# ShreyasBhaktharam/RDEIC

Hardware: AMD Instinct MI355X
Metric: 512x512 images/sec encode+relay-decode @ fixed bpp; 1/2/4/8 GPU (higher is better)
Workload: dtype bf16; 1 GPU; config 2: global batch 16 (16/GPU) 512x512, 2-step relay DDIM, encode+entropy-code+decode+VAE-decode; global_batch=16, image_size=512, ddim_steps=2, sampler=ddim, parallelism=dp1, codec_sessions_per_gpu=5

## Files before the change

### include/rdeic_hip.h

```cpp
#ifndef RDEIC_HIP_H
#define RDEIC_HIP_H
#include <stddef.h>
#include <stdint.h>
#ifdef __cplusplus
extern "C" {
#endif

int rdeic_version(void);
int rdeic_abi_count(void);

typedef struct rdeic_conv_desc {
  const void* in0;
  const void* in1;
  int32_t c0, c1;
  int32_t ld0, ld1;
  int32_t n, h, w;
  int32_t up2;
  const void* weight;
  int32_t wld;
  const float* bias;
  int32_t cout, kh, kw, stride, pad_t, pad_l;
  int32_t ho, wo;
  const float* gn_ab;
  int32_t gn_silu;
  const float* emb;
  int32_t emb_ld;
  int32_t act;
  float act_param;
  const void* res;
  int32_t res_ld;
  void* out;
  int32_t out_ld;
  int32_t out_mode;
  int32_t dtype;
  int32_t out_f32;
  int32_t batch;
  int64_t in_bs, w_bs, out_bs;
  float* gn_part;
  int32_t gn_hw;
  int32_t reserved;
  const float* ln_rows;
  const float* ln_colsum;
} rdeic_conv_desc;

int rdeic_conv2d(const rdeic_conv_desc* d, void* stream);
int rdeic_conv2d_tile(const rdeic_conv_desc* d, int32_t tile, void* stream);
int rdeic_conv2d_splitk(const rdeic_conv_desc* d, int32_t splits, float* ws, size_t ws_floats, void* stream);
int rdeic_conv2d_up2_phases(const rdeic_conv_desc* d, int64_t phase_stride, int32_t tile, void* stream);
int rdeic_conv2d_up2_group(const rdeic_conv_desc* d);
int rdeic_set_conv_path(int32_t path);
int rdeic_set_conv_option(int32_t key, int32_t value);

size_t rdeic_groupnorm_ws_floats(int32_t n, int32_t hw, int32_t c);
size_t rdeic_groupnorm_parts_floats(int64_t rows, int32_t c, int32_t hw);
int rdeic_groupnorm_parts_ab(const float* p0, int32_t c0, const float* p1, int32_t c1, int32_t n, int32_t hw,
                             int32_t groups, float eps, const float* gamma, const float* beta, float* ab,
                             void* stream);
int rdeic_groupnorm_stats(const void* x0, int32_t c0, int32_t ld0, const void* x1, int32_t c1, int32_t ld1,
                          int32_t n, int32_t hw, int32_t groups, float eps, const float* gamma, const float* beta,
                          float* ab, float* ws, int32_t dtype, void* stream);
int rdeic_groupnorm_parts_apply(const float* p0, int32_t c0, const float* p1, int32_t c1, const void* x0, int32_t ld0,
                                const void* x1, int32_t ld1, int32_t n, int32_t hw, int32_t groups, float eps,
                                const float* gamma, const float* beta, int32_t silu, float* ab, void* y, int32_t yld,
                                void* stream);
int rdeic_groupnorm_apply(const void* x, int32_t n, int32_t hw, int32_t c, int32_t ld, const float* ab,
                          int32_t ab_c, int32_t silu, float out_mul, void* y, int32_t yld, int32_t dtype,
                          void* stream);
int rdeic_layernorm(const void* x, int32_t rows, int32_t c, int32_t ld, const float* gamma, const float* beta,
                    float eps, void* y, int32_t yld, int32_t dtype, void* stream);

int rdeic_attention(const void* q, int32_t ldq, const void* k, int32_t ldk, const void* v, int32_t ldv,
                    void* o, int32_t ldo, int32_t batch, int32_t heads, int32_t lq, int32_t lk, int32_t dh,
                    float scale, int32_t kv_bcast, int32_t dtype, void* stream);
int rdeic_softmax_rows(const float* s, int64_t rows, int32_t cols, float scale, void* p, int32_t dtype, void* stream);
int rdeic_transpose(const void* in, int32_t rows, int32_t cols, int32_t ldin, void* out, int32_t ldout,
                    int32_t batch, int64_t in_bs, int64_t out_bs, int32_t dtype, void* stream);

int rdeic_geglu(const void* in, int32_t rows, int32_t c, int32_t ldin, void* out, int32_t ldout,
                int32_t dtype, void* stream);
int rdeic_nchw_to_nhwc(const float* in, int32_t n, int32_t c, int32_t h, int32_t w, float mul, float add,
                       void* out, int32_t ld, int32_t dtype, void* stream);
int rdeic_nhwc_to_nchw(const void* in, int32_t n, int32_t c, int32_t h, int32_t w, int32_t ld, float mul,
                       float add, float* out, int32_t dtype, void* stream);
int rdeic_axpby(const float* x, const float* z, int32_t n_img, int32_t per_img, const float* a,
                const float* b, float* y, void* stream);
int rdeic_timestep_embedding(const int64_t* t, const float* freqs, int32_t n, int32_t dim, float* out, void* stream);
int rdeic_ddim_step(const float* x, const float* e, int64_t count, float c_sq1m, float c_sqa, float c_sqap,
                    float c_dir, float* xp, float* x0, void* stream);
int rdeic_cfg_combine(const float* e_cond, const float* e_uncond, int64_t count, float scale, float* out,
                      void* stream);
int rdeic_spaced_step(const float* x, const float* e, const float* noise, int64_t count, float a, float b, float c1,
                      float c2, float s, float* xp, float* x0, void* stream);
int rdeic_silu_f32(const float* x, float* y, int64_t count, void* stream);
int rdeic_image_u8_to_nhwc(const uint8_t* img, int32_t n, int32_t h, int32_t w, void* out, int32_t ld,
                           int32_t dtype, void* stream);
int rdeic_nhwc_to_image_u8(const void* x, int32_t n, int32_t h, int32_t w, int32_t ld, uint8_t* img,
                           int32_t dtype, void* stream);
int rdeic_image_mse(const uint8_t* a, const uint8_t* b, int32_t n, int64_t per_img, float* out, void* stream);
int rdeic_fill_uniform(float* out, int64_t count, uint64_t seed, float scale, float offset, void* stream);
int rdeic_pack_conv_weight(const float* w, int32_t cout, int32_t cin, int32_t kh, int32_t kw, void* out,
                           int32_t wld, int32_t dtype, void* stream);
int rdeic_cast(const void* in, int32_t in_dtype, void* out, int32_t out_dtype, int64_t count, void* stream);

int rdeic_ckbd_encode(const void* y, int32_t yld, const void* params, int32_t pld, int32_t n, int32_t hy,
                      int32_t wy, int32_t c, int32_t phase, const float* scale_table, int32_t levels,
                      float scale_bound, int32_t* sym, int32_t* idx, int64_t img_stride, int64_t off,
                      void* yhat, int32_t yhld, void* anchor_out, int32_t ald, int32_t dtype, void* stream);
int rdeic_ckbd_indexes(const void* params, int32_t pld, int32_t n, int32_t hy, int32_t wy, int32_t c,
                       int32_t phase, const float* scale_table, int32_t levels, float scale_bound,
                       int32_t* idx, int64_t img_stride, int64_t off, int32_t dtype, void* stream);
int rdeic_ckbd_dequant(const int32_t* sym, const void* params, int32_t pld, int32_t n, int32_t hy,
                       int32_t wy, int32_t c, int32_t phase, int64_t img_stride, int64_t off, void* yhat,
                       int32_t yhld, void* anchor_out, int32_t ald, int32_t dtype, void* stream);
int rdeic_vq_argmin(const float* dot, const float* zn, const float* en, int32_t rows, int32_t ncode, int32_t* idx,
                    void* stream);
int rdeic_gather_rows(const float* table, int32_t ld_table, const int32_t* idx, int32_t rows, int32_t dim,
                      void* out, int32_t ld_out, int32_t dtype, void* stream);
int rdeic_row_sqnorm(const void* x, int32_t rows, int32_t dim, int32_t ld, float* out, int32_t dtype,
                     void* stream);

size_t rdeic_image_ssim_ws_floats(int32_t n, int32_t h, int32_t w, int32_t levels);
int rdeic_image_ssim(const uint8_t* a, const uint8_t* b, int32_t n, int32_t h, int32_t w, int32_t levels, float* ws,
                     size_t ws_floats, float* out, void* stream);

int rdeic_lpips_prep(const uint8_t* img, int32_t n, int32_t h, int32_t w, float* out, void* stream);
int rdeic_maxpool2d(const float* in, int32_t n, int32_t h, int32_t w, int32_t c, int32_t ld_in, int32_t k,
                    int32_t s, float* out, int32_t ld_out, void* stream);
size_t rdeic_lpips_layer_ws_floats(int32_t n, int64_t hw, int32_t c);
int rdeic_lpips_layer(const float* f0, int32_t ld0, const float* f1, int32_t ld1, const float* lin, int32_t n,
                      int64_t hw, int32_t c, int32_t accumulate, float* ws, size_t ws_floats, float* out,
                      void* stream);

int rdeic_pmf_to_quantized_cdf(const float* pmf, int32_t n, int32_t precision, uint32_t* cdf_out);
int rdeic_build_gaussian_tables(const float* pmf, const int32_t* pmf_len, int32_t levels, int32_t pmf_ld,
                                int32_t* cdf, int32_t cdf_ld, int32_t* cdf_len, void* reserved);

int rdeic_rans_encode(const int32_t* sym, const int32_t* idx, size_t n, const int32_t* cdf, int32_t cdf_ld,
                      const int32_t* cdf_len, const int32_t* offset, int32_t levels, uint8_t* out, size_t cap,
                      size_t* out_len);
int rdeic_rans_encode_batch(int32_t count, const int32_t* sym, const int32_t* idx, size_t n_per,
                            size_t stride, const int32_t* cdf, int32_t cdf_ld, const int32_t* cdf_len,
                            const int32_t* offset, int32_t levels, uint8_t* out, size_t cap_per,
                            size_t* out_len, int32_t threads);
void* rdeic_rans_enc_tables_create(const int32_t* cdf, int32_t cdf_ld, const int32_t* cdf_len,
                                   const int32_t* offset, int32_t levels);
void rdeic_rans_enc_tables_destroy(void* tables);
int rdeic_rans_encode_batch_t(const void* tables, int32_t count, const int32_t* sym, const int32_t* idx,
                              size_t n_per, size_t stride, uint8_t* out, size_t cap_per, size_t* out_len,
                              int32_t threads);
int rdeic_rans_enc_quotient(const void* tables, int32_t row, int32_t value, uint64_t x, uint64_t* q);
void* rdeic_rans_dec_open(const uint8_t* data, size_t len);
int rdeic_rans_decode(void* handle, const int32_t* idx, size_t n, const int32_t* cdf, int32_t cdf_ld,
                      const int32_t* cdf_len, const int32_t* offset, int32_t levels, int32_t* out);
int rdeic_rans_decode_batch(int32_t count, void** handles, const int32_t* idx, size_t n_per, size_t stride,
                            const int32_t* cdf, int32_t cdf_ld, const int32_t* cdf_len, const int32_t* offset,
                            int32_t levels, int32_t* out, int32_t threads);
void rdeic_rans_dec_close(void* handle);

int rdeic_ac_encode(const int16_t* sym, size_t n, const int16_t* cdf_row, int32_t lp, uint8_t* out,
                    size_t cap, size_t* out_len);
int rdeic_ac_decode(const uint8_t* data, size_t len, size_t n, const int16_t* cdf_row, int32_t lp,
                    int16_t* out);
int rdeic_ac_uniform_cdf(int32_t codebook_size, int16_t* cdf_row);

#define RDEIC_PROF_CONV 0
#define RDEIC_PROF_ATTN 1
#define RDEIC_PROF_ATTN_SMALL 2
#define RDEIC_PROF_GN_STATS 3
#define RDEIC_PROF_GN_APPLY 4
#define RDEIC_PROF_GEMM 5
#define RDEIC_PROF_ATTN_D512 6
#define RDEIC_PROF_CONV_BYTES 7
int rdeic_prof_start(int32_t capacity, int32_t every);
int rdeic_prof_read_keys(int32_t kind, int64_t* keys, int64_t* launches, double* work, double* ms, int32_t cap);
#define RDEIC_COUNT_HALO_CONV 0
#define RDEIC_COUNT_GN_APPLY 1
#define RDEIC_COUNT_LAYERNORM 2
#define RDEIC_COUNT_HALO_SMALL 3
#define RDEIC_COUNT_LN_FUSED 4
#define RDEIC_COUNT_SPLITK 5
#define RDEIC_COUNT_EDGE 6
#define RDEIC_COUNT_GN_PARTS_APPLY 7
#define RDEIC_COUNT_KINDS 8
int64_t rdeic_launch_count(int32_t kind);
int rdeic_layernorm_rowstats(const void* x, int32_t rows, int32_t c, int32_t ld, float eps, float* ms,
                             void* stream);
int rdeic_launch_count_reset(void);
int rdeic_prof_stop(void);
int rdeic_prof_read(int32_t kind, int64_t* launches, double* work, double* ms);

typedef struct rdeic_gemm_desc {
  const void* a;
  int64_t a_bs1, a_bs2, a_sm, a_sk;
  const void* b;
  int64_t b_bs1, b_bs2, b_sk, b_sn;
  void* c;
  int64_t c_bs1, c_bs2, c_sm;
  int32_t batch, nb2, m, n, k, ksplit, dtype, c_f32;
  float alpha, beta;
  float* rsum;
  int64_t rsum_bs;
} rdeic_gemm_desc;
int rdeic_gemm_strided(const rdeic_gemm_desc* d, void* stream);
int rdeic_pack_conv_weight_dgrad(const float* w, int32_t cout, int32_t cin, int32_t kh, int32_t kw, void* out,
                                 int32_t wld, int32_t to_bf16, void* stream);
typedef struct rdeic_pack_job {
  const float* w;
  void* out;
  int64_t start;
  int32_t cout, cin, kh, kw, wld, mode;
} rdeic_pack_job;
int rdeic_pack_batch(const rdeic_pack_job* jobs, int32_t njobs, int64_t total, int32_t row_floats, int32_t to_bf16,
                     void* stream);
int rdeic_zero_insert2(const void* src, int32_t n, int32_t h, int32_t w, int32_t c, int32_t ld, void* dst,
                       int32_t dst_ld, int32_t dtype, void* stream);
int rdeic_sum_pool2(const void* src, int32_t n, int32_t h, int32_t w, int32_t c, int32_t ld, void* dst,
                    int32_t dst_ld, int32_t dtype, void* stream);
int rdeic_pixel_unshuffle2(const void* src, int32_t n, int32_t h, int32_t w, int32_t c, int32_t ld, void* dst,
                           int32_t dst_ld, int32_t dtype, void* stream);
int rdeic_im2col(const void* x, int32_t n, int32_t h, int32_t w, int32_t c, int32_t ld, int32_t kh, int32_t kw,
                 int32_t stride, int32_t pad_t, int32_t pad_l, int32_t ho, int32_t wo, int32_t up2, void* out,
                 int64_t out_ld, int32_t dtype, void* stream);
int rdeic_wgrad_finalize(const float* part, int32_t splits, int32_t cout, int32_t cin, int32_t kh, int32_t kw,
                         float* dw, int32_t accumulate, const float* rpart, float* db, void* stream);
size_t rdeic_col_sum_ws_floats(int64_t rows, int32_t c, int32_t groups);
int rdeic_col_sum(const void* x, int64_t rows, int32_t c, int32_t ld, int32_t groups, float* out, int32_t accumulate,
                  float* ws, size_t ws_floats, int32_t dtype, void* stream);
int rdeic_act_fwd(const void* z, int64_t rows, int32_t c, int32_t ldz, const void* res, int32_t ldr, int32_t act,
                  float slope, void* out, int32_t ldo, int32_t dtype, void* stream);
int rdeic_act_bwd(const void* dy, int32_t ldy, const void* z, int32_t ldz, int64_t rows, int32_t c, int32_t act,
                  float slope, void* dz, int32_t lddz, int32_t dtype, void* stream);
size_t rdeic_gn_train_ws_doubles(int32_t n, int32_t hw, int32_t c);
int rdeic_gn_train_fwd(const void* x, int32_t ldx, int32_t n, int32_t hw, int32_t c, int32_t groups, float eps,
                       const float* gamma, const float* beta, float* mr, float* ab, double* ws, int32_t dtype,
                       void* stream);
int rdeic_gn_train_bwd(const void* x, int32_t ldx, const void* dy, int32_t ldy, int32_t n, int32_t hw, int32_t c,
                       int32_t groups, const float* mr, const float* gamma, const float* beta, int32_t silu, void* dx,
                       int32_t lddx, float* dgamma, float* dbeta, int32_t accumulate, double* ws, float* coef,
                       int32_t dtype, void* stream);
int rdeic_gn_train_bwd_res(const void* x, int32_t ldx, const void* dy, int32_t ldy, int32_t n, int32_t hw, int32_t c,
                           int32_t groups, const float* mr, const float* gamma, const float* beta, int32_t silu,
                           const void* dres, int32_t ldr, void* dx, int32_t lddx, float* dgamma, float* dbeta,
                           int32_t accumulate, double* ws, float* coef, int32_t dtype, void* stream);
size_t rdeic_layernorm_bwd_ws_floats(int64_t rows, int32_t c);
int rdeic_layernorm_bwd(const void* x, int32_t ldx, int64_t rows, int32_t c, const float* gamma, float eps,
                        const void* dy, int32_t ldy, void* dx, int32_t lddx, float* dgamma, float* dbeta,
                        int32_t accumulate, float* ws, size_t ws_floats, int32_t dtype, void* stream);
int rdeic_layernorm_bwd_res(const void* x, int32_t ldx, int64_t rows, int32_t c, const float* gamma, float eps,
                            const void* dy, int32_t ldy, const void* dres, int32_t ldr, void* dx, int32_t lddx,
                            float* dgamma, float* dbeta, int32_t accumulate, float* ws, size_t ws_floats,
                            int32_t dtype, void* stream);
int rdeic_softmax_bwd_rows(const void* p, const float* dp, int64_t rows, int32_t cols, float scale, void* ds,
                           int32_t dtype, void* stream);
int rdeic_attention_fwd_lse(const void* q, int32_t ldq, const void* k, int32_t ldk, const void* v, int32_t ldv,
                            void* o, int32_t ldo, float* lse, int32_t batch, int32_t heads, int32_t lq, int32_t lk,
                            int32_t dh, float scale, int32_t dtype, void* stream);
size_t rdeic_attention_bwd_workspace(int32_t batch, int32_t heads, int32_t lq, int32_t lk, int32_t dh);
int rdeic_attention_bwd(const void* q, int32_t ldq, const void* k, int32_t ldk, const void* v, int32_t ldv,
                        const void* o, int32_t ldo, const void* d_o, int32_t lddo, const float* lse,
                        void* dq, int32_t lddq, void* dk, int32_t lddk, void* dv, int32_t lddv,
                        void* ws, size_t ws_bytes, int32_t batch, int32_t heads, int32_t lq, int32_t lk,
                        int32_t dh, float scale, int32_t dtype, void* stream);
int rdeic_geglu_bwd(const void* x, int32_t ldx, int64_t rows, int32_t c, const void* dy, int32_t ldy, void* dx,
                    int32_t lddx, int32_t dtype, void* stream);
int rdeic_ckbd_train_anchor(const void* y, int32_t ldy, const void* pa, int32_t ldpa, int32_t n, int32_t h, int32_t w,
                            int32_t c, void* out, int32_t ldo, int32_t dtype, void* stream);
int rdeic_ckbd_mask(const void* x, int32_t ldx, int32_t n, int32_t h, int32_t w, int32_t c, int32_t which, void* out,
                    int32_t ldo, int32_t dtype, void* stream);
size_t rdeic_ckbd_train_ws_doubles(int32_t n, int32_t h, int32_t w, int32_t c);
int rdeic_ckbd_train_lik(const void* y, int32_t ldy, const void* pa, int32_t ldpa, const void* pn, int32_t ldpn,
                         const float* noise, int32_t n, int32_t h, int32_t w, int32_t c, void* nonanchor_hat,
                         int32_t ldo, double* ws, float* out2, int32_t dtype, void* stream);
int rdeic_ckbd_train_lik_bwd(const void* y, int32_t ldy, const void* pa, int32_t ldpa, const void* pn, int32_t ldpn,
                             const float* noise, int32_t n, int32_t h, int32_t w, int32_t c, const float* g_sum,
                             const void* d_nonanchor, int32_t ldd, void* dy, int32_t lddy, void* dpa, int32_t lddpa,
                             void* dpn, int32_t lddpn, int32_t dtype, void* stream);
int rdeic_vq_train(const float* dot, const float* zn, const float* en, const float* z, const int32_t* idx, int32_t P,
                   int32_t K, int32_t D, float* E, float* embed_prob, float beta, float decay, float temp,
                   float* code_out, float* dE_unit, float* loss3, void* stream);
int rdeic_vq_z_grad(const float* z, const float* zq, const void* dzq, int64_t count, const float* g_loss, float coef,
                    void* dz, int32_t dtype, void* stream);
int rdeic_scale_dev(const float* x, int64_t count, const float* s, float* y, int32_t accumulate, void* stream);
int rdeic_adamw(float* p, const float* g, float* m, float* v, int64_t count, float lr, float beta1, float beta2,
                float eps, float weight_decay, int32_t step, void* stream);
int rdeic_adamw_dev(float* p, const float* g, float* m, float* v, int64_t count, float lr, float beta1, float beta2,
                    float eps, float weight_decay, const float* step_scalars, void* stream);

#ifdef __cplusplus
}
#endif
#endif
```

### rdeic_amd/_lib.py

```python
from __future__ import annotations

import ctypes as C
import os
import threading

_HERE = os.path.dirname(os.path.abspath(__file__))
LIB_PATH = os.environ.get("RDEIC_LIB") or os.path.join(_HERE, "lib", "librdeic_hip.so")

EINVAL, ENOSPC, EBADMSG, ELAUNCH = -22, -28, -74, -5
_ERRNAMES = {EINVAL: "EINVAL (bad argument/shape)", ENOSPC: "ENOSPC (output capacity)",
             EBADMSG: "EBADMSG (corrupt or truncated bitstream)", ELAUNCH: "kernel launch failure"}


class RdeicError(RuntimeError):
    def __init__(self, fn: str, code: int):
        super().__init__(f"{fn} failed: {code} {_ERRNAMES.get(code, '')}")
        self.code = code


class BitstreamError(RdeicError, ValueError):
    """Corrupt / truncated bitstream (the reference's 'decode failure')."""


class ConvDesc(C.Structure):
    _fields_ = [
        ("in0", C.c_void_p), ("in1", C.c_void_p),
        ("c0", C.c_int32), ("c1", C.c_int32), ("ld0", C.c_int32), ("ld1", C.c_int32),
        ("n", C.c_int32), ("h", C.c_int32), ("w", C.c_int32), ("up2", C.c_int32),
        ("weight", C.c_void_p), ("wld", C.c_int32),
        ("bias", C.c_void_p),
        ("cout", C.c_int32), ("kh", C.c_int32), ("kw", C.c_int32), ("stride", C.c_int32),
        ("pad_t", C.c_int32), ("pad_l", C.c_int32),
        ("ho", C.c_int32), ("wo", C.c_int32),
        ("gn_ab", C.c_void_p), ("gn_silu", C.c_int32),
        ("emb", C.c_void_p), ("emb_ld", C.c_int32),
        ("act", C.c_int32), ("act_param", C.c_float),
        ("res", C.c_void_p), ("res_ld", C.c_int32),
        ("out", C.c_void_p), ("out_ld", C.c_int32), ("out_mode", C.c_int32),
        ("dtype", C.c_int32), ("out_f32", C.c_int32),
        ("batch", C.c_int32), ("in_bs", C.c_int64), ("w_bs", C.c_int64), ("out_bs", C.c_int64),
        ("gn_part", C.c_void_p), ("gn_hw", C.c_int32), ("reserved", C.c_int32),
        ("ln_rows", C.c_void_p), ("ln_colsum", C.c_void_p),
    ]


class GemmDesc(C.Structure):
    _fields_ = [
        ("a", C.c_void_p), ("a_bs1", C.c_int64), ("a_bs2", C.c_int64), ("a_sm", C.c_int64), ("a_sk", C.c_int64),
        ("b", C.c_void_p), ("b_bs1", C.c_int64), ("b_bs2", C.c_int64), ("b_sk", C.c_int64), ("b_sn", C.c_int64),
        ("c", C.c_void_p), ("c_bs1", C.c_int64), ("c_bs2", C.c_int64), ("c_sm", C.c_int64),
        ("batch", C.c_int32), ("nb2", C.c_int32), ("m", C.c_int32), ("n", C.c_int32), ("k", C.c_int32),
        ("ksplit", C.c_int32), ("dtype", C.c_int32), ("c_f32", C.c_int32),
        ("alpha", C.c_float), ("beta", C.c_float), ("rsum", C.c_void_p), ("rsum_bs", C.c_int64),
    ]


_p, _i32, _i64, _u64, _f, _sz = C.c_void_p, C.c_int32, C.c_int64, C.c_uint64, C.c_float, C.c_size_t

PROTOTYPES = {
    "rdeic_version": (C.c_int, []),
    "rdeic_abi_count": (C.c_int, []),
    "rdeic_conv2d": (C.c_int, [C.POINTER(ConvDesc), _p]),
    "rdeic_conv2d_splitk": (C.c_int, [C.POINTER(ConvDesc), _i32, _p, C.c_size_t, _p]),
    "rdeic_conv2d_tile": (C.c_int, [C.POINTER(ConvDesc), _i32, _p]),
    "rdeic_conv2d_up2_phases": (C.c_int, [C.POINTER(ConvDesc), _i64, _i32, _p]),
    "rdeic_conv2d_up2_group": (C.c_int, [C.POINTER(ConvDesc)]),
    "rdeic_prof_start": (C.c_int, [_i32, _i32]),
    "rdeic_prof_stop": (C.c_int, []),
    "rdeic_launch_count": (C.c_int64, [_i32]),
    "rdeic_launch_count_reset": (C.c_int, []),
    "rdeic_layernorm_rowstats": (C.c_int, [C.c_void_p, _i32, _i32, _i32, C.c_float, C.c_void_p, C.c_void_p]),
    "rdeic_prof_read": (C.c_int, [_i32, C.POINTER(C.c_int64), C.POINTER(C.c_double), C.POINTER(C.c_double)]),
    "rdeic_prof_read_keys": (C.c_int, [_i32, C.POINTER(C.c_int64), C.POINTER(C.c_int64), C.POINTER(C.c_double),
                                       C.POINTER(C.c_double), _i32]),
    "rdeic_groupnorm_ws_floats": (_sz, [_i32, _i32, _i32]),
    "rdeic_groupnorm_stats": (C.c_int, [_p, _i32, _i32, _p, _i32, _i32, _i32, _i32, _i32, _f, _p, _p, _p, _p,
                                        _i32, _p]),
    "rdeic_groupnorm_apply": (C.c_int, [_p, _i32, _i32, _i32, _i32, _p, _i32, _i32, _f, _p, _i32, _i32, _p]),
    "rdeic_set_conv_path": (C.c_int, [_i32]),
    "rdeic_set_conv_option": (C.c_int, [_i32, _i32]),
    "rdeic_layernorm": (C.c_int, [_p, _i32, _i32, _i32, _p, _p, _f, _p, _i32, _i32, _p]),
    "rdeic_softmax_rows": (C.c_int, [_p, _i64, _i32, _f, _p, _i32, _p]),
    "rdeic_transpose": (C.c_int, [_p, _i32, _i32, _i32, _p, _i32, _i32, _i64, _i64, _i32, _p]),
    "rdeic_attention": (C.c_int, [_p, _i32, _p, _i32, _p, _i32, _p, _i32, _i32, _i32, _i32, _i32, _i32, _f,
                                  _i32, _i32, _p]),
    "rdeic_geglu": (C.c_int, [_p, _i32, _i32, _i32, _p, _i32, _i32, _p]),
    "rdeic_nchw_to_nhwc": (C.c_int, [_p, _i32, _i32, _i32, _i32, _f, _f, _p, _i32, _i32, _p]),
    "rdeic_nhwc_to_nchw": (C.c_int, [_p, _i32, _i32, _i32, _i32, _i32, _f, _f, _p, _i32, _p]),
    "rdeic_axpby": (C.c_int, [_p, _p, _i32, _i32, _p, _p, _p, _p]),
    "rdeic_timestep_embedding": (C.c_int, [_p, _p, _i32, _i32, _p, _p]),
    "rdeic_ddim_step": (C.c_int, [_p, _p, _i64, _f, _f, _f, _f, _p, _p, _p]),
    "rdeic_spaced_step": (C.c_int, [_p, _p, _p, _i64, _f, _f, _f, _f, _f, _p, _p, _p]),
    "rdeic_cfg_combine": (C.c_int, [_p, _p, _i64, _f, _p, _p]),
    "rdeic_silu_f32": (C.c_int, [_p, _p, _i64, _p]),
    "rdeic_image_u8_to_nhwc": (C.c_int, [_p, _i32, _i32, _i32, _p, _i32, _i32, _p]),
    "rdeic_nhwc_to_image_u8": (C.c_int, [_p, _i32, _i32, _i32, _i32, _p, _i32, _p]),
    "rdeic_image_mse": (C.c_int, [_p, _p, _i32, _i64, _p, _p]),
    "rdeic_fill_uniform": (C.c_int, [_p, _i64, _u64, _f, _f, _p]),
    "rdeic_pack_conv_weight": (C.c_int, [_p, _i32, _i32, _i32, _i32, _p, _i32, _i32, _p]),
    "rdeic_cast": (C.c_int, [_p, _i32, _p, _i32, _i64, _p]),
    "rdeic_ckbd_encode": (C.c_int, [_p, _i32, _p, _i32, _i32, _i32, _i32, _i32, _i32, _p, _i32, _f, _p, _p,
                                    _i64, _i64, _p, _i32, _p, _i32, _i32, _p]),
    "rdeic_ckbd_indexes": (C.c_int, [_p, _i32, _i32, _i32, _i32, _i32, _i32, _p, _i32, _f, _p, _i64, _i64,
                                     _i32, _p]),
    "rdeic_ckbd_dequant": (C.c_int, [_p, _p, _i32, _i32, _i32, _i32, _i32, _i32, _i64, _i64, _p, _i32, _p,
                                     _i32, _i32, _p]),
    "rdeic_vq_argmin": (C.c_int, [_p, _p, _p, _i32, _i32, _p, _p]),
    "rdeic_gather_rows": (C.c_int, [_p, _i32, _p, _i32, _i32, _p, _i32, _i32, _p]),
    "rdeic_row_sqnorm": (C.c_int, [_p, _i32, _i32, _i32, _p, _i32, _p]),
    "rdeic_pmf_to_quantized_cdf": (C.c_int, [_p, _i32, _i32, _p]),
    "rdeic_build_gaussian_tables": (C.c_int, [_p, _p, _i32, _i32, _p, _i32, _p, _p]),
    "rdeic_rans_encode": (C.c_int, [_p, _p, _sz, _p, _i32, _p, _p, _i32, _p, _sz, C.POINTER(_sz)]),
    "rdeic_rans_encode_batch": (C.c_int, [_i32, _p, _p, _sz, _sz, _p, _i32, _p, _p, _i32, _p, _sz, _p, _i32]),
    "rdeic_image_ssim_ws_floats": (C.c_size_t, [_i32, _i32, _i32, _i32]),
    "rdeic_image_ssim": (C.c_int, [_p, _p, _i32, _i32, _i32, _i32, _p, C.c_size_t, _p, _p]),
    "rdeic_lpips_prep": (C.c_int, [_p, _i32, _i32, _i32, _p, _p]),
    "rdeic_maxpool2d": (C.c_int, [_p, _i32, _i32, _i32, _i32, _i32, _i32, _i32, _p, _i32, _p]),
    "rdeic_lpips_layer_ws_floats": (_sz, [_i32, _i64, _i32]),
    "rdeic_lpips_layer": (C.c_int, [_p, _i32, _p, _i32, _p, _i32, _i64, _i32, _i32, _p, _sz, _p, _p]),
    "rdeic_groupnorm_parts_floats": (C.c_size_t, [_i64, _i32, _i32]),
    "rdeic_groupnorm_parts_ab": (C.c_int, [_p, _i32, _p, _i32, _i32, _i32, _i32, _f, _p, _p, _p, _p]),
    "rdeic_groupnorm_parts_apply": (C.c_int, [_p, _i32, _p, _i32, _p, _i32, _p, _i32, _i32, _i32, _i32, _f, _p, _p,
                                              _i32, _p, _p, _i32, _p]),
    "rdeic_rans_enc_tables_create": (_p, [_p, _i32, _p, _p, _i32]),
    "rdeic_rans_enc_tables_destroy": (None, [_p]),
    "rdeic_rans_encode_batch_t": (C.c_int, [_p, _i32, _p, _p, _sz, _sz, _p, _sz, _p, _i32]),
    "rdeic_rans_enc_quotient": (C.c_int, [_p, _i32, _i32, C.c_uint64, C.POINTER(C.c_uint64)]),
    "rdeic_rans_dec_open": (_p, [_p, _sz]),
    "rdeic_rans_decode": (C.c_int, [_p, _p, _sz, _p, _i32, _p, _p, _i32, _p]),
    "rdeic_rans_decode_batch": (C.c_int, [_i32, _p, _p, _sz, _sz, _p, _i32, _p, _p, _i32, _p, _i32]),
    "rdeic_rans_dec_close": (None, [_p]),
    "rdeic_ac_encode": (C.c_int, [_p, _sz, _p, _i32, _p, _sz, C.POINTER(_sz)]),
    "rdeic_ac_decode": (C.c_int, [_p, _sz, _sz, _p, _i32, _p]),
    "rdeic_ac_uniform_cdf": (C.c_int, [_i32, _p]),
    "rdeic_gemm_strided": (C.c_int, [C.POINTER(GemmDesc), _p]),
    "rdeic_pack_conv_weight_dgrad": (C.c_int, [_p, _i32, _i32, _i32, _i32, _p, _i32, _i32, _p]),
    "rdeic_pack_batch": (C.c_int, [_p, _i32, _i64, _i32, _i32, _p]),
    "rdeic_zero_insert2": (C.c_int, [_p, _i32, _i32, _i32, _i32, _i32, _p, _i32, _i32, _p]),
    "rdeic_sum_pool2": (C.c_int, [_p, _i32, _i32, _i32, _i32, _i32, _p, _i32, _i32, _p]),
    "rdeic_pixel_unshuffle2": (C.c_int, [_p, _i32, _i32, _i32, _i32, _i32, _p, _i32, _i32, _p]),
    "rdeic_im2col": (C.c_int, [_p, _i32, _i32, _i32, _i32, _i32, _i32, _i32, _i32, _i32, _i32, _i32, _i32, _i32, _p,
                               _i64, _i32, _p]),
    "rdeic_wgrad_finalize": (C.c_int, [_p, _i32, _i32, _i32, _i32, _i32, _p, _i32, _p, _p, _p]),
    "rdeic_col_sum_ws_floats": (_sz, [_i64, _i32, _i32]),
    "rdeic_col_sum": (C.c_int, [_p, _i64, _i32, _i32, _i32, _p, _i32, _p, _sz, _i32, _p]),
    "rdeic_act_fwd": (C.c_int, [_p, _i64, _i32, _i32, _p, _i32, _i32, _f, _p, _i32, _i32, _p]),
    "rdeic_act_bwd": (C.c_int, [_p, _i32, _p, _i32, _i64, _i32, _i32, _f, _p, _i32, _i32, _p]),
    "rdeic_gn_train_ws_doubles": (_sz, [_i32, _i32, _i32]),
    "rdeic_gn_train_fwd": (C.c_int, [_p, _i32, _i32, _i32, _i32, _i32, _f, _p, _p, _p, _p, _p, _i32, _p]),
    "rdeic_gn_train_bwd": (C.c_int, [_p, _i32, _p, _i32, _i32, _i32, _i32, _i32, _p, _p, _p, _i32, _p, _i32, _p, _p,
                                     _i32, _p, _p, _i32, _p]),
    "rdeic_gn_train_bwd_res": (C.c_int, [_p, _i32, _p, _i32, _i32, _i32, _i32, _i32, _p, _p, _p, _i32, _p, _i32, _p,
                                         _i32, _p, _p, _i32, _p, _p, _i32, _p]),
    "rdeic_layernorm_bwd_ws_floats": (_sz, [_i64, _i32]),
    "rdeic_layernorm_bwd": (C.c_int, [_p, _i32, _i64, _i32, _p, _f, _p, _i32, _p, _i32, _p, _p, _i32, _p, _sz, _i32,
                                      _p]),
    "rdeic_layernorm_bwd_res": (C.c_int, [_p, _i32, _i64, _i32, _p, _f, _p, _i32, _p, _i32, _p, _i32, _p, _p, _i32, _p,
                                          _sz, _i32, _p]),
    "rdeic_softmax_bwd_rows": (C.c_int, [_p, _p, _i64, _i32, _f, _p, _i32, _p]),
    "rdeic_attention_fwd_lse": (C.c_int, [_p, _i32, _p, _i32, _p, _i32, _p, _i32, _p, _i32, _i32, _i32, _i32, _i32, _f,
                                          _i32, _p]),
    "rdeic_attention_bwd_workspace": (_sz, [_i32, _i32, _i32, _i32, _i32]),
    "rdeic_attention_bwd": (C.c_int, [_p, _i32, _p, _i32, _p, _i32, _p, _i32, _p, _i32, _p, _p, _i32, _p, _i32, _p,
                                      _i32, _p, _sz, _i32, _i32, _i32, _i32, _i32, _f, _i32, _p]),
    "rdeic_geglu_bwd": (C.c_int, [_p, _i32, _i64, _i32, _p, _i32, _p, _i32, _i32, _p]),
    "rdeic_ckbd_train_anchor": (C.c_int, [_p, _i32, _p, _i32, _i32, _i32, _i32, _i32, _p, _i32, _i32, _p]),
    "rdeic_ckbd_mask": (C.c_int, [_p, _i32, _i32, _i32, _i32, _i32, _i32, _p, _i32, _i32, _p]),
    "rdeic_ckbd_train_ws_doubles": (_sz, [_i32, _i32, _i32, _i32]),
    "rdeic_ckbd_train_lik": (C.c_int, [_p, _i32, _p, _i32, _p, _i32, _p, _i32, _i32, _i32, _i32, _p, _i32, _p, _p,
                                       _i32, _p]),
    "rdeic_ckbd_train_lik_bwd": (C.c_int, [_p, _i32, _p, _i32, _p, _i32, _p, _i32, _i32, _i32, _i32, _p, _p, _i32, _p,
                                           _i32, _p, _i32, _p, _i32, _i32, _p]),
    "rdeic_vq_train": (C.c_int, [_p, _p, _p, _p, _p, _i32, _i32, _i32, _p, _p, _f, _f, _f, _p, _p, _p, _p]),
    "rdeic_vq_z_grad": (C.c_int, [_p, _p, _p, _i64, _p, _f, _p, _i32, _p]),
    "rdeic_scale_dev": (C.c_int, [_p, _i64, _p, _p, _i32, _p]),
    "rdeic_adamw": (C.c_int, [_p, _p, _p, _p, _i64, _f, _f, _f, _f, _f, _i32, _p]),
    "rdeic_adamw_dev": (C.c_int, [_p, _p, _p, _p, _i64, _f, _f, _f, _f, _f, _p, _p]),
}

_lib = None
_lock = threading.Lock()


def load() -> C.CDLL:
    global _lib
    if _lib is not None:
        return _lib
    with _lock:
        if _lib is not None:
            return _lib
        if not os.path.exists(LIB_PATH):
            raise ImportError(f"librdeic_hip.so not built at {LIB_PATH}; run `make` (or __graft_entry__.build()).")
        import torch
        lib = C.CDLL(LIB_PATH, mode=C.RTLD_GLOBAL)
        for name, (res, args) in PROTOTYPES.items():
            fn = getattr(lib, name)
            fn.restype = res
            fn.argtypes = args
        _lib = lib
    return _lib


def check(name: str, rc: int) -> None:
    if rc != 0:
        if rc == EBADMSG:
            raise BitstreamError(name, rc)
        raise RdeicError(name, rc)


RECORDER = None


def call(name: str, *args, tag=None) -> None:
    fn = getattr(load(), name)
    if RECORDER is not None:
        RECORDER.append((name, fn, args, tag))
    rc = fn(*args)
    check(name, rc)


def call_soft(name: str, *args, tag=None) -> bool:
    fn = getattr(load(), name)
    rc = fn(*args)
    if rc == 1:
        return False
    check(name, rc)
    if RECORDER is not None:
        RECORDER.append((name, fn, args, tag))
    return True
```

### rdeic_amd/csrc/coders.cpp

```cpp
#include <stdint.h>
#include <string.h>

#include <algorithm>
#include <atomic>
#include <condition_variable>
#include <functional>
#include <mutex>
#include <cmath>
#include <new>
#include <stdexcept>
#include <thread>
#include <vector>

#include "../../include/rdeic_hip.h"

#define RDEIC_OK 0
#define RDEIC_EINVAL (-22)
#define RDEIC_ENOSPC (-28)
#define RDEIC_EBADMSG (-74)

namespace {

constexpr int kPrecision = 16;
constexpr uint32_t kBypassBits = 4;
// ... 94 lines not shown
  if (freq < 2) {
    s.rcp = ~0ull;
    s.shift = 0;
    s.bias = start + (1u << kPrecision) - 1;
  } else {
    uint32_t sh = 0;
    while (freq > (1u << sh)) ++sh;
    const unsigned __int128 num = ((unsigned __int128)1 << (sh + 63)) + (freq - 1);
    s.rcp = (uint64_t)(num / freq);
    s.shift = (uint8_t)(sh - 1);
    s.bias = start;
  }
  return s;
}

inline uint64_t enc_quot(uint64_t x, const EncSym& s) {
  return (uint64_t)(((unsigned __int128)x * s.rcp) >> 64) >> s.shift;
}

struct WordSink {
  std::vector<uint32_t>& buf;
  size_t wp;
  explicit WordSink(std::vector<uint32_t>& b) : buf(b), wp(b.size()) {}
  void emit(uint32_t w) {
    if (wp == 0) grow();
    buf[--wp] = w;
  }
  void grow() {
    const size_t old = buf.size(), add = std::max<size_t>(old, 1024);
    std::vector<uint32_t> nb(old + add);
    memcpy(nb.data() + add, buf.data(), old * sizeof(uint32_t));
    buf.swap(nb);
    wp += add;
  }
};

inline void enc_put(uint64_t& x, WordSink& ws, const EncSym& s) {
  if ((x >> 47) >= s.freq) {
    ws.emit((uint32_t)x);
    x >>= 32;
  }
  x = x + s.bias + enc_quot(x, s) * ((1u << kPrecision) - s.freq);
}

inline void enc_put_bits(uint64_t& x, WordSink& ws, uint32_t v) {
  if ((x >> 59) != 0) {
    ws.emit((uint32_t)x);
    x >>= 32;
  }
  x = (x << kBypassBits) | v;
}

int rans_encode_tab_impl(const EncTables& T, const int32_t* sym, const int32_t* idx, size_t n, uint8_t* out,
                         size_t cap, size_t* out_len, std::vector<uint32_t>& buf) {
  if (buf.size() < n / 2 + 256) buf.assign(n / 2 + 256, 0u);
  WordSink ws(buf);
  uint64_t x = kRansL;
  for (size_t i = n; i-- > 0;) {
    const int32_t ci = idx[i];
    if (ci < 0 || ci >= T.levels) return RDEIC_EINVAL;
    const int32_t max_value = T.max_value[ci];
    int32_t value = sym[i] - T.offset[ci];
    if (value < 0 || value >= max_value) {
      const uint32_t raw = value < 0 ? (uint32_t)(-2 * (int64_t)value - 1) : (uint32_t)(2 * (int64_t)(value - max_value));
      int32_t nb = 0;
      while (nb < 8 && (raw >> (nb * kBypassBits)) != 0) ++nb;
      for (int32_t j = nb; j-- > 0;) enc_put_bits(x, ws, (raw >> (j * kBypassBits)) & kBypassMax);
      enc_put_bits(x, ws, (uint32_t)(nb % (int32_t)kBypassMax));
      for (int32_t v = nb / (int32_t)kBypassMax; v-- > 0;) enc_put_bits(x, ws, kBypassMax);
      value = max_value;
    }
    enc_put(x, ws, T.sym[(size_t)T.row_off[ci] + value]);
  }
  ws.emit((uint32_t)(x >> 32));
  ws.emit((uint32_t)x);
  const size_t nbytes = (ws.buf.size() - ws.wp) * 4;
  *out_len = nbytes;
  if (nbytes > cap) return RDEIC_ENOSPC;
  memcpy(out, ws.buf.data() + ws.wp, nbytes);
  return RDEIC_OK;
}

struct RansDecoder {
  std::vector<uint32_t> words;
  size_t pos = 0;
  uint64_t x = 0;
  bool bad = false;

  bool read_word(uint32_t& w) {
    if (pos >= words.size()) { bad = true; return false; }
    w = words[pos++];
    return true;
  }
  uint32_t get_bits(uint32_t nbits) {
    uint32_t v = (uint32_t)(x & ((1u << nbits) - 1));
    x >>= nbits;
    if (x < kRansL) {
      uint32_t w;
      if (read_word(w)) x = (x << 32) | w;
    }
    return v;
  }
};

int rans_decode_impl(RansDecoder* d, const int32_t* idx, size_t n, const int32_t* cdf, int32_t cdf_ld,
                     const int32_t* cdf_len, const int32_t* offset, int32_t levels, int32_t* out) {
  if (d->bad) return RDEIC_EBADMSG;
  for (size_t i = 0; i < n; ++i) {
    const int32_t ci = idx[i];
    if (ci < 0 || ci >= levels) return RDEIC_EINVAL;
    const int32_t* row = cdf + (size_t)ci * cdf_ld;
    const int32_t len = cdf_len[ci];
    const int32_t max_value = len - 2;
    if (max_value < 0 || len > cdf_ld) return RDEIC_EINVAL;
    const uint32_t cum = (uint32_t)(d->x & ((1u << kPrecision) - 1));
    const int32_t* it = std::upper_bound(row, row + len, (int32_t)cum);
    int32_t s = (int32_t)(it - row) - 1;
    if (s < 0 || s >= len - 1) return RDEIC_EBADMSG;
    const uint64_t start = (uint32_t)row[s], freq = (uint32_t)(row[s + 1] - row[s]);
    uint64_t x = d->x;
    x = freq * (x >> kPrecision) + (x & ((1u << kPrecision) - 1)) - start;
    if (x < kRansL) {
      uint32_t w;
      if (!d->read_word(w)) return RDEIC_EBADMSG;
      x = (x << 32) | w;
    }
    d->x = x;
    int32_t value = s;
    if (value == max_value) {
      int32_t v = (int32_t)d->get_bits(kBypassBits);
      int32_t nb = v;
      while (v == (int32_t)kBypassMax) {
        if (d->bad || nb > 8) return RDEIC_EBADMSG;
        v = (int32_t)d->get_bits(kBypassBits);
        nb += v;
      }
      if (nb > 8) return RDEIC_EBADMSG;
      uint32_t raw = 0;
      for (int32_t j = 0; j < nb; ++j) {
        uint32_t nib = d->get_bits(kBypassBits);
        raw |= nib << (j * kBypassBits);
      }
      if (d->bad) return RDEIC_EBADMSG;
      value = (int32_t)(raw >> 1);
      if (raw & 1)
        value = -value - 1;
      else
        value += max_value;
    }
    out[i] = value + offset[ci];
  }
  return d->bad ? RDEIC_EBADMSG : RDEIC_OK;
}

class WorkerPool {
 public:
  static WorkerPool& get() {
    thread_local WorkerPool* p = new WorkerPool();
    return *p;
  }
  void run(int32_t count, int32_t threads, const std::function<void(int32_t)>& f) {
    std::lock_guard<std::mutex> job(job_mu_);
    int32_t helpers = std::max(0, std::min(threads, count) - 1);
    while ((int32_t)workers_.size() < helpers) {
      const int32_t id = (int32_t)workers_.size();
      try {
        workers_.reserve(workers_.size() + 1);
        std::thread(&WorkerPool::loop, this, id).detach();
      } catch (...) {
        helpers = (int32_t)workers_.size();
        break;
      }
      workers_.push_back(id);
    }
    {
      std::lock_guard<std::mutex> lk(mu_);
      fn_ = &f;
      count_ = count;
      next_.store(0);
      helpers_ = helpers;
      active_ = helpers;
      ++gen_;
    }
    cv_.notify_all();
    work();
    std::unique_lock<std::mutex> lk(mu_);
    done_cv_.wait(lk, [&] { return active_ == 0; });
    fn_ = nullptr;
  }

 private:
  void work() {
    for (;;) {
      const int32_t i = next_.fetch_add(1);
      if (i >= count_) break;
      (*fn_)(i);
    }
  }
  void loop(int32_t id) {
    uint64_t seen = 0;
    for (;;) {
      {
        std::unique_lock<std::mutex> lk(mu_);
        cv_.wait(lk, [&] { return gen_ != seen; });
        seen = gen_;
        if (id >= helpers_) continue;
      }
      work();
      std::lock_guard<std::mutex> lk(mu_);
      if (--active_ == 0) done_cv_.notify_all();
    }
  }

  std::mutex job_mu_, mu_;
  std::condition_variable cv_, done_cv_;
  std::vector<int32_t> workers_;
  const std::function<void(int32_t)>* fn_ = nullptr;
  std::atomic<int32_t> next_{0};
  int32_t count_ = 0, active_ = 0, helpers_ = 0;
  uint64_t gen_ = 0;
};

template <typename F>
int guard(F&& f) noexcept {
  try {
    return f();
  } catch (const std::bad_alloc&) {
    return RDEIC_ENOSPC;
  } catch (...) {
    return RDEIC_EINVAL;
  }
}

template <typename F>
void parallel_for(int32_t count, int32_t threads, F&& f) {
  if (threads <= 1 || count <= 1) {
    for (int32_t i = 0; i < count; ++i) f(i);
    return;
  }
  const std::function<void(int32_t)> fn = f;
  WorkerPool::get().run(count, threads, fn);
}

struct BitWriter {
  uint8_t* out;
  size_t cap;
  size_t len = 0;
  uint8_t cache = 0;
  int count = 0;
  bool overflow = false;
  void put(int bit) {
    cache = (uint8_t)((cache << 1) | (bit & 1));
    if (++count == 8) {
      if (len < cap) out[len] = cache; else overflow = true;
      ++len;
      count = 0;
      cache = 0;
    }
  }
  void put_with_pending(int bit, uint64_t& pending) {
    put(bit);
    while (pending > 0) { put(!bit); --pending; }
  }
  void flush() {
    while (count > 0) put(0);
  }
};

struct BitReader {
  const uint8_t* in;
  size_t n;
  size_t ptr = 0;
  uint8_t cache = 0;
  int cached = 0;
  void get(uint32_t& value) {
    if (cached == 0) {
      if (ptr == n) { value <<= 1; return; }
      cache = in[ptr++];
      cached = 8;
    }
    value = (value << 1) | ((cache >> (cached - 1)) & 1);
    --cached;
  }
};

inline uint16_t binsearch_u16(const uint16_t* cdf, uint16_t target, uint16_t max_sym) {
  uint16_t left = 0, right = (uint16_t)(max_sym + 1);
  while (left + 1 < right) {
    const uint16_t m = (uint16_t)((left + right) / 2);
    const uint16_t v = cdf[m];
    if (v < target) left = m;
    else if (v > target) right = m;
    else return m;
  }
  return left;
}

}

extern "C" {

int rdeic_version(void) { return 1; }

int rdeic_abi_count(void) { return 102; }

static int pmf_to_quantized_cdf_impl(const float* pmf, int32_t n, int32_t precision, uint32_t* cdf_out) {
  if (!pmf || !cdf_out || n <= 0 || precision <= 0 || precision > 24) return RDEIC_EINVAL;
  for (int32_t i = 0; i < n; ++i)
    if (!(pmf[i] >= 0.f) || !std::isfinite(pmf[i])) return RDEIC_EINVAL;
  const uint32_t one = 1u << precision;
  std::vector<uint32_t> cdf((size_t)n + 1);
  cdf[0] = 0;
  for (int32_t i = 0; i < n; ++i) cdf[i + 1] = (uint32_t)std::round(pmf[i] * (float)one);
  uint64_t total = 0;
  for (uint32_t v : cdf) total += v;
  if (total == 0) return RDEIC_EINVAL;
  for (auto& v : cdf) v = (uint32_t)(((uint64_t)one * v) / total);
  for (size_t i = 1; i < cdf.size(); ++i) cdf[i] += cdf[i - 1];
  cdf.back() = one;
  const int32_t m = (int32_t)cdf.size();
  for (int32_t i = 0; i < m - 1; ++i) {
    if (cdf[i] == cdf[i + 1]) {
      uint32_t best_freq = ~0u;
      int32_t best = -1;
      for (int32_t j = 0; j < m - 1; ++j) {
        const uint32_t f = cdf[j + 1] - cdf[j];
        if (f > 1 && f < best_freq) { best_freq = f; best = j; }
      }
      if (best < 0) return RDEIC_EINVAL;
      if (best < i) {
        for (int32_t j = best + 1; j <= i; ++j) cdf[j]--;
      } else {
        for (int32_t j = i + 1; j <= best; ++j) cdf[j]++;
      }
    }
  }
  memcpy(cdf_out, cdf.data(), cdf.size() * sizeof(uint32_t));
  return RDEIC_OK;
}

int rdeic_pmf_to_quantized_cdf(const float* pmf, int32_t n, int32_t precision, uint32_t* cdf_out) {
  return guard([&] { return pmf_to_quantized_cdf_impl(pmf, n, precision, cdf_out); });
}

static int build_gaussian_tables_impl(const float* pmf, const int32_t* pmf_len, int32_t levels, int32_t pmf_ld,
                                      int32_t* cdf, int32_t cdf_ld, int32_t* cdf_len) {
  if (!pmf || !pmf_len || !cdf || !cdf_len || levels <= 0) return RDEIC_EINVAL;
  std::vector<float> row;
  std::vector<uint32_t> q;
  for (int32_t i = 0; i < levels; ++i) {
    const int32_t L = pmf_len[i];
    if (L <= 0 || L + 1 > pmf_ld || L + 2 > cdf_ld) return RDEIC_EINVAL;
    row.assign(pmf + (size_t)i * pmf_ld, pmf + (size_t)i * pmf_ld + L + 1);
    q.assign((size_t)L + 2, 0u);
    int rc = pmf_to_quantized_cdf_impl(row.data(), L + 1, kPrecision, q.data());
    if (rc) return rc;
    int32_t* out = cdf + (size_t)i * cdf_ld;
    for (int32_t j = 0; j < cdf_ld; ++j) out[j] = j < L + 2 ? (int32_t)q[j] : 0;
    cdf_len[i] = L + 2;
  }
  return RDEIC_OK;
}

int rdeic_build_gaussian_tables(const float* pmf, const int32_t* pmf_len, int32_t levels, int32_t pmf_ld, int32_t* cdf,
                                int32_t cdf_ld, int32_t* cdf_len, void* reserved) {
  (void)reserved;
  return guard([&] { return build_gaussian_tables_impl(pmf, pmf_len, levels, pmf_ld, cdf, cdf_ld, cdf_len); });
}

int rdeic_rans_encode(const int32_t* sym, const int32_t* idx, size_t n, const int32_t* cdf, int32_t cdf_ld,
                      const int32_t* cdf_len, const int32_t* offset, int32_t levels, uint8_t* out, size_t cap,
                      size_t* out_len) {
  if ((!sym || !idx) && n) return RDEIC_EINVAL;
  if (!cdf || !cdf_len || !offset || !out || !out_len || levels <= 0) return RDEIC_EINVAL;
  return guard([&] {
    std::vector<RansSym> syms;
    std::vector<uint32_t> words;
    return rans_encode_impl(sym, idx, n, cdf, cdf_ld, cdf_len, offset, levels, out, cap, out_len, syms, words);
  });
}

int rdeic_rans_encode_batch(int32_t count, const int32_t* sym, const int32_t* idx, size_t n_per, size_t stride,
                            const int32_t* cdf, int32_t cdf_ld, const int32_t* cdf_len, const int32_t* offset,
                            int32_t levels, uint8_t* out, size_t cap_per, size_t* out_len, int32_t threads) {
  if (count <= 0 || !sym || !idx || !out || !out_len) return RDEIC_EINVAL;
  return guard([&] {
    std::vector<int> rc(count, 0);
    parallel_for(count, threads, [&](int32_t i) {
      rc[i] = guard([&] {
        std::vector<RansSym> syms;
        std::vector<uint32_t> words;
        return rans_encode_impl(sym + i * stride, idx + i * stride, n_per, cdf, cdf_ld, cdf_len, offset, levels,
                                out + i * cap_per, cap_per, &out_len[i], syms, words);
      });
    });
    for (int v : rc)
      if (v) return v;
    return (int)RDEIC_OK;
  });
}

void* rdeic_rans_enc_tables_create(const int32_t* cdf, int32_t cdf_ld, const int32_t* cdf_len, const int32_t* offset,
                                   int32_t levels) {
  if (!cdf || !cdf_len || !offset || levels <= 0 || cdf_ld < 2) return nullptr;
  EncTables* T = new (std::nothrow) EncTables();
  if (!T) return nullptr;
  try {
    T->levels = levels;
    T->row_off.resize(levels);
    T->max_value.resize(levels);
    T->offset.assign(offset, offset + levels);
    size_t total = 0;
    for (int32_t ci = 0; ci < levels; ++ci) {
      const int32_t len = cdf_len[ci];
      if (len < 2 || len > cdf_ld) throw std::invalid_argument("cdf_len");
      T->row_off[ci] = (int32_t)total;
      T->max_value[ci] = len - 2;
      total += (size_t)len - 1;
    }
    T->sym.resize(total);
    for (int32_t ci = 0; ci < levels; ++ci) {
      const int32_t* row = cdf + (size_t)ci * cdf_ld;
      for (int32_t v = 0; v <= T->max_value[ci]; ++v) {
        const int32_t start = row[v], freq = row[v + 1] - row[v];
        if (start < 0 || freq <= 0 || start + freq > (1 << kPrecision)) throw std::invalid_argument("cdf row");
        T->sym[(size_t)T->row_off[ci] + v] = make_enc_sym((uint32_t)start, (uint32_t)freq);
      }
    }
  } catch (...) {
    delete T;
    return nullptr;
  }
  return T;
}

void rdeic_rans_enc_tables_destroy(void* tables) { delete (EncTables*)tables; }

int rdeic_rans_encode_batch_t(const void* tables, int32_t count, const int32_t* sym, const int32_t* idx, size_t n_per,
                              size_t stride, uint8_t* out, size_t cap_per, size_t* out_len, int32_t threads) {
  if (!tables || count <= 0 || ((!sym || !idx) && n_per) || !out || !out_len) return RDEIC_EINVAL;
  const EncTables& T = *(const EncTables*)tables;
  return guard([&] {
    std::vector<int> rc(count, 0);
    parallel_for(count, threads, [&](int32_t i) {
      rc[i] = guard([&] {
        thread_local std::vector<uint32_t> buf;
        return rans_encode_tab_impl(T, sym + i * stride, idx + i * stride, n_per, out + i * cap_per, cap_per,
                                    &out_len[i], buf);
      });
    });
    for (int v : rc)
      if (v) return v;
    return (int)RDEIC_OK;
  });
}

int rdeic_rans_enc_quotient(const void* tables, int32_t row, int32_t value, uint64_t x, uint64_t* q) {
  if (!tables || !q) return RDEIC_EINVAL;
  const EncTables& T = *(const EncTables*)tables;
  if (row < 0 || row >= T.levels || value < 0 || value > T.max_value[row]) return RDEIC_EINVAL;
  const EncSym& s = T.sym[(size_t)T.row_off[row] + value];
  *q = s.freq < 2 ? x : enc_quot(x, s);
  return RDEIC_OK;
}

void* rdeic_rans_dec_open(const uint8_t* data, size_t len) {
  if (!data && len) return nullptr;
  RansDecoder* d = new (std::nothrow) RansDecoder();
  if (!d) return nullptr;
  const size_t nw = len / 4;
  try {
    d->words.resize(nw);
  } catch (...) {
    delete d;
    return nullptr;
  }
  if (nw) memcpy(d->words.data(), data, nw * 4);
  if (len % 4 != 0 || nw < 2) {
    d->bad = true;
    return d;
  }
  d->x = (uint64_t)d->words[0] | ((uint64_t)d->words[1] << 32);
  d->pos = 2;
  return d;
}

int rdeic_rans_decode(void* handle, const int32_t* idx, size_t n, const int32_t* cdf, int32_t cdf_ld,
                      const int32_t* cdf_len, const int32_t* offset, int32_t levels, int32_t* out) {
  if (!handle || (!idx && n) || (!out && n) || !cdf || !cdf_len || !offset) return RDEIC_EINVAL;
  return guard([&] { return rans_decode_impl((RansDecoder*)handle, idx, n, cdf, cdf_ld, cdf_len, offset, levels, out); });
}

int rdeic_rans_decode_batch(int32_t count, void** handles, const int32_t* idx, size_t n_per, size_t stride,
                            const int32_t* cdf, int32_t cdf_ld, const int32_t* cdf_len, const int32_t* offset,
                            int32_t levels, int32_t* out, int32_t threads) {
  if (count <= 0 || !handles || !idx || !out) return RDEIC_EINVAL;
  return guard([&] {
    std::vector<int> rc(count, 0);
    parallel_for(count, threads, [&](int32_t i) {
      rc[i] = handles[i] ? guard([&] {
        return rans_decode_impl((RansDecoder*)handles[i], idx + i * stride, n_per, cdf, cdf_ld, cdf_len, offset,
                                levels, out + i * stride);
      })
                         : (int)RDEIC_EINVAL;
    });
    for (int v : rc)
      if (v) return v;
    return (int)RDEIC_OK;
  });
}

void rdeic_rans_dec_close(void* handle) { delete (RansDecoder*)handle; }

int rdeic_ac_uniform_cdf(int32_t codebook_size, int16_t* cdf_row) {
  if (codebook_size <= 0 || codebook_size > 32768 || !cdf_row) return RDEIC_EINVAL;
  const int32_t lp = codebook_size + 1;
  const float p = 1.0f / (float)codebook_size;
  float acc = 0.f;
  const float maxv = 65536.0f - (float)(lp - 1);
  for (int32_t k = 0; k < lp; ++k) {
    float c = (k == lp - 1) ? 1.0f : acc;
    float v = std::nearbyint(c * maxv);
    int32_t iv = (int32_t)v;
    cdf_row[k] = (int16_t)(uint16_t)((uint32_t)(iv + k) & 0xFFFFu);
    acc += p;
  }
  return RDEIC_OK;
}

int rdeic_ac_encode(const int16_t* sym, size_t n, const int16_t* cdf_row, int32_t lp, uint8_t* out, size_t cap,
                    size_t* out_len) {
  if ((!sym && n) || !cdf_row || lp < 2 || !out || !out_len) return RDEIC_EINVAL;
  const uint16_t* cdf = (const uint16_t*)cdf_row;
  const int32_t max_symbol = lp - 2;
  BitWriter bw{out, cap};
  uint32_t low = 0, high = 0xFFFFFFFFu;
  uint64_t pending = 0;
  for (size_t i = 0; i < n; ++i) {
    const int32_t s = sym[i];
    if (s < 0 || s > max_symbol) return RDEIC_EINVAL;
    const uint64_t span = (uint64_t)high - (uint64_t)low + 1;
    const uint32_t c_low = cdf[s];
    const uint32_t c_high = s == max_symbol ? 0x10000u : cdf[s + 1];
    high = (low - 1) + (uint32_t)((span * c_high) >> kPrecision);
    low = low + (uint32_t)((span * c_low) >> kPrecision);
    for (;;) {
      if (high < 0x80000000u) {
        bw.put_with_pending(0, pending);
        low <<= 1;
        high = (high << 1) | 1;
      } else if (low >= 0x80000000u) {
        bw.put_with_pending(1, pending);
        low <<= 1;
        high = (high << 1) | 1;
      } else if (low >= 0x40000000u && high < 0xC0000000u) {
        ++pending;
        low = (low << 1) & 0x7FFFFFFFu;
        high = (high << 1) | 0x80000001u;
      } else {
        break;
      }
    }
  }
  pending += 1;
  bw.put_with_pending(low < 0x40000000u ? 0 : 1, pending);
  bw.flush();
  *out_len = bw.len;
  return bw.overflow ? RDEIC_ENOSPC : RDEIC_OK;
}

int rdeic_ac_decode(const uint8_t* data, size_t len, size_t n, const int16_t* cdf_row, int32_t lp, int16_t* out) {
  if ((!data && len) || !cdf_row || lp < 2 || (!out && n)) return RDEIC_EINVAL;
  if (n == 0) return RDEIC_OK;
  const uint16_t* cdf = (const uint16_t*)cdf_row;
  const uint16_t max_symbol = (uint16_t)(lp - 2);
  BitReader br{data, len};
  uint32_t low = 0, high = 0xFFFFFFFFu, value = 0;
  for (int i = 0; i < 32; ++i) br.get(value);
  for (size_t i = 0; i < n; ++i) {
    const uint64_t span = (uint64_t)high - (uint64_t)low + 1;
    const uint16_t count = (uint16_t)((((uint64_t)value - (uint64_t)low + 1) * 0x10000u - 1) / span);
    const uint16_t s = binsearch_u16(cdf, count, max_symbol);
    out[i] = (int16_t)s;
    if (i == n - 1) break;
    const uint32_t c_low = cdf[s];
    const uint32_t c_high = s == max_symbol ? 0x10000u : cdf[s + 1];
    high = (low - 1) + (uint32_t)((span * c_high) >> kPrecision);
    low = low + (uint32_t)((span * c_low) >> kPrecision);
    for (;;) {
      if (low >= 0x80000000u || high < 0x80000000u) {
        low <<= 1;
        high = (high << 1) | 1;
        br.get(value);
      } else if (low >= 0x40000000u && high < 0xC0000000u) {
        low = (low << 1) & 0x7FFFFFFFu;
        high = (high << 1) | 0x80000001u;
        value -= 0x40000000u;
        br.get(value);
      } else {
        break;
      }
    }
  }
  return RDEIC_OK;
}

}
// ... 1 lines not shown
```

### rdeic_amd/csrc/conv_gemm.hip

```cpp
#include "conv_common.h"

namespace rdeic_conv {

int g_conv_path = 2;
int g_epi_vec = 1;
int g_swz = 1;
int g_force_tile = -1;
int g_dma = 1;
int g_halo = 1;
int g_halo8 = 1;
int g_up2_phases = 1;

namespace {

template <typename T, int BM, int BN, int WGM, int WGN, bool VEC, bool GNP = true, bool SWZ = true>
__global__ __launch_bounds__(WGM * WGN * 64) void conv_kernel(ConvArgs a) {
  constexpr int NT = WGM * WGN * 64;
  constexpr int BK = MmaTraits<T>::BK;
  constexpr int EPC = MmaTraits<T>::EPC;
  constexpr int ES = sizeof(T);
  constexpr int WTM = BM / WGM, WTN = BN / WGN;
  constexpr int TM = WTM / 16, TN = WTN / 16;
  constexpr int RPI = NT / 8;
  constexpr int AR = BM / RPI;
// ... 425 lines not shown
    if (a.res) v[e] += a.out_f32 ? reinterpret_cast<const float*>(a.res)[(long)m * a.res_ld + nn + e]
                                 : to_f32(reinterpret_cast<const bf16*>(a.res)[(long)m * a.res_ld + nn + e]);
  }
  if (a.out_f32) {
    float* o = reinterpret_cast<float*>(a.out) + (long)m * a.out_ld + nn;
#pragma unroll
    for (int e = 0; e < 8; ++e) o[e] = v[e];
    if (st) {
#pragma unroll
      for (int e = 0; e < 8; ++e) st[e] = v[e];
    }
  } else {
    bf16 ov[8];
#pragma unroll
    for (int e = 0; e < 8; ++e) ov[e] = from_f32<bf16>(v[e]);
    *reinterpret_cast<uint4*>(reinterpret_cast<bf16*>(a.out) + (long)m * a.out_ld + nn) = *reinterpret_cast<uint4*>(ov);
    if (st) {
#pragma unroll
      for (int e = 0; e < 8; ++e) st[e] = to_f32(ov[e]);
    }
  }
}

__global__ __launch_bounds__(256) void splitk_reduce_kernel(ConvArgs a, const float* __restrict__ part) {
  const int cp = a.cout >> 3;
  const long i = (long)blockIdx.x * 256 + threadIdx.x;
  if (i >= (long)a.M * cp) return;
  const int m = (int)(i / cp), nn = (int)(i - (long)m * cp) * 8;
  splitk_reduce_chunk(a, part, m, nn);
}

}

int make_args(const rdeic_conv_desc* d, ConvArgs& a, bool& vec) {
  if (!d || !d->in0 || !d->weight || !d->out) return RDEIC_EINVAL;
  if (d->c0 <= 0 || d->c1 < 0 || (d->c1 > 0 && !d->in1) || d->cout <= 0 || d->kh <= 0 || d->kw <= 0 ||
      d->stride <= 0 || d->n <= 0 || d->ho <= 0 || d->wo <= 0)
    return RDEIC_EINVAL;
  if (d->dtype != 0 && d->dtype != 1) return RDEIC_EINVAL;
  a.in0 = (const char*)d->in0; a.in1 = (const char*)(d->in1 ? d->in1 : d->in0);
  a.c0 = d->c0; a.c1 = d->c1; a.ld0 = d->ld0; a.ld1 = d->c1 ? d->ld1 : d->ld0;
  a.n = d->n; a.h = d->h; a.w = d->w; a.up2 = d->up2;
  a.weight = (const char*)d->weight; a.wld = d->wld; a.bias = d->bias;
  a.cout = d->cout; a.kh = d->kh; a.kw = d->kw; a.stride = d->stride; a.pad_t = d->pad_t; a.pad_l = d->pad_l;
  a.ho = d->ho; a.wo = d->wo;
  a.gn_ab = d->gn_ab; a.gn_silu = d->gn_silu;
  a.emb = d->emb; a.emb_ld = d->emb_ld;
  a.act = d->act; a.act_param = d->act_param;
  a.res = (const char*)d->res; a.res_ld = d->res_ld;
  a.out = (char*)d->out; a.out_ld = d->out_ld; a.out_mode = d->out_mode;
  a.out_f32 = d->out_f32;
  a.epi_vec = g_epi_vec;
  a.splits = 1; a.kper = 0;
  a.gn_part = d->gn_part; a.gn_row0 = 0; a.gn_hw = d->gn_hw;
  a.ln_rows = d->ln_rows; a.ln_cs = d->ln_colsum;
  if ((d->ln_rows != nullptr) != (d->ln_colsum != nullptr)) return RDEIC_EINVAL;
  if (d->ln_rows && (d->dtype != 1 || d->batch > 1 || d->out_mode == 1 || d->gn_ab || ((uintptr_t)d->ln_colsum) % 16))
    return RDEIC_EINVAL;
  a.M = d->n * d->ho * d->wo;
  a.batch = d->batch > 1 ? d->batch : 1;
  a.in_bs = d->in_bs; a.w_bs = d->w_bs; a.out_bs = d->out_bs;
  if (a.batch > 1 && (d->res || d->emb || d->out_mode)) return RDEIC_EINVAL;
  a.cin = d->c0 + d->c1;
  a.ktot = d->kh * d->kw * a.cin;
  const int BK = d->dtype == 1 ? 64 : 32;
  if (d->wld < a.ktot || d->wld % 64 != 0) return RDEIC_EINVAL;
  a.nk = (a.ktot + BK - 1) / BK;
  if (d->out_mode < 0 || d->out_mode > 2) return RDEIC_EINVAL;
  if (d->out_mode == 1 && (d->cout % 4 != 0)) return RDEIC_EINVAL;
  if (d->out_mode == 2 && (d->dtype != 1 || d->cout % 8 || d->res || d->emb || d->act || d->out_f32 || d->gn_ab ||
                           a.batch > 1 || d->out_ld % 4 || ((uintptr_t)d->out) % 8))
    return RDEIC_EINVAL;
  const int epc = d->dtype == 1 ? 8 : 4;
  vec = (d->c0 % epc == 0) && (d->ld0 % epc == 0) && (((uintptr_t)d->in0) % 16 == 0);
  if (d->c1) vec = vec && (d->c1 % epc == 0) && (d->ld1 % epc == 0) && (((uintptr_t)d->in1) % 16 == 0);
  if (((uintptr_t)d->weight) % 16 != 0) return RDEIC_EINVAL;
  return RDEIC_OK;
}
}

using namespace rdeic_conv;

static int conv2d_run(const rdeic_conv_desc* d, void* stream, bool* fused) {
  ConvArgs a;
  bool vec = false;
  const int rc = make_args(d, a, vec);
  if (rc != RDEIC_OK) return rc;
  float* const part = a.gn_part;
  a.gn_part = nullptr;
  hipStream_t s = (hipStream_t)stream;
  {
    ConvArgs e = a;
    e.gn_part = part;
    const int rc2 = launch_edge(d, e, s, fused);
    if (rc2 != -1) return rc2;
  }
  if (d->out_mode == 2) {
    const int rc2 = vec ? dma_grouped(d, -1, s) : -1;
    return rc2 == -1 ? RDEIC_EINVAL : rc2;
  }

  if (vec && g_halo && (d->gn_ab || g_halo == 2) && halo_ok(d, a)) {
    a.gn_part = part;
    const int rc2 = launch_halo(d, a, s, fused);
    if (rc2 != -1) return rc2;
    a.gn_part = nullptr;
  }
  if (d->dtype == 1 && vec && d->cout <= 4 && d->c0 % 32 == 0 && d->kh == 3 && d->kw == 3 && d->stride == 1 && d->pad_t == 1 &&
      d->pad_l == 1 && !d->up2 && !d->c1 && d->out_mode == 0 && a.batch == 1 && d->ho == d->h && d->wo == d->w &&
      g_conv_path != 0)
    return launch_smallc(a, s);
  if (d->dtype == 1 && vec && !d->gn_ab && d->cout > 32 && g_conv_path != 0) {
    if (g_dma) {
      const int rc2 = dma_grouped(d, -1, s, fused);
      if (rc2 != -1) return rc2;
    }
    a.gn_part = part;
    return launch_plain_auto(a, s, -1, fused);
  }
  if (d->dtype == 1) {
    if (d->cout <= 16) return launch_cfg<bf16, 128, 16, 4, 1>(a, vec, s);
    if (d->cout <= 32) return launch_cfg<bf16, 128, 32, 4, 1>(a, vec, s);
    if (d->cout % 128 != 0 && d->cout % 64 == 0) return launch_cfg<bf16, 128, 64, 2, 2>(a, vec, s);
    if (a.M <= 4096) return launch_cfg<bf16, 64, 128, 2, 2>(a, vec, s);
    return launch_cfg<bf16, 128, 128, 2, 2>(a, vec, s);
  } else {
    if (d->cout <= 16) return launch_cfg<float, 64, 16, 4, 1>(a, vec, s);
    if (d->cout >= 128 && (long)cdiv(a.M, 128) * cdiv(a.cout, 128) * a.batch >= 512)
      return launch_cfg<float, 128, 128, 2, 2>(a, vec, s);
    return launch_cfg<float, 64, 64, 2, 2>(a, vec, s);
  }
}

static int conv2d_tile_run(const rdeic_conv_desc* d, int32_t tile, void* stream, bool* fused) {
  ConvArgs a;
  bool vec = false;
  const int rc = make_args(d, a, vec);
  if (rc != RDEIC_OK) return rc;
  if (vec) {
    const int rc2 = launch_edge(d, a, (hipStream_t)stream, fused);
    if (rc2 != -1) return rc2;
  }
  if (d->out_mode == 2) {
    const int rc2 = vec ? dma_grouped(d, tile >= 20 ? tile : -1, (hipStream_t)stream) : -1;
    return rc2 == -1 ? RDEIC_EINVAL : rc2;
  }
  if (d->dtype == 1 && vec && !d->gn_ab && d->cout > 32 && g_conv_path != 0) {
    if (tile >= 20) {
      const int rc2 = dma_grouped(d, tile, (hipStream_t)stream, fused);
      if (rc2 != -1) return rc2;
      tile = -1;
    }
    return launch_plain_auto(a, (hipStream_t)stream, tile, fused);
  }
  return conv2d_run(d, stream, fused);
}

static double conv_flops(const rdeic_conv_desc* d) {
  if (!d) return 0.0;
  const double b = d->batch > 1 ? d->batch : 1;
  return 2.0 * b * d->n * d->ho * d->wo * d->cout * (double)d->kh * d->kw * (d->c0 + d->c1);
}

static double conv_bytes(const rdeic_conv_desc* d) {
  if (!d) return 0.0;
  const double b = d->batch > 1 ? d->batch : 1;
  const double es = d->dtype == 1 ? 2.0 : 4.0, os = (d->dtype == 0 || d->out_f32) ? 4.0 : 2.0;
  const double in = b * d->n * (double)d->h * d->w * (d->c0 + d->c1) * es;
  const double w = (double)(d->batch > 1 ? b : 1) * d->cout * d->wld * es;
  double outc = d->out_mode == 2 ? d->cout / 2.0 : (double)d->cout;
  const double out = b * d->n * (d->out_mode == 1 ? 4.0 : 1.0) * d->ho * d->wo * (d->out_mode == 1 ? outc / 4 : outc) * os;
  return in + w + out + (d->res ? out : 0.0);
}

static int conv2d_impl(const rdeic_conv_desc* d, int32_t tile, void* stream) {
  if (d && d->gn_part &&
      (d->gn_hw <= 0 || d->gn_hw % 64 || d->batch > 1 || d->out_mode != 0 || (long)d->n * d->ho * d->wo % d->gn_hw))
    return RDEIC_EINVAL;
  bool fused = false;
  int rc;
  {
    rdeic_prof_add_bytes(conv_bytes(d));
    ProfScope ps((hipStream_t)stream, RDEIC_PROF_CONV, conv_flops(d));
    rc = tile == -2 ? conv2d_run(d, stream, &fused) : conv2d_tile_run(d, tile, stream, &fused);
  }
  if (rc != RDEIC_OK || !d->gn_part || fused) return rc;
  const long rows = (long)d->n * d->ho * d->wo;
  return gn_rows_partial(d->out, rows, d->cout, d->out_ld, d->gn_hw, d->gn_part,
                         (d->out_f32 || d->dtype == 0) ? 0 : 1, (hipStream_t)stream);
}

static int conv2d_splitk_impl(const rdeic_conv_desc* d, int32_t splits, float* ws, size_t ws_floats,
                              void* stream) {
  ConvArgs a;
  bool vec = false;
  const int rc = make_args(d, a, vec);
  if (rc != RDEIC_OK) return rc;
  if (!vec || d->gn_ab || d->out_mode != 0 || a.batch != 1 || d->cout % 8 || splits < 2 || !ws ||
      (d->out_ld % 8) || ((uintptr_t)d->out % 16) || ((uintptr_t)ws % 16))
    return RDEIC_EINVAL;
  if (ws_floats < (size_t)splits * a.M * a.cout) return RDEIC_ENOSPC;
  hipStream_t s = (hipStream_t)stream;
  float* const part = ws;
  if (d->dtype == 0) {
    ConvArgs p = a;
    p.bias = nullptr; p.emb = nullptr; p.act = 0; p.res = nullptr; p.gn_part = nullptr; p.ln_rows = nullptr;
    p.out = (char*)part; p.out_ld = a.cout; p.out_f32 = 0;
    p.splits = splits;
    p.kper = (a.nk + splits - 1) / splits;
    dim3 grid(cdiv(a.M, 64), cdiv(a.cout, 64), splits);
    constexpr int lds = conv_lds_bytes<float, 64, 64>();
    hipLaunchKernelGGL((conv_kernel<float, 64, 64, 2, 2, true, false, true>), grid, dim3(256), lds, s, p);
    a.splits = splits;
    a.out_f32 = 1;
    const long chunks = (long)a.M * (a.cout / 8);
    hipLaunchKernelGGL(splitk_reduce_kernel, dim3((unsigned)((chunks + 255) / 256)), dim3(256), 0, s, a,
                       (const float*)part);
    return launch_status();
  }
  if (g_dma) {
    rdeic_conv_desc e = *d;
    e.bias = nullptr; e.emb = nullptr; e.act = 0; e.res = nullptr; e.gn_part = nullptr; e.ln_rows = nullptr;
    e.out = part; e.out_ld = d->cout; e.out_f32 = 1;
    ConvArgs pa;
    bool pv = false;
    unsigned b0, b1, bw;
    if (make_args(&e, pa, pv) == RDEIC_OK && pv && dma_ok(&e, pa, b0, b1, bw)) {
      pa.splits = splits; pa.kper = (pa.nk + splits - 1) / splits;
      if (launch_dma_auto(pa, b0, b1, bw, s, -1) == RDEIC_OK) {
        a.splits = splits;
        const long chunks = (long)a.M * (a.cout / 8);
        hipLaunchKernelGGL(splitk_reduce_kernel, dim3((unsigned)((chunks + 255) / 256)), dim3(256), 0, s, a,
                           (const float*)part);
        return launch_status();
      }
    }
  }
  ConvArgs p = a;
  p.bias = nullptr; p.emb = nullptr; p.act = 0; p.res = nullptr; p.gn_part = nullptr; p.ln_rows = nullptr;
  p.out = (char*)part; p.out_ld = a.cout; p.out_f32 = 1;
  p.splits = splits;
  p.kper = (a.nk + splits - 1) / splits;
  dim3 grid(cdiv(a.M, 128), cdiv(a.cout, 128), splits);
  constexpr int lds = conv_lds_bytes<bf16, 128, 128>();
  hipLaunchKernelGGL((conv_kernel<bf16, 128, 128, 2, 2, true, false, true>), grid, dim3(256), lds, s, p);
  a.splits = splits;
  const long chunks = (long)a.M * (a.cout / 8);
  hipLaunchKernelGGL(splitk_reduce_kernel, dim3((unsigned)((chunks + 255) / 256)), dim3(256), 0, s, a,
                     (const float*)part);
  return launch_status();
}

extern "C" int rdeic_conv2d(const rdeic_conv_desc* d, void* stream) { return conv2d_impl(d, -2, stream); }

extern "C" int rdeic_conv2d_tile(const rdeic_conv_desc* d, int32_t tile, void* stream) {
  return conv2d_impl(d, tile, stream);
}

extern "C" int rdeic_conv2d_splitk(const rdeic_conv_desc* d, int32_t splits, float* ws, size_t ws_floats,
                                   void* stream) {
  if (d && d->gn_part && (d->gn_hw <= 0 || d->gn_hw % 64 || (long)d->n * d->ho * d->wo % d->gn_hw))
    return RDEIC_EINVAL;
  int rc;
  {
    rdeic_prof_add_bytes(conv_bytes(d));
    ProfScope ps((hipStream_t)stream, RDEIC_PROF_CONV, conv_flops(d));
    rc = conv2d_splitk_impl(d, splits, ws, ws_floats, stream);
  }
  if (rc == RDEIC_OK) rdeic_count_launch(RDEIC_COUNT_SPLITK);
  if (rc != RDEIC_OK || !d->gn_part) return rc;
  return gn_rows_partial(d->out, (long)d->n * d->ho * d->wo, d->cout, d->out_ld, d->gn_hw, d->gn_part,
                         d->out_f32 ? 0 : 1, (hipStream_t)stream);
}

extern "C" int rdeic_conv2d_up2_phases(const rdeic_conv_desc* d, int64_t phase_stride, int32_t tile, void* stream) {
  if (!d) return RDEIC_EINVAL;
  if (!g_up2_phases || !g_dma || g_conv_path == 0) return 1;
  if (d->gn_part && (d->gn_hw <= 0 || d->gn_hw % 64 || (long)d->n * d->ho * d->wo % d->gn_hw)) return RDEIC_EINVAL;
  if (!up2_phases_ok(d, phase_stride)) return 1;
  bool fused = false;
  int rc;
  {
    const double pix = (double)d->n * d->h * d->w;
    rdeic_prof_add_bytes(2.0 * (pix * d->c0 + 4.0 * d->cout * d->wld + 4.0 * pix * d->cout));
    ProfScope ps((hipStream_t)stream, RDEIC_PROF_CONV, 2.0 * pix * 4.0 * d->c0 * d->cout * 4.0);
    rc = launch_up2_phases(d, phase_stride, tile, (hipStream_t)stream, &fused);
  }
  if (rc == -1) return RDEIC_EINVAL;
  if (rc != RDEIC_OK || !d->gn_part || fused) return rc;
  return gn_rows_partial(d->out, (long)d->n * d->ho * d->wo, d->cout, d->out_ld, d->gn_hw, d->gn_part, 1,
                         (hipStream_t)stream);
}

extern "C" int rdeic_conv2d_up2_group(const rdeic_conv_desc* d) { return d ? up2_phase_group(d) : 0; }

extern "C" int rdeic_set_conv_path(int32_t path) {
  int prev = g_conv_path;
  g_conv_path = path;
  return prev;
}

extern int rdeic_g_attn64;
extern int rdeic_g_attn512;

extern "C" int rdeic_set_conv_option(int32_t key, int32_t value) {
  if (key == 0) { int prev = g_epi_vec; g_epi_vec = value; return prev; }
  if (key == 1) { int prev = rdeic_g_attn64; rdeic_g_attn64 = value; return prev; }
  if (key == 3) { int prev = g_swz; g_swz = value; return prev; }
  if (key == 4) { int prev = g_force_tile; g_force_tile = value; return prev; }
  if (key == 5) { int prev = g_dma; g_dma = value; return prev; }
  if (key == 6) { int prev = g_halo; g_halo = value; return prev; }
  if (key == 8) { int prev = rdeic_g_attn512; rdeic_g_attn512 = value; return prev; }
  if (key == 9) { int prev = g_halo8; g_halo8 = value; return prev; }
  if (key == 10) { int prev = g_edge; g_edge = value; return prev; }
  if (key == 11) { int prev = g_up2_phases; g_up2_phases = value; return prev; }
  return RDEIC_EINVAL;
}
```

### rdeic_amd/csrc/prof.hip

```cpp
#include <atomic>
#include <mutex>
#include <vector>

#include "common.h"
#include "prof.h"
#include "../../include/rdeic_hip.h"

std::atomic<long long> g_launch_counts[RDEIC_COUNT_KINDS];

void rdeic_count_launch(int kind) {
  if (kind >= 0 && kind < RDEIC_COUNT_KINDS) g_launch_counts[kind].fetch_add(1, std::memory_order_relaxed);
}

extern "C" int64_t rdeic_launch_count(int32_t kind) {
  if (kind < 0 || kind >= RDEIC_COUNT_KINDS) return RDEIC_EINVAL;
  return g_launch_counts[kind].load(std::memory_order_relaxed);
}

extern "C" int rdeic_launch_count_reset(void) {
  for (auto& c : g_launch_counts) c.store(0, std::memory_order_relaxed);
  return RDEIC_OK;
}

namespace {
struct Slot { hipEvent_t a = nullptr, b = nullptr; int kind = -1; double work = 0.0; double weight = 1.0; long long key = 0; };
std::vector<Slot> g_slots;
int g_used = 0;
bool g_on = false;
int g_every = 1;
long g_seen[8] = {};
double g_bytes_n = 0.0, g_bytes = 0.0;
std::mutex g_mu;

double always_threshold(int kind) {
  return (kind <= RDEIC_PROF_ATTN_SMALL || kind == RDEIC_PROF_GEMM || kind == RDEIC_PROF_ATTN_D512) ? 50e9 : 64e6;
}
}

int rdeic_prof_begin(hipStream_t s, int kind, double work) {
  if (!g_on) return -1;
  std::lock_guard<std::mutex> lk(g_mu);
  if (!g_on || g_used >= (int)g_slots.size()) return -1;
  double weight = 1.0;
  if (kind >= 0 && kind < 8 && g_every > 1 && work < always_threshold(kind)) {
    unsigned long long z = (unsigned long long)(g_seen[kind]++) + 0x9E3779B97F4A7C15ull;
    z = (z ^ (z >> 30)) * 0xBF58476D1CE4E5B9ull;
    z = (z ^ (z >> 27)) * 0x94D049BB133111EBull;
    z ^= z >> 31;
    if (z % (unsigned long long)g_every != 0) return -1;
    weight = (double)g_every;
  }
  const int i = g_used++;
  g_slots[i].kind = -1;
  g_slots[i].weight = weight;
  if (hipEventRecord(g_slots[i].a, s) != hipSuccess) return -1;
  return i;
}

void rdeic_prof_add_bytes(double bytes) {
  if (!g_on) return;
  std::lock_guard<std::mutex> lk(g_mu);
  if (!g_on) return;
  g_bytes_n += 1.0;
  g_bytes += bytes;
}

void rdeic_prof_end(int slot, hipStream_t s, int kind, double work, long long key) {
  if (slot < 0) return;
  std::lock_guard<std::mutex> lk(g_mu);
  if (hipEventRecord(g_slots[slot].b, s) != hipSuccess) return;
  g_slots[slot].kind = kind;
  g_slots[slot].work = work;
  g_slots[slot].key = key;
}

extern "C" int rdeic_prof_start(int32_t capacity, int32_t every) {
  if (capacity <= 0 || every <= 0) return RDEIC_EINVAL;
  std::lock_guard<std::mutex> lk(g_mu);
  while ((int)g_slots.size() < capacity) {
    Slot sl;
    if (hipEventCreateWithFlags(&sl.a, hipEventDisableSystemFence) != hipSuccess ||
        hipEventCreateWithFlags(&sl.b, hipEventDisableSystemFence) != hipSuccess)
      return RDEIC_ELAUNCH;
    g_slots.push_back(sl);
  }
  g_used = 0;
  g_bytes_n = g_bytes = 0.0;
  g_every = every;
  for (long& c : g_seen) c = 0;
  g_on = true;
  return RDEIC_OK;
}

extern "C" int rdeic_prof_stop(void) {
  std::lock_guard<std::mutex> lk(g_mu);
  g_on = false;
  return g_used;
}

extern "C" int rdeic_prof_read(int32_t kind, int64_t* launches, double* work, double* ms) {
  if (!launches || !work || !ms) return RDEIC_EINVAL;
  std::lock_guard<std::mutex> lk(g_mu);
  if (kind == RDEIC_PROF_CONV_BYTES) {
    *launches = (int64_t)(g_bytes_n + 0.5); *work = g_bytes; *ms = 0.0;
    return RDEIC_OK;
  }
  double n = 0.0, w = 0.0, t_ms = 0.0;
  for (int i = 0; i < g_used; ++i) {
    const Slot& sl = g_slots[i];
    if (sl.kind != kind) continue;
    if (hipEventSynchronize(sl.b) != hipSuccess) return RDEIC_ELAUNCH;
    float t = 0.f;
    if (hipEventElapsedTime(&t, sl.a, sl.b) != hipSuccess) return RDEIC_ELAUNCH;
    n += sl.weight; w += sl.weight * sl.work; t_ms += sl.weight * t;
  }
  *launches = (int64_t)(n + 0.5); *work = w; *ms = t_ms;
  return RDEIC_OK;
}

extern "C" int rdeic_prof_read_keys(int32_t kind, int64_t* keys, int64_t* launches, double* work, double* ms,
                                    int32_t cap) {
  if (!keys || !launches || !work || !ms || cap <= 0) return RDEIC_EINVAL;
  std::lock_guard<std::mutex> lk(g_mu);
  std::vector<long long> ks;
  std::vector<double> n, w, t;
  for (int i = 0; i < g_used; ++i) {
    const Slot& sl = g_slots[i];
    if (sl.kind != kind) continue;
    if (hipEventSynchronize(sl.b) != hipSuccess) return RDEIC_ELAUNCH;
    float e = 0.f;
    if (hipEventElapsedTime(&e, sl.a, sl.b) != hipSuccess) return RDEIC_ELAUNCH;
    size_t j = 0;
    while (j < ks.size() && ks[j] != sl.key) ++j;
    if (j == ks.size()) { ks.push_back(sl.key); n.push_back(0.0); w.push_back(0.0); t.push_back(0.0); }
    n[j] += sl.weight; w[j] += sl.weight * sl.work; t[j] += sl.weight * e;
  }
  const int m = (int)ks.size() < cap ? (int)ks.size() : cap;
  for (int j = 0; j < m; ++j) {
    keys[j] = ks[j]; launches[j] = (int64_t)(n[j] + 0.5); work[j] = w[j]; ms[j] = t[j];
  }
  return m;
}
```

### rdeic_amd/finetune.py

```python
from __future__ import annotations

import math
from typing import Dict, List, Optional, Sequence

import torch

from . import autograd as AG
from . import ops
from .rdeic import RDEIC
from .unet import Conv, Down, ResBlock, SpatialTransformer, Up

TRAINABLE_PREFIXES = ("control_model.", "preprocess_model.")


class FineTuneConfig:

    def __init__(self, learning_rate=2e-5, l_guide_weight=3.0, l_bpp_weight=1.0, used_timesteps=300,
                 betas=(0.9, 0.999), eps=1e-8, weight_decay=1e-2, vq_beta=0.25, vq_decay=0.99, vq_temp=0.07):
        self.learning_rate = learning_rate
        self.l_guide_weight = l_guide_weight
        self.l_bpp_weight = l_bpp_weight
        self.used_timesteps = used_timesteps
        self.betas, self.eps, self.weight_decay = betas, eps, weight_decay
        self.vq_beta, self.vq_decay, self.vq_temp = vq_beta, vq_decay, vq_temp


FT_SPLITK = "short"


def _ft_splitk_ctx():
    import contextlib
    if FT_SPLITK == "off":
        return contextlib.nullcontext()
    return ops.splitk_allowed(short_k=FT_SPLITK == "short")


class FineTuner:

    def __init__(self, model: RDEIC, cfg: Optional[FineTuneConfig] = None,
                 embed_prob: Optional[torch.Tensor] = None):
        self.m = model
        self.cfg = cfg or FineTuneConfig(used_timesteps=model.used_timesteps)
        st = model.store
        self.dtype = st.compute_dtype
        dev = st.device
        names = [n for n in st.names() if n.startswith(TRAINABLE_PREFIXES)]
        self.names = names
        total = sum(math.prod(st.shapes[n]) for n in names)
        self.flat = torch.empty(total, dtype=torch.float32, device=dev)
        self.grad = torch.zeros(total, dtype=torch.float32, device=dev)
        self.exp_avg = torch.zeros(total, dtype=torch.float32, device=dev)
        self.exp_avg_sq = torch.zeros(total, dtype=torch.float32, device=dev)
        self.offsets: Dict[str, tuple] = {}
        off = 0
        for n in names:
            shape = st.shapes[n]
            k = math.prod(shape)
            self.flat[off:off + k].copy_(st.t[n].reshape(-1))
            p = self.flat[off:off + k].view(shape)
            p.requires_grad_(True)
            p.grad = self.grad[off:off + k].view(shape)
            p._rdeic_gview = p.grad
            st.t[n] = p
            self.offsets[n] = (off, k)
            off += k
        st._packed.clear()
        AG.PACKS.clear()
        AG.STEP_PACKS.clear()
        cb = model.preprocess_model.codebook_size
        self.embed_prob = torch.zeros(cb, dtype=torch.float32, device=dev)
        if embed_prob is not None:
            if tuple(embed_prob.shape) != (cb,):
                raise ValueError(f"embed_prob has shape {tuple(embed_prob.shape)}, the codebook has {cb} codes")
            self.embed_prob.copy_(embed_prob.to(torch.float32))
        self.step_count = 0
        self.buckets = None

    def load_optimizer_state(self, exp_avg: torch.Tensor, exp_avg_sq: torch.Tensor, step: int) -> None:
        for dst, src, name in ((self.exp_avg, exp_avg, "exp_avg"), (self.exp_avg_sq, exp_avg_sq, "exp_avg_sq")):
            if src.numel() != dst.numel():
                raise ValueError(f"optimizer.{name} holds {src.numel()} values, the trainable buffer {dst.numel()}")
            dst.copy_(src.reshape(-1).to(torch.float32))
        self.step_count = int(step)

    def enable_ddp(self, bucket_bytes: int = 32 << 20, group=None):
        from .parallel import GradBuckets
        params = [(self.m.store.t[n], o, k) for n, (o, k) in self.offsets.items()]
        self.buckets = GradBuckets(self.grad, params, bucket_bytes, group)
        return self.buckets

    def p(self, name: str) -> torch.Tensor:
        return self.m.store.t[name]

    def num_params(self) -> int:
        return self.flat.numel()

    def conv(self, x, prefix, *, stride=1, pad=None, up2=False, emb=None, res=None, act=AG.NONE, slope=0.0,
             pixel_shuffle=False, out_f32=False):
        w = self.p(prefix + ".weight")
        b = self.m.store.t.get(prefix + ".bias")
        kh = w.shape[2] if w.dim() == 4 else 1
        cfg = AG.ConvCfg(kh, kh, stride, kh // 2 if pad is None else pad, up2, pixel_shuffle, act, slope, out_f32,
                         key=None if w.requires_grad else prefix)
        return AG.conv2d(x, w, b, emb=emb, res=res, cfg=cfg)

    def linear(self, x, prefix, *, res=None, out_f32=False):
        w = self.p(prefix + ".weight")
        b = self.m.store.t.get(prefix + ".bias")
        return AG.linear(x, w, b, res=res, key=None if w.requires_grad else prefix, out_f32=out_f32)

    def gn(self, x, prefix, groups, eps, silu, passthrough=False):
        return AG.group_norm(x, self.p(prefix + ".weight"), self.p(prefix + ".bias"), groups, eps, silu, passthrough)

    def ln(self, x, prefix, passthrough=False):
        return AG.layer_norm(x, self.p(prefix + ".weight"), self.p(prefix + ".bias"), 1e-5, passthrough)

    def time_embed(self, net, temb):
        e = AG.act(self.linear(temb, net.prefix + "time_embed.0"), AG.SILU)
        e = self.linear(e, net.prefix + "time_embed.2")
        return AG.act(e, AG.SILU)

    def resblock(self, rb: ResBlock, x, semb):
        h, xs = self.gn(x, rb.prefix + ".in_layers.0", rb.gn_in, 1e-5, True, passthrough=True)
        emb = self.linear(semb, rb.prefix + ".emb_layers.1")
        h = self.conv(h, rb.prefix + ".in_layers.2", emb=emb)
        h = self.gn(h, rb.prefix + ".out_layers.0", rb.gn_out, 1e-5, True)
        skip = xs if rb.cin == rb.cout else self.conv(xs, rb.prefix + ".skip_connection")
        return self.conv(h, rb.prefix + ".out_layers.3", res=skip)

    def transformer(self, t: SpatialTransformer, x, ctx_rows, batch):
        B, H, W_, C = x.shape
        L = H * W_
        tb = t.prefix + ".transformer_blocks.0"
        h, xs = self.gn(x, t.prefix + ".norm", t.gn, 1e-6, False, passthrough=True)
        h = self.linear(h.reshape(B * L, C), t.prefix + ".proj_in")
        scale = t.dh ** -0.5
        n1, hs = self.ln(h, tb + ".norm1", passthrough=True)
        q = self.linear(n1, tb + ".attn1.to_q")
        k = self.linear(n1, tb + ".attn1.to_k")
        v = self.linear(n1, tb + ".attn1.to_v")
        o = AG.attention(q, k, v, batch, t.heads, scale)
        h = self.linear(o, tb + ".attn1.to_out.0", res=hs)
        n2, hs = self.ln(h, tb + ".norm2", passthrough=True)
        q = self.linear(n2, tb + ".attn2.to_q")
        k = self.linear(ctx_rows, tb + ".attn2.to_k")
        v = self.linear(ctx_rows, tb + ".attn2.to_v")
        o = AG.attention(q, k, v, batch, t.heads, scale)
        h = self.linear(o, tb + ".attn2.to_out.0", res=hs)
        n3, hs = self.ln(h, tb + ".norm3", passthrough=True)
        g = AG.geglu(self.linear(n3, tb + ".ff.net.0.proj"))
        h = self.linear(g, tb + ".ff.net.2", res=hs)
        out = self.linear(h, t.prefix + ".proj_out", res=xs.reshape(B * L, C))
        return out.view(B, H, W_, C)

    def run_layers(self, net, layers, x, semb, ctx_rows, batch):
        for layer in layers:
            if isinstance(layer, Conv):
                x = self.conv(x, layer.prefix)
            elif isinstance(layer, ResBlock):
                x = self.resblock(layer, x, semb)
            elif isinstance(layer, SpatialTransformer):
                x = self.transformer(layer, x, ctx_rows, batch)
            elif isinstance(layer, Down):
                x = self.conv(x, layer.prefix, stride=2, pad=1)
            elif isinstance(layer, Up):
                x = self.conv(x, layer.prefix, up2=True)
            else:
                raise TypeError(layer)
        return x

    def noise_estimator(self, x_noisy, hint, t, ctx):
        ne = self.m.control_model
        if ne.control_scale != 1.0:
            raise NotImplementedError("control_scale != 1 in the fine-tune step")
        B = x_noisy.shape[0]
        temb = ne.timestep_embedding(t.to(device=x_noisy.device, dtype=torch.int64).contiguous())
        semb_c = self.time_embed(ne.ctrl, temb)
        semb_b = self.time_embed(ne.base, temb)
        Bc, Lc, Dc = ctx.shape
        if Bc != B:
            ctx = ctx.expand(B, Lc, Dc)
        ctx_rows = ctx.reshape(B * Lc, Dc).to(self.dtype).contiguous()
        h_base = AG.cast(x_noisy, self.dtype)
        h_ctr = torch.cat([h_base, hint], dim=3)
        hs_base, hs_ctr = [], []
        for i, (lb, lc) in enumerate(zip(ne.base.input_blocks, ne.ctrl.input_blocks)):
            h_base = self.run_layers(ne.base, lb, h_base, semb_b, ctx_rows, B)
            h_ctr = self.run_layers(ne.ctrl, lc, h_ctr, semb_c, ctx_rows, B)
            h_base = self.conv(h_ctr, ne.enc_zero[i], res=h_base)
            hs_base.append(h_base)
            hs_ctr.append(h_ctr)
        h_base = self.run_layers(ne.base, ne.base.middle, h_base, semb_b, ctx_rows, B)
        h_ctr = self.run_layers(ne.ctrl, ne.ctrl.middle, h_ctr, semb_c, ctx_rows, B)
        h_base = self.conv(h_ctr, ne.mid_zero, res=h_base)
        for i, lb in enumerate(ne.base.output_blocks):
            h_base = self.conv(hs_ctr.pop(), ne.dec_zero[i], res=h_base)
            h_base = torch.cat([h_base, hs_base.pop()], dim=3)
            h_base = self.run_layers(ne.base, lb, h_base, semb_b, ctx_rows, B)
        p = ne.base.prefix
        h = self.gn(h_base, p + "out.0", 32, 1e-5, True)
        return self.conv(h, p + "out.2", out_f32=True)

    def _block(self, blk, x):
        pre, kind, ci, co = blk
        L = AG.LEAKY
        if kind == "conv":
            return self.conv(x, pre)
        if kind == "rb":
            identity = x if ci == co else self.conv(x, pre + ".adaptor")
            out = self.conv(x, pre + ".conv1", act=L, slope=0.01)
            return self.conv(out, pre + ".conv2", act=L, slope=0.01, res=identity)
        if kind == "rbs":
            out = self.conv(x, pre + ".conv1", stride=2, pad=1, act=L, slope=0.01)
            identity = self.conv(x, pre + ".downsample", stride=2, pad=0)
            return self.conv(out, pre + ".conv2", act=L, slope=0.1, res=identity)
        if kind == "rbu":
            out = self.conv(x, pre + ".subpel_conv.0", pixel_shuffle=True, act=L, slope=0.01)
            identity = self.conv(x, pre + ".upsample.0", pixel_shuffle=True)
            return self.conv(out, pre + ".conv", act=L, slope=0.1, res=identity)
        raise ValueError(kind)

    def _seq(self, blocks, x):
        for b in blocks:
            x = self._block(b, x)
        return x

    def _ep(self, name, i, x):
        p = self.m.preprocess_model.p
        h = self.conv(x, f"{p}{name}.{i}.fusion.0", act=AG.GELU)
        h = self.conv(h, f"{p}{name}.{i}.fusion.2", act=AG.GELU)
        return self.conv(h, f"{p}{name}.{i}.fusion.4")

    def _channel_ctx(self, i, x):
        p = self.m.preprocess_model.p
        h = self.conv(x, f"{p}channel_context.{i}.fushion.0", act=AG.GELU)
        h = self.conv(h, f"{p}channel_context.{i}.fushion.2", act=AG.GELU)
        return self.conv(h, f"{p}channel_context.{i}.fushion.4")

    def compression_forward(self, h, slice_noise: Sequence[torch.Tensor]):
        cm = self.m.preprocess_model
        p = cm.p
        y = self._seq(cm.g_a, h)
        z = self._seq(cm.hyper_enc, y)
        zq, emb_loss = AG.VQTrainFn.apply(z, self.p(p + "quantize.embedding.weight"), self.embed_prob,
                                          self.cfg.vq_beta, self.cfg.vq_decay, self.cfg.vq_temp)
        hyper = self._seq(cm.hyper_dec, zq)
        S_tot, qS_tot = None, None
        yhat_slices: List[torch.Tensor] = []
        for i, c in enumerate(cm.slice_ch):
            s0 = cm.slice_off[i]
            ys = y[..., s0:s0 + c]
            if i == 0:
                pa = self._ep("entropy_parameters_anchor", 0, hyper)
                channel_ctx = None
            else:
                channel_ctx = self._channel_ctx(i, torch.cat(yhat_slices, dim=3))
                pa = self._ep("entropy_parameters_anchor", i, torch.cat([channel_ctx, hyper], dim=3))
            anchor_hat = AG.CkbdAnchorFn.apply(ys, pa)
            local_ctx = self.conv(anchor_hat, f"{p}local_context.{i}")
            ctx_in = [local_ctx, hyper] if i == 0 else [local_ctx, channel_ctx, hyper]
            pn = self._ep("entropy_parameters_nonanchor", i, torch.cat(ctx_in, dim=3))
            S, qS, non = AG.CkbdLikFn.apply(ys, pa, pn, slice_noise[i])
            yhat_slices.append(anchor_hat + non)
            S_tot = S if S_tot is None else S_tot + S
            qS_tot = qS if qS_tot is None else qS_tot + qS
        y_hat = torch.cat(yhat_slices, dim=3)
        guide_hint = self._seq(cm.g_s, y_hat)
        c_latent = self.conv(guide_hint, p + "out", out_f32=True)
        return c_latent, S_tot, qS_tot, emb_loss, guide_hint

    @torch.no_grad()
    def get_first_stage(self, img_u8: torch.Tensor, post_eps_nhwc: torch.Tensor):
        m = self.m
        B, H, W_, _ = img_u8.shape
        cpad = 8 if self.dtype == torch.bfloat16 else 3
        x = torch.empty((B, H, W_, cpad), dtype=self.dtype, device=img_u8.device)
        ops.call("rdeic_image_u8_to_nhwc", img_u8.contiguous().data_ptr(), B, H, W_, x.data_ptr(), cpad,
                 ops.dt_code(x), ops.stream_ptr())
        h, mom = m.first_stage_model.encode_hc_moments(x, out_mul=m.scale_factor)
        mean, logvar = mom[..., :4], mom[..., 4:]
        std = torch.exp(0.5 * torch.clamp(logvar, -30.0, 20.0))
        x_start = m.scale_factor * (mean + std * post_eps_nhwc)
        return x_start.contiguous(), h

    def losses(self, x_start, h, ctx, t, noise, slice_noise):
        m, cfg = self.m, self.cfg
        c_latent, S, qS, emb_loss, guide_hint = self.compression_forward(h, slice_noise)
        B, hl, wl, _ = x_start.shape
        num_pixels = B * hl * wl * 64
        bpp = AG.bpp_from_sum(S, num_pixels)
        q_bpp = AG.bpp_from_sum(qS, num_pixels)
        lamba = m.sqrt_recipm1_alphas_cumprod[m.used_timesteps - 1]
        t = t.to(device=x_start.device, dtype=torch.int64)
        noise = noise + (c_latent - x_start) / lamba
        a = m.sqrt_alphas_cumprod[t].view(-1, 1, 1, 1)
        b = m.sqrt_one_minus_alphas_cumprod[t].view(-1, 1, 1, 1)
        x_noisy = a * x_start + b * noise
        eps = self.noise_estimator(x_noisy, guide_hint, t, ctx)
        model_output = (m.sqrt_recip_alphas_cumprod[t].view(-1, 1, 1, 1) * x_noisy -
                        m.sqrt_recipm1_alphas_cumprod[t].view(-1, 1, 1, 1) * eps)
        loss_simple = ((x_start - model_output) ** 2).mean(dim=(1, 2, 3))
        loss = cfg.l_guide_weight * loss_simple.mean()
        loss = loss + cfg.l_bpp_weight * bpp[0]
        loss = loss + cfg.l_bpp_weight * emb_loss[0]
        loss_guide = ((x_start - c_latent) ** 2).mean()
        loss = loss + cfg.l_guide_weight * loss_guide
        d = {"T/l_simple": loss_simple.mean(), "T/l_bpp": bpp[0], "T/q_bpp": q_bpp[0], "T/l_emb": emb_loss[0],
             "T/l_guide": loss_guide, "T/loss": loss}
        self._last = dict(c_latent=c_latent.detach(), eps=eps.detach(), x_noisy=x_noisy.detach(),
                          guide_hint=guide_hint.detach())
        return loss, d

    def zero_grad(self):
        self.grad.zero_()
        for n in self.offsets:
            p = self.m.store.t[n]
            p._rdeic_uses = 0
            p._rdeic_direct = False

    def adam_scalars(self, step: int) -> torch.Tensor:
        c = self.cfg
        b1, b2 = c.betas
        return torch.tensor([-c.learning_rate / (1 - b1 ** step), (1 - b2 ** step) ** 0.5], dtype=torch.float32)

    def adamw_launch(self, sc_dev: torch.Tensor):
        c = self.cfg
        AG.call("rdeic_adamw_dev", self.flat.data_ptr(), self.grad.data_ptr(), self.exp_avg.data_ptr(),
                self.exp_avg_sq.data_ptr(), self.flat.numel(), float(c.learning_rate), float(c.betas[0]),
                float(c.betas[1]), float(c.eps), float(c.weight_decay), sc_dev.data_ptr(), ops.stream_ptr())

    def optimizer_step(self):
        self.step_count += 1
        if getattr(self, "_sc", None) is None:
            self._sc = torch.zeros(2, dtype=torch.float32, device=self.flat.device)
        self._sc.copy_(self.adam_scalars(self.step_count), non_blocking=True)
        self.adamw_launch(self._sc)

    def training_step(self, img_u8, ctx, draws: dict, sync_grads=None):
        self.zero_grad()
        AG.STEP_PACKS.refresh()
        x_start, h = self.get_first_stage(img_u8, draws["post_eps"])
        if self.buckets is not None:
            self.buckets.begin()
        with _ft_splitk_ctx(), AG.STEP_PACKS.active():
            loss, d = self.losses(x_start, h, ctx, draws["t"], draws["noise"], draws["slice_noise"])
            loss.backward()
        if self.buckets is not None:
            self.buckets.finish()
        elif sync_grads is not None:
            sync_grads(self.grad)
        self.optimizer_step()
        if self.buckets is not None:
            self.sync_codebook()
        return {k: v.detach() for k, v in d.items()}

    def sync_codebook(self, src: int = 0):
        import torch.distributed as dist
        if not (dist.is_available() and dist.is_initialized()) or dist.get_world_size() == 1:
            return
        o, k = self.offsets[self.m.preprocess_model.p + "quantize.embedding.weight"]
        dist.broadcast(self.flat[o:o + k], src)
        dist.broadcast(self.embed_prob, src)


class CapturedStep:

    def __init__(self, ft: "FineTuner", img_u8: torch.Tensor, ctx: torch.Tensor, draws: dict):
        if ft.buckets is not None:
            raise ValueError("graph capture is single-GPU (the DDP all-reduce runs from backward hooks)")
# ... 55 lines not shown
```

### rdeic_amd/ops.py

```python
from __future__ import annotations

import ctypes as C
import json
import math
import os
import threading
from dataclasses import dataclass
from typing import Optional

import torch

from . import _lib
from ._lib import ConvDesc, call

NONE, LEAKY, GELU, SILU = 0, 1, 2, 3


def dt_code(t: torch.Tensor) -> int:
    if t.dtype == torch.bfloat16:
        return 1
    if t.dtype == torch.float32:
        return 0
    raise TypeError(f"unsupported activation dtype {t.dtype}")

# ... 89 lines not shown
    if p.weight.dtype != x.dtype:
        raise TypeError(f"weight dtype {p.weight.dtype} != activation dtype {x.dtype}")
    hi, wi = (2 * h, 2 * w) if up2 else (h, w)
    pt = p.pad if pad_t is None else pad_t
    pl = p.pad if pad_l is None else pad_l
    if out_hw is None:
        ho = (hi + 2 * p.pad - p.kh) // p.stride + 1
        wo = (wi + 2 * p.pad - p.kw) // p.stride + 1
    else:
        ho, wo = out_hw
    odt = torch.float32 if (out_f32 or x.dtype == torch.float32) else x.dtype
    if geglu:
        if x.dtype != torch.bfloat16 or c0 % 64 or c1 % 64 or p.cout % 8 or res is not None or emb is not None \
                or act != NONE or out_f32 or pixel_shuffle:
            raise ValueError("fused GEGLU: bf16, 64-channel-aligned input, no residual / emb / activation")
        oshape = (n, ho, wo, p.cout // 2)
    elif pixel_shuffle:
        oshape = (n, 2 * ho, 2 * wo, p.cout // 4)
    else:
        oshape = (n, ho, wo, p.cout)
    if out is None:
        out = torch.empty(oshape, dtype=odt, device=x.device)
    elif tuple(out.shape) != oshape or out.dtype != odt:
        raise ValueError(f"out has shape {tuple(out.shape)}/{out.dtype}, expected {oshape}/{odt}")
    d = ConvDesc()
    d.in0 = x.data_ptr()
    d.in1 = _ptr(x2)
    d.c0, d.c1, d.ld0, d.ld1 = c0, c1, ld0, ld1
    d.n, d.h, d.w, d.up2 = n, h, w, int(up2)
    d.weight, d.wld, d.bias = p.weight.data_ptr(), p.wld, _ptr(p.bias)
    d.cout, d.kh, d.kw, d.stride, d.pad_t, d.pad_l = p.cout, p.kh, p.kw, p.stride, pt, pl
    d.ho, d.wo = ho, wo
    if gn is not None:
        if gn.shape != (n, p.cin, 2):
            raise ValueError("gn affine must be [n, cin, 2]")
        _ab_ready(gn)
        d.gn_ab = gn.data_ptr()
        d.gn_silu = int(gn_silu)
    if emb is not None:
        if emb.dtype != torch.float32 or emb.shape[0] != n or emb.stride(1) != 1:
            raise ValueError("emb must be fp32 [n, >=cout] row-major")
        d.emb = emb.data_ptr()
        d.emb_ld = emb.stride(0)
    d.act, d.act_param = act, float(slope)
    if res is not None:
        if tuple(res.shape) != oshape or res.dtype != odt:
            raise ValueError(f"residual {tuple(res.shape)}/{res.dtype} does not match output {oshape}/{odt}")
        d.res = res.data_ptr()
        d.res_ld = pix_ld(res)
    d.out = out.data_ptr()
    d.out_ld = pix_ld(out)
    d.out_mode = 2 if geglu else (1 if pixel_shuffle else 0)
    d.dtype = dt_code(x)
    d.out_f32 = int(odt == torch.float32 and x.dtype != torch.float32)
    d.batch = 1
    if ln_rows is not None:
        if p.ln_cs is None or ln_rows.dtype != torch.float32 or tuple(ln_rows.shape) != (n * ho * wo, 2) \
                or not ln_rows.is_contiguous():
            raise ValueError("ln_rows needs a ParamStore.conv_ln weight and an fp32 [M, 2] contiguous (mean, rstd)")
        d.ln_rows, d.ln_colsum = ln_rows.data_ptr(), p.ln_cs.data_ptr()
    elif p.ln_cs is not None:
        raise ValueError("a LayerNorm-folded weight needs ln_rows")
    part = None
    if stats and GN_STATS_FUSE and x.dtype == torch.bfloat16 and not (geglu or pixel_shuffle):
        ghw = int(stats_hw or ho * wo)
        nf = int(_lib.load().rdeic_groupnorm_parts_floats(n * ho * wo, p.cout, ghw))
        if nf:
            part = torch.empty(nf, dtype=torch.float32, device=x.device)
            d.gn_part, d.gn_hw = part.data_ptr(), ghw
    flops = 2.0 * n * ho * wo * p.cout * p.kh * p.kw * p.cin
    splits = _splitk_count(x, x2, n * ho * wo, p, gn is not None or pixel_shuffle or geglu, out,
                           n if images is None else images)

    tile = -1
    if splits == 1 and x.dtype == torch.bfloat16 and gn is None and _gn_materialize(x, x2, p):
        key = tile_key(n * ho * wo, c0, c1, p, up2, d.out_mode, res is not None, emb is not None, act, odt)
        tile = TILE_TABLE.get(key, -1) if FORCE_TILE is None else FORCE_TILE
        if AUTOTUNE and FORCE_TILE is None and key not in TILE_TABLE:
            scratch = torch.empty_strided(out.size(), out.stride(), dtype=out.dtype, device=out.device)
            dma = c0 % 64 == 0 and c1 % 64 == 0
            tile = _autotune_tile(d, scratch, DMA_TILE_CANDIDATES if dma else TILE_CANDIDATES)
            if tile >= 0:
                TILE_TABLE[key] = tile

    if up2 and phases is not None and UP2_PHASES and splits == 1 and x.dtype == torch.bfloat16 and gn is None \
            and x2 is None and emb is None and res is None and ln_rows is None and d.out_mode == 0 and not d.out_f32 \
            and (p.kh, p.kw, p.stride, pt, pl) == (3, 3, 1, 1, 1) and (ho, wo) == (2 * h, 2 * w) \
            and phases.weight.dtype == torch.bfloat16 and phases.cout == p.cout and phases.wld == 4 * c0:
        dp = ConvDesc.from_buffer_copy(d)
        dp.weight, dp.wld = phases.weight.data_ptr(), phases.wld
        key = tile_key(n * h * w, c0, 0, phases, 2, 0, False, False, act, odt)
        ptile = TILE_TABLE.get(key, -1) if FORCE_TILE is None else FORCE_TILE
        ptag = ("conv", 2.0 * n * h * w * 4 * c0 * p.cout * 4,
                (n, h, w, c0, c1, p.cout, p.kh, p.stride, False, 2, d.out_mode))
        if _launch_soft(ptag, "rdeic_conv2d_up2_phases", C.byref(dp), phases.weight.stride(0), ptile, stream_ptr()):
            if part is not None:
                _attach_gn_part(out, part, d.gn_hw)
            return out
    tag = ("conv", flops, (n, h, w, c0, c1, p.cout, p.kh, p.stride, gn is not None, int(up2), d.out_mode))
    if splits > 1:
        ws = _splitk_workspace(splits * n * ho * wo * p.cout, x.device)
        _launch(tag, "rdeic_conv2d_splitk", C.byref(d), splits, ws.data_ptr(), ws.numel(), stream_ptr())
    elif tile >= 0:
        _launch(tag, "rdeic_conv2d_tile", C.byref(d), tile, stream_ptr())
    else:
        _launch(tag, "rdeic_conv2d", C.byref(d), stream_ptr())
    if part is not None:
        _attach_gn_part(out, part, d.gn_hw)
    return out


GN_STATS_FUSE = True


def _attach_gn_part(t: torch.Tensor, part: torch.Tensor, hw: int) -> None:
    t._rdeic_gn_part = (part, t.data_ptr(), tuple(t.shape), tuple(t.stride()), hw)


def _gn_part_of(t: Optional[torch.Tensor], hw: int):
    info = getattr(t, "_rdeic_gn_part", None) if t is not None else None
    if info is None:
        return None
    part, ptr, shape, stride, phw = info
    if ptr != t.data_ptr() or shape != tuple(t.shape) or stride != tuple(t.stride()) or phw != hw:
        return None
    return part


AUTOTUNE = False
UP2_PHASES = True
FORCE_TILE: Optional[int] = None
GEGLU_FUSED = True
TILE_CANDIDATES = (0, 1, 3, 4, 6, 8, 10)
DMA_TILE_CANDIDATES = (25, 32, 34, 26, 30, 33, 24, 31, 35, 36, 37, 38)
ALL_TILES = (0, 1, 2, 3, 4, 6, 7, 8, 9, 10) + tuple(range(21, 39))
TILE_TABLE_PATH = os.environ.get("RDEIC_TILE_TABLE") or os.path.join(os.path.dirname(os.path.abspath(__file__)),
                                                                     "conv_tiles.json")


def tile_key(m: int, c0: int, c1: int, p: "ConvParams", up2, out_mode: int, res: bool, emb: bool, act: int,
             odt) -> str:
    return (f"m{m}:c{c0}+{c1}:o{p.cout}:k{p.kh}x{p.kw}:s{p.stride}:up{int(up2)}:om{out_mode}:"
            f"r{int(res)}:e{int(emb)}:a{act}:{'f32' if odt == torch.float32 else 'bf16'}")


def _load_tile_table() -> dict:
    if not os.path.exists(TILE_TABLE_PATH):
        return {}
    with open(TILE_TABLE_PATH) as f:
        tab = json.load(f)["tiles"]
    bad = {k: v for k, v in tab.items() if v not in ALL_TILES}
    if bad:
        raise ValueError(f"{TILE_TABLE_PATH}: unknown tile ids {bad}")
    return tab


TILE_TABLE: dict = _load_tile_table()


def _autotune_tile(d0, scratch: torch.Tensor, candidates=None) -> int:
    if _lib.RECORDER is not None:
        return -1
    d = ConvDesc.from_buffer_copy(d0)
    d.out = scratch.data_ptr()
    s = stream_ptr()
    best, best_t = -1, float("inf")
    for t in (TILE_CANDIDATES if candidates is None else candidates):
        call("rdeic_conv2d_tile", C.byref(d), t, s)
        e0 = torch.cuda.Event(enable_timing=True)
        e1 = torch.cuda.Event(enable_timing=True)
        e0.record()
        for _ in range(2):
            call("rdeic_conv2d_tile", C.byref(d), t, s)
        e1.record()
        e1.synchronize()
        ms = e0.elapsed_time(e1)
        if ms < best_t:
            best, best_t = t, ms
    return best


_SPLITK_WS: dict = {}
_SPLITK_TLS = threading.local()


def splitk_state():
    return getattr(_SPLITK_TLS, "allowed", False), getattr(_SPLITK_TLS, "short", False)


SPLITK_NOMINAL_BATCH = 16
SPLITK_BLOCKS, SPLITK_MAX = 512, 8
SPLITK_TRAIN = None
SPLITK_ENTROPY = True


class splitk_allowed:

    def __init__(self, short_k: bool = False):
        self.short_k = short_k

    def __enter__(self):
        self._prev = splitk_state()
        _SPLITK_TLS.allowed, _SPLITK_TLS.short = True, self.short_k or self._prev[1]
        return self

    def __exit__(self, *exc):
        _SPLITK_TLS.allowed, _SPLITK_TLS.short = self._prev


class splitk_as:

    def __init__(self, state):
        self.state = tuple(state)

    def __enter__(self):
        self._prev = splitk_state()
        _SPLITK_TLS.allowed, _SPLITK_TLS.short = self.state
        return self

    def __exit__(self, *exc):
        _SPLITK_TLS.allowed, _SPLITK_TLS.short = self._prev


def _splitk_count(x, x2, M: int, p: "ConvParams", fused: bool, out: torch.Tensor, n: int) -> int:
    allowed, short = splitk_state()
    if not short:
        M = (M // max(1, n)) * SPLITK_NOMINAL_BATCH
    if not allowed or fused or x.dtype not in (torch.bfloat16, torch.float32) or p.cout % 8 \
            or pix_ld(out) % 8 or out.data_ptr() % 16:
        return 1
    for t in (x, x2):
        if t is not None and (t.shape[3] % 8 or pix_ld(t) % 8 or t.data_ptr() % 16):
            return 1
    if x.dtype == torch.float32:
        tiles = -(-M // 64) * -(-p.cout // 64)
        nk = -(-(p.kh * p.kw * p.cin) // 32)
        if short and tiles < 256 and 8 <= nk < 32:
            return max(1, min(-(-512 // tiles), nk // 4, 16))
        if tiles >= 256 or nk < 32:
            return 1
        return max(1, min(-(-512 // tiles), nk // 8, 16))
    tiles = -(-M // 128) * -(-p.cout // 128)
    nk = -(-(p.kh * p.kw * p.cin) // 64)
    if short and tiles < 128 and 8 <= nk < 32:
        return max(1, min(-(-512 // tiles), nk // 4, 8))
    if short and SPLITK_TRAIN is not None and tiles < 192 and nk >= 32:
        kdiv, smax, target = SPLITK_TRAIN
        return max(1, min(-(-target // tiles), nk // kdiv, smax))
    if tiles >= 192 or nk < 32:
        return 1
    return max(1, min(SPLITK_BLOCKS // tiles, nk // 16, SPLITK_MAX))


_SPLITK_KEEP: list = []


def _splitk_workspace(n: int, device) -> torch.Tensor:
    key = (str(device), stream_ptr())
    buf = _SPLITK_WS.get(key)
    if buf is None or buf.numel() < n:
        buf = torch.empty(n, dtype=torch.float32, device=device)
        _SPLITK_WS[key] = buf
        _SPLITK_KEEP.append(buf)
    return buf


PROFILE = None
PROFILE_OTHER: dict = {}


def _launch(tag, name: str, *args):
    if PROFILE is None:
        return call(name, *args, tag=tag)
    ev0 = torch.cuda.Event(enable_timing=True)
    ev1 = torch.cuda.Event(enable_timing=True)
    ev0.record()
    call(name, *args, tag=tag)
    ev1.record()
    record_profile(tag, ev0, ev1)


def _launch_soft(tag, name: str, *args) -> bool:
    if PROFILE is None:
        return _lib.call_soft(name, *args, tag=tag)
    ev0 = torch.cuda.Event(enable_timing=True)
    ev1 = torch.cuda.Event(enable_timing=True)
    ev0.record()
    if not _lib.call_soft(name, *args, tag=tag):
        return False
    ev1.record()
    record_profile(tag, ev0, ev1)
    return True


def record_profile(tag, ev0, ev1):
    kind, work, meta = tag
    if kind == "conv":
        PROFILE.append((work, ev0, ev1, None, meta))
    else:
        PROFILE_OTHER.setdefault(kind, []).append((work, ev0, ev1))


PROF_KINDS = {"conv": 0, "attention": 1, "attention_dh16": 2, "gn_stats": 3, "gn_apply": 4, "gemm": 5,
              "attention_d512": 6, "conv_bytes": 7}


def prof_start(capacity: int = 65536, every: int = 1) -> None:
    call("rdeic_prof_start", capacity, every)


def prof_stop() -> int:
    return int(_lib.load().rdeic_prof_stop())


def prof_read() -> dict:
    out = {}
    for kind, code in PROF_KINDS.items():
        n, w, ms = C.c_int64(), C.c_double(), C.c_double()
        call("rdeic_prof_read", code, C.byref(n), C.byref(w), C.byref(ms))
        if n.value:
            out[kind] = (n.value, w.value, ms.value)
    return out


def prof_read_keys(kind: str, cap: int = 64) -> list:
    keys, n = (C.c_int64 * cap)(), (C.c_int64 * cap)()
    w, ms = (C.c_double * cap)(), (C.c_double * cap)()
    m = int(_lib.load().rdeic_prof_read_keys(PROF_KINDS[kind], keys, n, w, ms, cap))
    return [(int(keys[i]), int(n[i]), float(w[i]), float(ms[i])) for i in range(max(0, m))]


def attention_key(key: int) -> dict:
    return {"dh": (key >> 48) & 0xffff, "lq": (key >> 32) & 0xffff, "lk": (key >> 16) & 0xffff, "bh": key & 0xffff}


def other_profile_summary():
    out = {}
    for kind, recs in PROFILE_OTHER.items():
        out[kind] = (len(recs), sum(r[0] for r in recs), sum(r[1].elapsed_time(r[2]) for r in recs))
    return out


def conv_profile_summary(records):
    total_ms = 0.0
    total_flops = 0.0
    for rec in records:
        flops, e0, e1 = rec[0], rec[1], rec[2]
        total_ms += e0.elapsed_time(e1)
        total_flops += flops
    return len(records), total_flops, total_ms


def conv_profile_breakdown(records):
    out = {}
    for rec in records:
        flops, e0, e1, meta = rec[0], rec[1], rec[2], rec[4]
        key = str(meta)
        v = out.setdefault(key, [0, 0.0, 0.0])
        v[0] += 1
        v[1] += flops / 1e9
        v[2] += e0.elapsed_time(e1)
    return out


CONV_PATH = 2


def set_conv_path(path: int) -> int:
    global CONV_PATH
    prev = CONV_PATH
    CONV_PATH = int(path)
    _lib.load().rdeic_set_conv_path(CONV_PATH)
    return prev


def set_conv_option(key: int, value: int) -> int:
    return int(_lib.load().rdeic_set_conv_option(int(key), int(value)))


HALO_CONV = 1
HALO_MAX_C = 512


COUNT_HALO_CONV, COUNT_GN_APPLY, COUNT_LAYERNORM, COUNT_HALO_SMALL, COUNT_LN_FUSED, COUNT_SPLITK, COUNT_EDGE, \
    COUNT_GN_PARTS_APPLY = 0, 1, 2, 3, 4, 5, 6, 7


def set_up2_phases(on: bool) -> bool:
    global UP2_PHASES
    prev = UP2_PHASES
    UP2_PHASES = bool(on)
    _lib.load().rdeic_set_conv_option(11, int(UP2_PHASES))
    return prev


def launch_count(kind: int) -> int:
    return int(_lib.load().rdeic_launch_count(int(kind)))


def launch_count_reset() -> None:
    call("rdeic_launch_count_reset")


def set_halo_conv(mode: int) -> int:
    global HALO_CONV
    prev = HALO_CONV
    HALO_CONV = int(mode)
    _lib.load().rdeic_set_conv_option(6, HALO_CONV)
    return prev


def _halo_eligible(x, x2, p: "ConvParams", up2, pad_t, pad_l, out_hw, special, out) -> bool:
    if not HALO_CONV or x.dtype != torch.bfloat16 or x2 is not None or up2 or special:
        return False
    if p.kh != 3 or p.kw != 3 or p.stride != 1 or p.pad != 1 or (pad_t not in (None, 1)) or (pad_l not in (None, 1)):
        return False
    n, h, w, c = x.shape
    if out_hw is not None and tuple(out_hw) != (h, w):
        return False
    if c % 32 or c > min(512, HALO_MAX_C) or p.cout > HALO_MAX_C or p.cout % 128 or h % 4 or w % 64 \
            or x.stride(2) % 8 or x.data_ptr() % 16:
        return False
    if out is not None and (pix_ld(out) % 8 or out.data_ptr() % 16):
        return False
    return True


EDGE_CONV = 1


def set_edge_conv(mode: int) -> int:
    global EDGE_CONV
    prev = EDGE_CONV
    EDGE_CONV = int(mode)
    _lib.load().rdeic_set_conv_option(10, EDGE_CONV)
    return prev


def _edge_narrow_eligible(x, x2, p: "ConvParams", up2, pad_t, pad_l, out_hw, special) -> bool:
    if not EDGE_CONV or x.dtype != torch.bfloat16 or x2 is not None or up2 or special:
        return False
    if p.kh != 3 or p.kw != 3 or p.stride != 1 or p.pad != 1 or (pad_t not in (None, 1)) or (pad_l not in (None, 1)):
        return False
    n, h, w, c = x.shape
    if out_hw is not None and tuple(out_hw) != (h, w):
        return False
    lds = 10 * 66 * 64 + c * 8 + p.cout * 9 * c * 2
    return p.cout <= 16 and c % 32 == 0 and lds <= 160 * 1024 and h % 8 == 0 and w % 64 == 0 \
        and x.stride(2) % 8 == 0 and x.data_ptr() % 16 == 0


def _gn_materialize(x: torch.Tensor, x2: Optional[torch.Tensor], p: ConvParams) -> bool:
    if CONV_PATH == 0 or x.dtype != torch.bfloat16:
        return False
    if p.cout <= 32 and not (p.cout <= 4 and x.shape[0] * x.shape[1] * x.shape[2] >= (1 << 20)):
        return False
    for t in (x, x2):
        if t is None:
            continue
        if t.shape[3] % 8 or t.stride(2) % 8 or t.data_ptr() % 16:
            return False
    return True


def linear(x: torch.Tensor, p: ConvParams, *, act: int = NONE, res: Optional[torch.Tensor] = None,
           out: Optional[torch.Tensor] = None, out_f32: bool = False, geglu: bool = False,
           stats_hw: Optional[int] = None, images: int, ln_rows: Optional[torch.Tensor] = None) -> torch.Tensor:
    rows, c = x.shape
    x4 = x.as_strided((1, rows, 1, c), (rows * x.stride(0), x.stride(0), x.stride(0), 1))
    odt = torch.float32 if (out_f32 or x.dtype == torch.float32) else x.dtype
    cw = p.cout // 2 if geglu else p.cout
    if out is None:
        out = torch.empty((rows, cw), dtype=odt, device=x.device)
    o4 = out.as_strided((1, rows, 1, cw), (rows * out.stride(0), out.stride(0), out.stride(0), 1))
    r4 = None
    if res is not None:
        r4 = res.as_strided((1, rows, 1, p.cout), (rows * res.stride(0), res.stride(0), res.stride(0), 1))
    conv2d(x4, p, act=act, res=r4, out=o4, out_f32=out_f32, geglu=geglu, stats=stats_hw is not None,
           stats_hw=stats_hw, images=images, ln_rows=ln_rows)
    info = getattr(o4, "_rdeic_gn_part", None)
    if info is not None:
        out._rdeic_gn_tokens = info
    return out


def tokens_to_nhwc(t: torch.Tensor, n: int, h: int, w: int) -> torch.Tensor:
    v = t.view(n, h, w, t.shape[1])
    info = getattr(t, "_rdeic_gn_tokens", None)
    if info is not None and info[4] == h * w:
        _attach_gn_part(v, info[0], h * w)
    return v


def gemm_batched(a: torch.Tensor, b_nk: torch.Tensor, out: torch.Tensor, *, batch: int, m: int, n: int, k: int,
                 lda: int, ldb: int, a_bs: int, b_bs: int, out_bs: int) -> torch.Tensor:
    d = ConvDesc()
    d.in0 = a.data_ptr()
    d.c0, d.ld0 = k, lda
    d.n, d.h, d.w = 1, m, 1
    d.weight, d.wld = b_nk.data_ptr(), ldb
    d.cout, d.kh, d.kw, d.stride = n, 1, 1, 1
    d.ho, d.wo = m, 1
    d.out = out.data_ptr()
    d.out_ld = n
    d.dtype = dt_code(a)
    d.out_f32 = int(out.dtype == torch.float32 and a.dtype != torch.float32)
    d.batch = batch
    d.in_bs, d.w_bs, d.out_bs = a_bs, b_bs, out_bs
    _launch(("conv", 2.0 * batch * m * n * k, ("bgemm", batch, m, n, k)), "rdeic_conv2d", C.byref(d), stream_ptr())
    return out


GN_PARTS_APPLY = True
GN_PARTS_APPLY_HW = (64, 128, 256)


def _ab_ready(ab: Optional[torch.Tensor]) -> None:
    pend = getattr(ab, "_rdeic_pending", None) if ab is not None else None
    if pend is None:
        return
    p0, c0, p1, c1, n, hw, groups, eps, gamma, beta = pend
    call("rdeic_groupnorm_parts_ab", p0.data_ptr(), c0, _ptr(p1), c1, n, hw, groups, float(eps),
         gamma.data_ptr(), beta.data_ptr(), ab.data_ptr(), stream_ptr())
    del ab._rdeic_pending


def group_norm_ab(x: torch.Tensor, gamma: torch.Tensor, beta: torch.Tensor, groups: int, eps: float,
                  x2: Optional[torch.Tensor] = None, defer: bool = False) -> torch.Tensor:
    n, h, w, c0 = x.shape
    ld0 = pix_ld(x)
    c1, ld1 = (x2.shape[3], pix_ld(x2)) if x2 is not None else (0, 0)
    c = c0 + c1
    p0, p1 = _gn_part_of(x, h * w), _gn_part_of(x2, h * w)
    if p0 is not None and (x2 is None or p1 is not None):
        ab = torch.empty((n, c, 2), dtype=torch.float32, device=x.device)
        if defer and GN_PARTS_APPLY and h * w in GN_PARTS_APPLY_HW and x.dtype == torch.bfloat16 and groups <= 256:
            ab._rdeic_pending = (p0, c0, p1, c1, n, h * w, groups, float(eps), gamma, beta)
            return ab
        call("rdeic_groupnorm_parts_ab", p0.data_ptr(), c0, _ptr(p1), c1, n, h * w, groups, float(eps),
             gamma.data_ptr(), beta.data_ptr(), ab.data_ptr(), stream_ptr())
        return ab
    ws = torch.empty(int(_lib.load().rdeic_groupnorm_ws_floats(n, h * w, c)), dtype=torch.float32, device=x.device)
    ab = torch.empty((n, c, 2), dtype=torch.float32, device=x.device)
    _launch(("gn_stats", float(n * h * w * c * x.element_size()), None),
            "rdeic_groupnorm_stats", x.data_ptr(), c0, ld0, _ptr(x2), c1, ld1, n, h * w, groups,
            float(eps), gamma.data_ptr(), beta.data_ptr(), ab.data_ptr(), ws.data_ptr(), dt_code(x), stream_ptr())
    return ab


def group_norm_apply(x: torch.Tensor, ab: torch.Tensor, silu: bool, out: Optional[torch.Tensor] = None,
                     out_mul: float = 1.0) -> torch.Tensor:
    _ab_ready(ab)
    n, h, w, c = x.shape
    if out is None:
        out = torch.empty((n, h, w, c), dtype=x.dtype, device=x.device)
    if ab.shape[1] < c or ab.stride(2) != 1 or ab.stride(1) != 2:
        raise ValueError("group-norm affine must be [n, >=c, 2] with packed (a, b) pairs")
    _launch(("gn_apply", float(2 * n * h * w * c * x.element_size()), None),
            "rdeic_groupnorm_apply", x.data_ptr(), n, h * w, c, pix_ld(x), ab.data_ptr(),
            ab.stride(0) // 2, int(silu), float(out_mul), out.data_ptr(), pix_ld(out), dt_code(x), stream_ptr())
    return out


LN_FOLD = True


def layer_norm_rowstats(x: torch.Tensor, eps: float = 1e-5, out: Optional[torch.Tensor] = None) -> torch.Tensor:
    rows, c = x.shape
    if out is None:
        out = torch.empty((rows, 2), dtype=torch.float32, device=x.device)
    call("rdeic_layernorm_rowstats", x.data_ptr(), rows, c, x.stride(0), float(eps), out.data_ptr(), stream_ptr())
    return out


def layer_norm(x: torch.Tensor, gamma: torch.Tensor, beta: torch.Tensor, eps: float = 1e-5,
               out: Optional[torch.Tensor] = None) -> torch.Tensor:
    rows, c = x.shape
    if out is None:
        out = torch.empty((rows, c), dtype=x.dtype, device=x.device)
    call("rdeic_layernorm", x.data_ptr(), rows, c, x.stride(0), gamma.data_ptr(), beta.data_ptr(), float(eps),
         out.data_ptr(), out.stride(0), dt_code(x), stream_ptr())
    return out


def attention(q: torch.Tensor, k: torch.Tensor, v: torch.Tensor, out: torch.Tensor, *, batch: int, heads: int,
              lq: int, lk: int, dh: int, scale: float, kv_bcast: bool = False) -> torch.Tensor:
    _launch(("attention_d512" if dh == 512 else "attention" if dh >= 64 else "attention_dh%d" % dh,
             4.0 * batch * heads * lq * lk * dh, None),
            "rdeic_attention", q.data_ptr(), q.stride(0), k.data_ptr(), k.stride(0), v.data_ptr(),
            v.stride(0), out.data_ptr(), out.stride(0), batch, heads, lq, lk, dh, float(scale),
            int(kv_bcast), dt_code(q), stream_ptr())
    return out


VAE_FLASH_ATTENTION = True

SCORE_BUDGET_BYTES = 1 << 28


def attention_single_head_materialized(q: torch.Tensor, k: torch.Tensor, v: torch.Tensor, out: torch.Tensor, *,
                                       batch: int, length: int, dim: int, scale: float) -> torch.Tensor:
    if dim % 64 != 0 or length % 64 != 0:
        raise ValueError("materialised attention needs dim, length multiples of 64")
    dt = dt_code(q)
    L = length
    per_img = L * L * 4
    if per_img <= SCORE_BUDGET_BYTES:
        g, qrows = max(1, min(batch, SCORE_BUDGET_BYTES // per_img)), L
    else:
        g, qrows = 1, max(64, (SCORE_BUDGET_BYTES // (L * 4)) // 64 * 64)
    vt = torch.empty((batch, dim, L), dtype=q.dtype, device=q.device)
    call("rdeic_transpose", v.data_ptr(), L, dim, v.stride(0), vt.data_ptr(), L, batch,
         L * v.stride(0), dim * L, dt, stream_ptr())
    s = torch.empty((g, qrows, L), dtype=torch.float32, device=q.device)
    p = torch.empty((g, qrows, L), dtype=q.dtype, device=q.device)
    for b0 in range(0, batch, g):
        nb = min(g, batch - b0)
        for q0 in range(0, L, qrows):
            nq = min(qrows, L - q0)
            qa = q[b0 * L + q0:]
            gemm_batched(qa, k[b0 * L:], s, batch=nb, m=nq, n=L, k=dim, lda=q.stride(0), ldb=k.stride(0),
                         a_bs=L * q.stride(0), b_bs=L * k.stride(0), out_bs=nq * L)
            call("rdeic_softmax_rows", s.data_ptr(), nb * nq, L, float(scale), p.data_ptr(), dt, stream_ptr())
            gemm_batched(p, vt[b0:], out[b0 * L + q0:], batch=nb, m=nq, n=dim, k=L, lda=L, ldb=L,
                         a_bs=nq * L, b_bs=dim * L, out_bs=L * out.stride(0))
    return out


def geglu(x: torch.Tensor, out: Optional[torch.Tensor] = None) -> torch.Tensor:
    rows, c2 = x.shape
    c = c2 // 2
    if out is None:
        out = torch.empty((rows, c), dtype=x.dtype, device=x.device)
    call("rdeic_geglu", x.data_ptr(), rows, c, x.stride(0), out.data_ptr(), out.stride(0), dt_code(x), stream_ptr())
    return out


def cfg_combine(e_cond: torch.Tensor, e_uncond: torch.Tensor, scale: float) -> torch.Tensor:
    if e_cond.dtype != torch.float32 or e_uncond.dtype != torch.float32 or e_cond.shape != e_uncond.shape:
        raise ValueError("cfg_combine needs two fp32 tensors of one shape")
    ec, eu = e_cond.contiguous(), e_uncond.contiguous()
    out = torch.empty_like(ec)
    call("rdeic_cfg_combine", ec.data_ptr(), eu.data_ptr(), ec.numel(), float(scale), out.data_ptr(), stream_ptr())
    return out


def nchw_to_nhwc(x: torch.Tensor, dtype, mul: float = 1.0, add: float = 0.0, out=None) -> torch.Tensor:
    x = x.to(torch.float32).contiguous()
    n, c, h, w = x.shape
    if out is None:
        out = torch.empty((n, h, w, c), dtype=dtype, device=x.device)
    call("rdeic_nchw_to_nhwc", x.data_ptr(), n, c, h, w, float(mul), float(add), out.data_ptr(), pix_ld(out),
         dt_code(out), stream_ptr())
    return out


def nhwc_to_nchw(x: torch.Tensor, mul: float = 1.0, add: float = 0.0) -> torch.Tensor:
    n, h, w, c = x.shape
    out = torch.empty((n, c, h, w), dtype=torch.float32, device=x.device)
    call("rdeic_nhwc_to_nchw", x.data_ptr(), n, c, h, w, pix_ld(x), float(mul), float(add), out.data_ptr(),
         dt_code(x), stream_ptr())
    return out


def cast(x: torch.Tensor, dtype) -> torch.Tensor:
    x = x.contiguous()
    out = torch.empty(x.shape, dtype=dtype, device=x.device)
    call("rdeic_cast", x.data_ptr(), dt_code(x), out.data_ptr(), dt_code(out), x.numel(), stream_ptr())
    return out


def fill_uniform(out: torch.Tensor, seed: int, scale: float, offset: float) -> torch.Tensor:
    if out.dtype != torch.float32 or not out.is_contiguous():
        raise ValueError("fill_uniform expects a contiguous fp32 tensor")
    call("rdeic_fill_uniform", out.data_ptr(), out.numel(), C.c_uint64(seed & 0xFFFFFFFFFFFFFFFF),
         float(scale) * 2.0 ** -23, float(offset), stream_ptr())
    return out


def silu_f32(x: torch.Tensor) -> torch.Tensor:
    out = torch.empty_like(x)
    call("rdeic_silu_f32", x.data_ptr(), out.data_ptr(), x.numel(), stream_ptr())
    return out
```

### rdeic_amd/params.py

```python
from __future__ import annotations

from typing import Dict, Iterable, Optional, Sequence, Tuple

import torch

from . import ops
from . import weights as W


def fold_up2_phases(w: torch.Tensor, dtype=torch.float32) -> torch.Tensor:
    cout, cin, kh, kw = w.shape
    if (kh, kw) != (3, 3):
        raise ValueError("the phase fold is for 3x3 convs")
    r = torch.tensor([[[1, 0, 0], [0, 1, 1]], [[1, 1, 0], [0, 0, 1]]], dtype=torch.float64, device=w.device)
    f = torch.einsum("ayk,oikl,bxl->aboyxi", r, w.double(), r)
    return f.reshape(4, cout, 4 * cin).to(dtype).contiguous()


class ParamStore:
    def __init__(self, compute_dtype=torch.bfloat16, device="cuda"):
        self.compute_dtype = compute_dtype
        self.device = torch.device(device)
        self.shapes: Dict[str, Tuple[int, ...]] = {}
        self.t: Dict[str, torch.Tensor] = {}
        self._packed: Dict[tuple, ops.ConvParams] = {}

    def declare(self, name: str, shape: Sequence[int]):
        shape = tuple(int(s) for s in shape)
        if name in self.shapes and self.shapes[name] != shape:
            raise ValueError(f"{name} declared twice with different shapes")
        self.shapes[name] = shape

    def declare_conv(self, prefix: str, cout: int, cin: int, k: int, bias: bool = True):
        self.declare(prefix + ".weight", (cout, cin, k, k))
        if bias:
            self.declare(prefix + ".bias", (cout,))

    def declare_linear(self, prefix: str, cout: int, cin: int, bias: bool = True):
        self.declare(prefix + ".weight", (cout, cin))
        if bias:
            self.declare(prefix + ".bias", (cout,))

    def declare_norm(self, prefix: str, c: int):
        self.declare(prefix + ".weight", (c,))
        self.declare(prefix + ".bias", (c,))

    def init_synthetic(self, global_seed: int = W.GLOBAL_SEED, rate_gain: float = 1.0):
        for name, shape in self.shapes.items():
            scale, offset = W.init_spec(name, shape, rate_gain)
            t = torch.empty(shape, dtype=torch.float32, device=self.device)
            ops.fill_uniform(t, W.param_seed(name, global_seed), scale, offset)
            self.t[name] = t
        self._packed.clear()

    def load_state_dict(self, sd: Dict[str, torch.Tensor], strict: bool = True):
        missing = [n for n in self.shapes if n not in sd]
        if strict and missing:
            raise KeyError(f"missing parameters: {missing[:8]}{' ...' if len(missing) > 8 else ''}")
        for name, shape in self.shapes.items():
            if name not in sd:
                continue
            v = sd[name]
            if tuple(v.shape) != shape:
                raise ValueError(f"{name}: checkpoint shape {tuple(v.shape)} != {shape}")
            self.t[name] = v.detach().to(device=self.device, dtype=torch.float32).contiguous()
        self._packed.clear()

    def names(self) -> Iterable[str]:
        return self.shapes.keys()

    def get(self, name: str) -> torch.Tensor:
        return self.t[name]

    def has(self, name: str) -> bool:
        return name in self.shapes

    def conv(self, prefix: str, stride: int = 1, pad: Optional[int] = None, dtype=None,
             scale: float = 1.0, cin_pad: Optional[int] = None, cout_pad: Optional[int] = None) -> ops.ConvParams:
        dtype = dtype or self.compute_dtype
        key = (prefix, stride, pad, dtype, scale, cin_pad, cout_pad)
        p = self._packed.get(key)
        if p is None:
            w = self.t[prefix + ".weight"]
            b = self.t.get(prefix + ".bias")
            if scale != 1.0:
                w, b = w * scale, (None if b is None else b * scale)
            if cin_pad is not None and cin_pad > w.shape[1]:
                w = torch.nn.functional.pad(w, (0, 0) * (w.dim() - 2) + (0, cin_pad - w.shape[1]))
            if cout_pad is not None and cout_pad > w.shape[0]:
                w = torch.nn.functional.pad(w, (0, 0) * (w.dim() - 1) + (0, cout_pad - w.shape[0]))
                if b is not None:
                    b = torch.nn.functional.pad(b, (0, cout_pad - b.shape[0]))
            k = w.shape[-1] if w.dim() == 4 else 1
            p = ops.ConvParams.pack(w, b, stride=stride, pad=(k // 2 if pad is None else pad), dtype=dtype)
            self._packed[key] = p
        return p

    def conv_up2_phases(self, prefix: str) -> Optional[ops.ConvParams]:
        w = self.t[prefix + ".weight"]
        if self.compute_dtype != torch.bfloat16 or w.dim() != 4 or tuple(w.shape[2:]) != (3, 3) or w.shape[1] % 64:
            return None
        key = (prefix, "up2_phases")
        p = self._packed.get(key)
        if p is None:
            b = self.t.get(prefix + ".bias")
            f = fold_up2_phases(w).to(torch.bfloat16).contiguous()
            p = ops.ConvParams(f, 4 * w.shape[1], self.conv(prefix).bias if b is not None else None, w.shape[0],
                               w.shape[1], 2, 2, 1, 1)
            self._packed[key] = p
        return p

    def conv_split_pad(self, prefix: str, c0: int, c0_pad: int, dtype=None) -> ops.ConvParams:
        dtype = dtype or self.compute_dtype
        key = (prefix, "split_pad", c0, c0_pad, dtype)
        p = self._packed.get(key)
        if p is None:
            w = self.t[prefix + ".weight"]
            cout, cin, kh, kw = w.shape
            wp = torch.zeros((cout, cin - c0 + c0_pad, kh, kw), dtype=w.dtype, device=w.device)
            wp[:, :c0] = w[:, :c0]
            wp[:, c0_pad:] = w[:, c0:]
            p = ops.ConvParams.pack(wp, self.t.get(prefix + ".bias"), stride=1, pad=kh // 2, dtype=dtype)
            self._packed[key] = p
        return p

    def conv_geglu(self, prefix: str, dtype=None) -> ops.ConvParams:
        dtype = dtype or self.compute_dtype
        key = (prefix, "geglu", dtype)
        p = self._packed.get(key)
        if p is None:
            w = self.t[prefix + ".weight"]
            b = self.t.get(prefix + ".bias")
            c = w.shape[0] // 2
            if c % 4:
                raise ValueError("GEGLU width must be a multiple of 4")
            perm = torch.arange(2 * c, device=w.device).view(2, c // 4, 4).permute(1, 0, 2).reshape(-1)
            p = ops.ConvParams.pack(w[perm], None if b is None else b[perm], dtype=dtype)
            self._packed[key] = p
        return p

    def conv_ln(self, prefixes: Sequence[str], ln_prefix: str, geglu: bool = False, dtype=None) -> ops.ConvParams:
        dtype = dtype or self.compute_dtype
        key = (tuple(prefixes), "ln", ln_prefix, geglu, dtype)
        p = self._packed.get(key)
        if p is None:
            gamma, beta = self.t[ln_prefix + ".weight"], self.t[ln_prefix + ".bias"]
            ws, bs = [], []
            for pre in prefixes:
                w = self.t[pre + ".weight"]
                b = self.t.get(pre + ".bias")
                ws.append(w)
                bs.append(b if b is not None else torch.zeros(w.shape[0], device=self.device))
            w = torch.cat(ws, 0)
            b = torch.cat(bs, 0).double() + w.double() @ beta.double()
            w = w * gamma[None, :]
            if geglu:
                c = w.shape[0] // 2
                perm = torch.arange(2 * c, device=w.device).view(2, c // 4, 4).permute(1, 0, 2).reshape(-1)
                w, b = w[perm], b[perm]
            p = ops.ConvParams.pack(w, b.float(), dtype=dtype)
            p.ln_cs = p.weight.double().sum(1).float().contiguous()
            self._packed[key] = p
        return p

    def conv_cat(self, prefixes: Sequence[str], dtype=None) -> ops.ConvParams:
        dtype = dtype or self.compute_dtype
        key = (tuple(prefixes), "cat", dtype)
        p = self._packed.get(key)
        if p is None:
            ws, bs = [], []
            for pre in prefixes:
                w = self.t[pre + ".weight"]
                ws.append(w if w.dim() == 4 else w[:, :, None, None])
                b = self.t.get(pre + ".bias")
                bs.append(b if b is not None else torch.zeros(w.shape[0], device=self.device))
            any_bias = any(self.t.get(pre + ".bias") is not None for pre in prefixes)
            w = torch.cat(ws, 0)
            p = ops.ConvParams.pack(w, torch.cat(bs, 0) if any_bias else None, stride=1, pad=w.shape[-1] // 2,
                                    dtype=dtype)
            self._packed[key] = p
        return p
```

### rdeic_amd/rdeic.py

```python
from __future__ import annotations

import os
from pathlib import Path
from typing import Dict, List, Optional, Sequence

import numpy as np
import torch

from . import bitstream, ops
from .compression import Compression
from .config import default_config
from .params import ParamStore
from .unet import NoiseEstimator
from .vae import AutoencoderKL


def make_schedule(timesteps: int, linear_start: float, linear_end: float) -> Dict[str, torch.Tensor]:
    betas = (torch.linspace(linear_start ** 0.5, linear_end ** 0.5, timesteps, dtype=torch.float64) ** 2).numpy()
    alphas = 1.0 - betas
    ac = np.cumprod(alphas, axis=0)
    ac_prev = np.append(1.0, ac[:-1])
    f = lambda a: torch.tensor(a, dtype=torch.float32)
    return dict(betas=f(betas), alphas_cumprod=f(ac), alphas_cumprod_prev=f(ac_prev),
                sqrt_alphas_cumprod=f(np.sqrt(ac)), sqrt_one_minus_alphas_cumprod=f(np.sqrt(1.0 - ac)),
                log_one_minus_alphas_cumprod=f(np.log(1.0 - ac)), sqrt_recip_alphas_cumprod=f(np.sqrt(1.0 / ac)),
                sqrt_recipm1_alphas_cumprod=f(np.sqrt(1.0 / ac - 1)),
                posterior_variance=f(betas * (1.0 - ac_prev) / (1.0 - ac)),
                posterior_log_variance_clipped=f(np.log(np.maximum(betas * (1.0 - ac_prev) / (1.0 - ac), 1e-20))),
                posterior_mean_coef1=f(betas * np.sqrt(ac_prev) / (1.0 - ac)),
                posterior_mean_coef2=f((1.0 - ac_prev) * np.sqrt(alphas) / (1.0 - ac)))


class RDEIC:
    parameterization = "eps"

    def __init__(self, config: Optional[dict] = None, compute_dtype=torch.bfloat16, device="cuda"):
        cfg = config or default_config()
        self.cfg = cfg
        self.store = ParamStore(compute_dtype, device)
        self.control_model = NoiseEstimator(self.store, cfg["unet"], cfg["control"])
        self.first_stage_model = AutoencoderKL(self.store, cfg["ddconfig"], cfg["embed_dim"])
        self.preprocess_model = Compression(self.store, **cfg["compression"])
        self.scale_factor = float(cfg["scale_factor"])
        self.num_timesteps = int(cfg["timesteps"])
        self.used_timesteps = int(cfg["used_timesteps"])
        self.linear_start, self.linear_end = float(cfg["linear_start"]), float(cfg["linear_end"])
        self.channels = 4
        sched = make_schedule(self.num_timesteps, cfg["linear_start"], cfg["linear_end"])
        self._sched_cpu = sched
        self.device = torch.device(device)
        for k, v in sched.items():
            setattr(self, k, v.to(self.device))
        from .plan import PlanCache
        self.use_plans = True
        self._plans = PlanCache()
        self._consts = {}

    @property
    def compute_dtype(self):
        return self.store.compute_dtype

    def init_synthetic(self, seed: Optional[int] = None, rate_gain: float = 1.0):
        from . import weights as W
        self.store.init_synthetic(W.GLOBAL_SEED if seed is None else seed, rate_gain)
        self._clear_plans()
        return self

    def load_state_dict(self, sd: Dict[str, torch.Tensor], strict: bool = True):
        self.store.load_state_dict({k: v for k, v in sd.items() if k in self.store.shapes}, strict=strict)
        self._clear_plans()
        return self

    @property
    def use_plans(self) -> bool:
        return self._use_plans

    @use_plans.setter
    def use_plans(self, v: bool):
        self._use_plans = bool(v)
        self.preprocess_model.use_plans = bool(v)

    def session(self) -> "RDEIC":
        import copy
        from .plan import PlanCache
        s = copy.copy(self)
        s._plans = PlanCache()
        s._consts = {}
        pm = copy.copy(self.preprocess_model)
        pm._plans = PlanCache()
        pm._io = {}
        pm.__dict__.pop("_pin_cache", None)
        s.preprocess_model = pm
        return s

    def _clear_plans(self):
        self._plans.clear()
        self.preprocess_model._plans.clear()
        self.preprocess_model._en = None

    def param_shapes(self):
        return dict(self.store.shapes)

    def encode_images_nhwc(self, img_u8: torch.Tensor) -> torch.Tensor:
        B, H, W_, _ = img_u8.shape
        cpad = 8 if self.compute_dtype == torch.bfloat16 else 3
        x = torch.empty((B, H, W_, cpad), dtype=self.compute_dtype, device=img_u8.device)
        ops.call("rdeic_image_u8_to_nhwc", img_u8.contiguous().data_ptr(), B, H, W_, x.data_ptr(), cpad,
                 ops.dt_code(x), ops.stream_ptr())
        return self.first_stage_model.encode_hc(x, out_mul=self.scale_factor)

    def encode_nchw_nhwc(self, x: torch.Tensor) -> torch.Tensor:
        xh = ops.nchw_to_nhwc(x.to(self.device), self.compute_dtype, mul=2.0, add=-1.0)
        return self.first_stage_model.encode_hc(xh, out_mul=self.scale_factor)

    def q_sample_nhwc(self, x0: torch.Tensor, t: torch.Tensor, noise: torch.Tensor) -> torch.Tensor:
        B = x0.shape[0]
        t = t.to(self.device).long()
        a = self.sqrt_alphas_cumprod[t].contiguous()
        b = self.sqrt_one_minus_alphas_cumprod[t].contiguous()
        out = torch.empty_like(x0)
        ops.call("rdeic_axpby", x0.contiguous().data_ptr(), noise.contiguous().data_ptr(), B, x0[0].numel(),
                 a.data_ptr(), b.data_ptr(), out.data_ptr(), ops.stream_ptr())
        return out

    def eps_nhwc(self, x: torch.Tensor, t: torch.Tensor, guide_hint: torch.Tensor, context: torch.Tensor):
        return self.control_model.forward(x, guide_hint, t, context.to(self.device))

    def eps_uncond_nhwc(self, x: torch.Tensor, t: torch.Tensor, context: torch.Tensor):
        return self.control_model.forward_unconditional(x, t, context.to(self.device))

    def decode_nhwc(self, z: torch.Tensor, out_f32: bool = True, consts=None) -> torch.Tensor:
        B = z.shape[0]
        zs = torch.empty_like(z)
        consts = consts or self._region_consts(B, 0, z.device)
        inv, zero = consts["inv_scale"], consts["zero"]
        ops.call("rdeic_axpby", z.contiguous().data_ptr(), z.contiguous().data_ptr(), B, z[0].numel(), inv.data_ptr(),
                 zero.data_ptr(), zs.data_ptr(), ops.stream_ptr())
        zc = ops.cast(zs, self.compute_dtype)
        return self.first_stage_model.decode(zc, out_f32=out_f32)

    def to_image_u8(self, x: torch.Tensor) -> torch.Tensor:
        B, H, W_, C = x.shape
        img = torch.empty((B, H, W_, 3), dtype=torch.uint8, device=x.device)
        ops.call("rdeic_nhwc_to_image_u8", x.data_ptr(), B, H, W_, ops.pix_ld(x), img.data_ptr(), ops.dt_code(x),
                 ops.stream_ptr())
        return img

    @torch.no_grad()
    def apply_condition_compress(self, x: torch.Tensor, stream_path: str, H: int, W: int) -> float:
        if x.shape[0] != 1:
            raise ValueError("apply_condition_compress codes one image per file (the reference's decompress "
                             "supports batch 1 only); use compress_images for batches")
        h = self.encode_nchw_nhwc(x)
        out = self.preprocess_model.compress(h)[0]
        with Path(stream_path).open("wb") as f:
            bitstream.write_body(f, out["shape"], out["strings"])
        size = bitstream.filesize(stream_path)
        return float(size) * 8 / (H * W)

    @torch.no_grad()
    def apply_condition_decompress(self, stream_path: str):
        with Path(stream_path).open("rb") as f:
            strings, shape = bitstream.read_body(f)
        c_lat, hint = self.preprocess_model.decompress([strings], shape, device=self.device)
        return ops.nhwc_to_nchw(c_lat), ops.nhwc_to_nchw(hint)

    def q_sample(self, x_start: torch.Tensor, t: torch.Tensor, noise: Optional[torch.Tensor] = None):
        if noise is None:
            noise = torch.randn_like(x_start)
        B, C, H, W_ = x_start.shape
        out = self.q_sample_nhwc(x_start.float().contiguous(), t, noise.float().contiguous().to(x_start.device))
        return out

    @torch.no_grad()
    def apply_model(self, x_noisy: torch.Tensor, t: torch.Tensor, cond: dict) -> torch.Tensor:
        ctx = torch.cat(cond["c_crossattn"], 1)
        x = ops.nchw_to_nhwc(x_noisy.float().to(self.device), torch.float32)
        hint = cond["guide_hint"]
        hint_nhwc = ops.nchw_to_nhwc(hint.float().to(self.device), self.compute_dtype)
        eps = self.eps_nhwc(x, t.to(self.device), hint_nhwc, ctx)
        return ops.nhwc_to_nchw(eps)

    @torch.no_grad()
    def apply_model_unconditional(self, x_noisy: torch.Tensor, t: torch.Tensor, cond: dict) -> torch.Tensor:
        ctx = torch.cat(cond["c_crossattn"], 1)
        x = ops.nchw_to_nhwc(x_noisy.float().to(self.device), torch.float32)
        return ops.nhwc_to_nchw(self.eps_uncond_nhwc(x, t.to(self.device), ctx))

    @torch.no_grad()
    def decode_first_stage(self, z: torch.Tensor) -> torch.Tensor:
        zn = ops.nchw_to_nhwc(z.float().to(self.device), torch.float32)
        return ops.nhwc_to_nchw(self.decode_nhwc(zn, out_f32=True))

    @torch.no_grad()
    def compress_images(self, img_u8: torch.Tensor) -> List[bytes]:
        img = img_u8.to(self.device).contiguous()
        outs = self.preprocess_model.compress_with(self.encode_images_nhwc, img)
        return [bitstream.pack_body(o["shape"], o["strings"]) for o in outs]

    @torch.no_grad()
    def decompress_bodies(self, bodies: Sequence[bytes]):
        parsed = [bitstream.unpack_body(b) for b in bodies]
        shape = parsed[0][1]
        if any(p[1] != shape for p in parsed):
            raise ValueError("batched decompress needs one latent shape per batch")
        return self.preprocess_model.decompress([p[0] for p in parsed], shape, device=self.device)

    @staticmethod
    def _sampler(model, sampler: str):
        if sampler == "ddim":
            from .ddim_sampler_relay import DDIMSampler
            return DDIMSampler(model)
        if sampler == "ddpm":
            from .spaced_sampler_relay import SpacedSampler
            return SpacedSampler(model, var_type="fixed_small")
        raise ValueError(f"sampler {sampler!r} (ddpm | ddim)")

    def _step_timesteps(self, steps: int, sampler: str):
        if sampler == "ddpm":
            from .spaced_sampler_relay import space_timesteps
            return sorted(space_timesteps(self.used_timesteps, str(steps)))
        from .ddim_sampler_relay import make_ddim_timesteps
        return [int(t) for t in make_ddim_timesteps(steps, self.used_timesteps)]

    @torch.no_grad()
    def relay_sample_nhwc(self, c_latent: torch.Tensor, guide_hint: torch.Tensor, context: torch.Tensor,
                          noise: torch.Tensor, steps: int, sampler: str = "ddim", step_noise=None) -> torch.Tensor:
        B = c_latent.shape[0]
        t = torch.full((B,), self.used_timesteps - 1, dtype=torch.long, device=self.device)
        x = self.q_sample_nhwc(c_latent, t, noise)
        if sampler == "ddpm":
            return self._sampler(self, sampler).sample_nhwc(steps, x, guide_hint, context, step_noise=step_noise)
        return self._sampler(self, sampler).sample_nhwc(steps, x, guide_hint, context)

    def _region_consts(self, B: int, steps: int, device, sampler: str = "ddim") -> dict:
        key = (B, steps, str(device), sampler)
        c = self._consts.get(key)
        if c is None:
            t = torch.full((B,), self.used_timesteps - 1, dtype=torch.long, device=device)
            c = {"qa": self.sqrt_alphas_cumprod[t].contiguous(), "qb": self.sqrt_one_minus_alphas_cumprod[t].contiguous(),
                 "inv_scale": torch.full((B,), 1.0 / self.scale_factor, dtype=torch.float32, device=device),
                 "zero": torch.zeros((B,), dtype=torch.float32, device=device), "ts": {}}
            if steps:
                for st in self._step_timesteps(steps, sampler):
                    c["ts"][int(st)] = torch.full((B,), int(st), dtype=torch.long, device=device)
            self._consts[key] = c
        return c

    def _relay_decode_u8(self, c_latent, guide_hint, context, noise, steps: int, sampler: str = "ddim",
                         step_noise=None):
        B = c_latent.shape[0]
        c = self._region_consts(B, steps, c_latent.device, sampler)
        x = torch.empty_like(c_latent)
        ops.call("rdeic_axpby", c_latent.data_ptr(), noise.data_ptr(), B, c_latent[0].numel(), c["qa"].data_ptr(),
                 c["qb"].data_ptr(), x.data_ptr(), ops.stream_ptr())
        smp = self._sampler(self, sampler)
        if sampler == "ddpm":
            z = smp.sample_nhwc(steps, x, guide_hint, context, step_noise=list(step_noise.unbind(0)),
                                ts_tensors=c["ts"])
        else:
            z = smp.sample_nhwc(steps, x, guide_hint, context, ts_tensors=c["ts"])
        return self.to_image_u8(self.decode_nhwc(z, out_f32=True, consts=c))

    @torch.no_grad()
    def relay_decode_u8(self, c_latent: torch.Tensor, guide_hint: torch.Tensor, context: torch.Tensor,
                        noise: torch.Tensor, steps: int, sampler: str = "ddim", step_noise=None) -> torch.Tensor:
        ctx = context.to(device=self.device, dtype=self.compute_dtype).contiguous()
        ins = [c_latent.contiguous(), guide_hint.contiguous(), ctx, noise.contiguous()]
        if sampler == "ddpm":
            if step_noise is None or tuple(step_noise.shape) != (steps,) + tuple(noise.shape):
                raise ValueError("sampler 'ddpm' needs step_noise of shape [steps, *noise.shape]")
            ins.append(step_noise.to(device=self.device, dtype=torch.float32).contiguous())
        elif sampler != "ddim":
            raise ValueError(f"sampler {sampler!r} (ddpm | ddim)")
        fn = (lambda a, b, c, d, *e: self._relay_decode_u8(a, b, c, d, steps, sampler, e[0] if e else None))
        if not self.use_plans:
            return fn(*ins)
        key = ("relay_decode", steps, sampler) + tuple((tuple(t.shape), t.dtype) for t in ins)
        return self._plans.run(key, fn, ins).clone()

    @torch.no_grad()
    def codec_images(self, img_u8: torch.Tensor, context: torch.Tensor, noise_nchw: torch.Tensor, steps: int = 2,
                     sampler: str = "ddim", step_noise_nchw: Optional[torch.Tensor] = None):
        bodies = self.compress_images(img_u8)
        c_lat, hint = self.decompress_bodies(bodies)
        noise = ops.nchw_to_nhwc(noise_nchw.float().to(self.device), torch.float32)
        step_noise = None
        if step_noise_nchw is not None:
            step_noise = torch.stack([ops.nchw_to_nhwc(n.float().to(self.device), torch.float32)
                                      for n in step_noise_nchw])
        return self.relay_decode_u8(c_lat, hint, context, noise, steps, sampler, step_noise), bodies
```

### rdeic_amd/unet.py

```python
from __future__ import annotations

from dataclasses import dataclass, field
from typing import List, Optional

import torch

from . import ops
from .params import ParamStore


def find_denominator(number: int, start: int) -> int:
    if start >= number:
        return number
    while start != 0:
        if number % start == 0:
            return start
        start -= 1
    return 1


@dataclass
class ResBlock:
    prefix: str
    cin: int
    cout: int
    gn_in: int
    gn_out: int
    emb_off: int = 0


@dataclass
class SpatialTransformer:
    prefix: str
    ch: int
    heads: int
    dh: int
    gn: int


@dataclass
class Conv:
    prefix: str
    cin: int
    cout: int


@dataclass
class Down:
    prefix: str
    ch: int


@dataclass
class Up:
    prefix: str
    ch: int


class UNet:

    def __init__(self, store: ParamStore, prefix: str, cfg: dict, control: bool = False):
        self.store, self.prefix, self.control = store, prefix, control
        mc0 = cfg["model_channels"]
        self.mc0 = mc0
        ted = mc0 * 4
        self.ted = ted
        ctx_dim = cfg["context_dim"]
        self.ctx_dim = ctx_dim
        store.declare_linear(prefix + "time_embed.0", ted, mc0)
        store.declare_linear(prefix + "time_embed.2", ted, ted)
        mc = int(mc0 * cfg["control_model_ratio"]) if control else mc0
        in_ch = cfg["in_channels"] + (cfg["hint_channels"] if control else 0)
        nhc = cfg["num_head_channels"]
        attn_res = cfg["attention_resolutions"]
        nrb = cfg["num_res_blocks"]
        mults = cfg["channel_mult"]
        self.resblocks: List[ResBlock] = []
        gn = (lambda c: find_denominator(c, 32)) if control else (lambda c: 32)

        def res(pre, cin, cout):
            rb = ResBlock(pre, cin, cout, gn(cin), gn(cout))
            store.declare_norm(pre + ".in_layers.0", cin)
            store.declare_conv(pre + ".in_layers.2", cout, cin, 3)
            store.declare_linear(pre + ".emb_layers.1", cout, ted)
            store.declare_norm(pre + ".out_layers.0", cout)
            store.declare_conv(pre + ".out_layers.3", cout, cout, 3)
            if cin != cout:
                store.declare_conv(pre + ".skip_connection", cout, cin, 1)
            self.resblocks.append(rb)
            return rb

        def st(pre, ch):
            nonlocal nhc_cur
            if control:
                nhc_cur = find_denominator(ch, nhc)
            heads, dh = ch // nhc_cur, nhc_cur
            inner = heads * dh
            store.declare_norm(pre + ".norm", ch)
            store.declare_linear(pre + ".proj_in", inner, ch)
            tb = pre + ".transformer_blocks.0"
            for a in ("attn1", "attn2"):
                kv_in = ch if a == "attn1" else ctx_dim
                store.declare_linear(f"{tb}.{a}.to_q", inner, ch, bias=False)
                store.declare_linear(f"{tb}.{a}.to_k", inner, kv_in, bias=False)
                store.declare_linear(f"{tb}.{a}.to_v", inner, kv_in, bias=False)
                store.declare_linear(f"{tb}.{a}.to_out.0", ch, inner)
            store.declare_linear(tb + ".ff.net.0.proj", inner * 8, inner)
            store.declare_linear(tb + ".ff.net.2", inner, inner * 4)
            for nn_ in ("norm1", "norm2", "norm3"):
                store.declare_norm(f"{tb}.{nn_}", inner)
            store.declare_linear(pre + ".proj_out", inner, ch)
            return SpatialTransformer(pre, ch, heads, dh, find_denominator(ch, 32))

        nhc_cur = nhc
        self.input_blocks: List[list] = []
        p0 = prefix + "input_blocks.0.0"
        store.declare_conv(p0, mc, in_ch, 3)
        self.input_blocks.append([Conv(p0, in_ch, mc)])
        chans, ch, ds, idx = [mc], mc, 1, 1
        for level, mult in enumerate(mults):
            for _ in range(nrb):
                layers = [res(f"{prefix}input_blocks.{idx}.0", ch, mult * mc)]
                ch = mult * mc
                if ds in attn_res:
                    layers.append(st(f"{prefix}input_blocks.{idx}.1", ch))
                self.input_blocks.append(layers)
                chans.append(ch)
                idx += 1
            if level != len(mults) - 1:
                pre = f"{prefix}input_blocks.{idx}.0.op"
                store.declare_conv(pre, ch, ch, 3)
                self.input_blocks.append([Down(pre, ch)])
                chans.append(ch)
                ds *= 2
                idx += 1
        self.enc_out_ch = list(chans)
        self.middle = [res(prefix + "middle_block.0", ch, ch), st(prefix + "middle_block.1", ch),
                       res(prefix + "middle_block.2", ch, ch)]
        self.mid_ch = ch
        self.output_blocks: List[list] = []
        self.dec_out_ch: List[int] = []
        if not control:
            k = 0
            for level, mult in list(enumerate(mults))[::-1]:
                for i in range(nrb + 1):
                    ich = chans.pop()
                    layers = [res(f"{prefix}output_blocks.{k}.0", ch + ich, mc * mult)]
                    ch = mc * mult
                    if ds in attn_res:
                        layers.append(st(f"{prefix}output_blocks.{k}.1", ch))
                    if level and i == nrb:
                        pre = f"{prefix}output_blocks.{k}.{len(layers)}.conv"
                        store.declare_conv(pre, ch, ch, 3)
                        layers.append(Up(pre, ch))
                        ds //= 2
                    self.output_blocks.append(layers)
                    self.dec_out_ch.append(ch)
                    k += 1
            store.declare_norm(prefix + "out.0", ch)
            store.declare_conv(prefix + "out.2", cfg["out_channels"], mc, 3)
        off = 0
        for rb in self.resblocks:
            rb.emb_off = off
            off += rb.cout
        self.emb_total = off

    def time_embed(self, temb: torch.Tensor) -> torch.Tensor:
        s = self.store
        B = temb.shape[0]
        e = ops.linear(temb, s.conv(self.prefix + "time_embed.0", dtype=torch.float32), act=ops.SILU, images=B)
        e = ops.linear(e, s.conv(self.prefix + "time_embed.2", dtype=torch.float32), act=ops.SILU, images=B)
        stacked = s.conv_cat([rb.prefix + ".emb_layers.1" for rb in self.resblocks], dtype=torch.float32)
        return ops.linear(e, stacked, images=B)

    def resblock(self, rb: ResBlock, x: torch.Tensor, emb_all: torch.Tensor,
                 x2: Optional[torch.Tensor] = None, stats: bool = False) -> torch.Tensor:
        s = self.store
        ab1 = ops.group_norm_ab(x, s.get(rb.prefix + ".in_layers.0.weight"), s.get(rb.prefix + ".in_layers.0.bias"),
                                rb.gn_in, 1e-5, x2=x2, defer=True)
        h = ops.conv2d(x, s.conv(rb.prefix + ".in_layers.2"), x2=x2, gn=ab1, gn_silu=True,
                       emb=emb_all[:, rb.emb_off:rb.emb_off + rb.cout], stats=True)
        ab2 = ops.group_norm_ab(h, s.get(rb.prefix + ".out_layers.0.weight"),
                                s.get(rb.prefix + ".out_layers.0.bias"), rb.gn_out, 1e-5, defer=True)
        if rb.cin != rb.cout:
            skip = ops.conv2d(x, s.conv(rb.prefix + ".skip_connection"), x2=x2)
        else:
            if x2 is not None:
                raise ValueError("identity skip with a concatenated input")
            skip = x
        return ops.conv2d(h, s.conv(rb.prefix + ".out_layers.3"), gn=ab2, gn_silu=True, res=skip, stats=stats)

    def transformer(self, t: SpatialTransformer, x: torch.Tensor, ctx_kv_in: torch.Tensor, ctx_batch: int,
                    ctx_len: int, stats: bool = False) -> torch.Tensor:
        s = self.store
        B, H, W_, C = x.shape
        L = H * W_
        rows = B * L
        tb = t.prefix + ".transformer_blocks.0"
        ab = ops.group_norm_ab(x, s.get(t.prefix + ".norm.weight"), s.get(t.prefix + ".norm.bias"), t.gn, 1e-6,
                               defer=True)
        h4 = ops.conv2d(x, s.conv(t.prefix + ".proj_in"), gn=ab, gn_silu=False)
        h = h4.view(rows, C)
        scale = t.dh ** -0.5
        fold = x.dtype == torch.bfloat16 and ops.LN_FOLD and C % 64 == 0
        qkv_names = [tb + ".attn1.to_q", tb + ".attn1.to_k", tb + ".attn1.to_v"]
        if fold:
            qkv = ops.linear(h, s.conv_ln(qkv_names, tb + ".norm1"), ln_rows=ops.layer_norm_rowstats(h), images=B)
        else:
            n1 = ops.layer_norm(h, s.get(tb + ".norm1.weight"), s.get(tb + ".norm1.bias"))
            qkv = ops.linear(n1, s.conv_cat(qkv_names), images=B)
        o = torch.empty((rows, C), dtype=x.dtype, device=x.device)
        ops.attention(qkv[:, :C], qkv[:, C:2 * C], qkv[:, 2 * C:], o, batch=B, heads=t.heads, lq=L, lk=L, dh=t.dh,
                      scale=scale)
        h = ops.linear(o, s.conv(tb + ".attn1.to_out.0"), res=h, images=B)
        if fold:
            q = ops.linear(h, s.conv_ln([tb + ".attn2.to_q"], tb + ".norm2"), ln_rows=ops.layer_norm_rowstats(h),
                           images=B)
        else:
            n2 = ops.layer_norm(h, s.get(tb + ".norm2.weight"), s.get(tb + ".norm2.bias"))
            q = ops.linear(n2, s.conv(tb + ".attn2.to_q"), images=B)
        kv = ops.linear(ctx_kv_in, s.conv_cat([tb + ".attn2.to_k", tb + ".attn2.to_v"]), images=ctx_batch)
        ops.attention(q, kv[:, :C], kv[:, C:], o, batch=B, heads=t.heads, lq=L, lk=ctx_len, dh=t.dh, scale=scale,
                      kv_bcast=(ctx_batch == 1 and B > 1))
        h = ops.linear(o, s.conv(tb + ".attn2.to_out.0"), res=h, images=B)
        if fold and ops.GEGLU_FUSED:
            gg = ops.linear(h, s.conv_ln([tb + ".ff.net.0.proj"], tb + ".norm3", geglu=True),
                            ln_rows=ops.layer_norm_rowstats(h), geglu=True, images=B)
        else:
            n3 = ops.layer_norm(h, s.get(tb + ".norm3.weight"), s.get(tb + ".norm3.bias"))
            if x.dtype == torch.bfloat16 and ops.GEGLU_FUSED and C % 64 == 0:
                gg = ops.linear(n3, s.conv_geglu(tb + ".ff.net.0.proj"), geglu=True, images=B)
            else:
                gg = ops.geglu(ops.linear(n3, s.conv(tb + ".ff.net.0.proj"), images=B))
        h = ops.linear(gg, s.conv(tb + ".ff.net.2"), res=h, images=B)
        if not x.is_contiguous():
            raise ValueError("transformer input must be contiguous NHWC")
        out = ops.linear(h, s.conv(t.prefix + ".proj_out"), res=x.view(rows, C), stats_hw=L if stats else None,
                         images=B)
        return ops.tokens_to_nhwc(out, B, H, W_)

    def run_layers(self, layers, x, emb_all, ctx_rows, ctx_batch, ctx_len, x2=None, stats_last: bool = True):
        s = self.store
        for li, layer in enumerate(layers):
            st = stats_last or li + 1 < len(layers)
            if isinstance(layer, Conv):
                x = ops.conv2d(x, s.conv(layer.prefix), x2=x2, stats=st)
                x2 = None
            elif isinstance(layer, ResBlock):
                x = self.resblock(layer, x, emb_all, x2=x2, stats=st)
                x2 = None
            elif isinstance(layer, SpatialTransformer):
                x = self.transformer(layer, x, ctx_rows, ctx_batch, ctx_len, stats=st)
            elif isinstance(layer, Down):
                x = ops.conv2d(x, s.conv(layer.prefix, stride=2, pad=1), stats=st)
            elif isinstance(layer, Up):
                x = ops.conv2d(x, s.conv(layer.prefix), up2=True, stats=st, phases=s.conv_up2_phases(layer.prefix))
            else:
                raise TypeError(layer)
        return x


class NoiseEstimator:

    def __init__(self, store: ParamStore, unet_cfg: dict, control_cfg: dict,
                 base_prefix: str = "model.diffusion_model.", ctrl_prefix: str = "control_model."):
        self.store = store
        self.base = UNet(store, base_prefix, unet_cfg, control=False)
        self.ctrl = UNet(store, ctrl_prefix + "control_model.", control_cfg, control=True)
        self.model_channels = unet_cfg["model_channels"]
        self.control_scale = float(control_cfg.get("control_scale", 1.0))
        cp = ctrl_prefix
        enc_c, enc_b = self.ctrl.enc_out_ch, self.base.enc_out_ch
        self.enc_zero = [f"{cp}enc_zero_convs_out.{i}.0" for i in range(len(enc_c))]
        for i, pre in enumerate(self.enc_zero):
            store.declare_conv(pre, enc_b[i], enc_c[i], 1)
        self.mid_zero = f"{cp}middle_block_out.0"
        store.declare_conv(self.mid_zero, self.base.mid_ch, self.ctrl.mid_ch, 1)
        self.dec_zero = []
        for i in range(len(enc_c)):
            pre = f"{cp}dec_zero_convs_out.{i}.0"
            cout = self.base.mid_ch if i == 0 else self.base.dec_out_ch[i - 1]
            store.declare_conv(pre, cout, enc_c[-(i + 1)], 1)
            self.dec_zero.append(pre)
        half = self.model_channels // 2
        import math
        self._freqs_cpu = torch.exp(-math.log(10000) * torch.arange(start=0, end=half, dtype=torch.float32) / half)
        self._freqs = None

    def _pad64(self, x: torch.Tensor) -> torch.Tensor:
        B, H, W_, c = x.shape
        key = (B, H, W_, x.dtype, ops.stream_ptr())
        cache = self.__dict__.setdefault("_pad_cache", {})
        buf = cache.get(key)
        if buf is None:
            buf = torch.zeros((B, H, W_, 64), dtype=x.dtype, device=x.device)
            cache[key] = buf
        xc = x.contiguous()
        ops.call("rdeic_act_fwd", xc.data_ptr(), B * H * W_, c, c, None, 0, 0, 0.0, buf.data_ptr(), 64,
                 ops.dt_code(x), ops.stream_ptr())
        return buf

    def timestep_embedding(self, t: torch.Tensor) -> torch.Tensor:
        if self._freqs is None:
            self._freqs = self._freqs_cpu.to(t.device)
        B = t.shape[0]
        out = torch.empty((B, self.model_channels), dtype=torch.float32, device=t.device)
        ops.call("rdeic_timestep_embedding", t.data_ptr(), self._freqs.data_ptr(), B, self.model_channels,
                 out.data_ptr(), ops.stream_ptr())
        return out

    def forward(self, x: torch.Tensor, hint: torch.Tensor, t: torch.Tensor, ctx: torch.Tensor) -> torch.Tensor:
        with ops.splitk_allowed():
            return self._forward(x, hint, t, ctx)

    def forward_unconditional(self, x: torch.Tensor, t: torch.Tensor, ctx: torch.Tensor) -> torch.Tensor:
        with ops.splitk_allowed():
            s = self.store
            dt = s.compute_dtype
            t = t.to(device=x.device, dtype=torch.int64).contiguous()
            emb_b = self.base.time_embed(self.timestep_embedding(t))
            ctx = ctx.to(dt).contiguous()
            Bc, Lc, Dc = ctx.shape
            ctx_rows = ctx.view(Bc * Lc, Dc)
            h_base = ops.cast(x, dt)
            hs_base = []
            for lb in self.base.input_blocks:
                h_base = self.base.run_layers(lb, h_base, emb_b, ctx_rows, Bc, Lc)
                hs_base.append(h_base)
            h_base = self.base.run_layers(self.base.middle, h_base, emb_b, ctx_rows, Bc, Lc)
            for lb in self.base.output_blocks:
                h_base = self.base.run_layers(lb, h_base, emb_b, ctx_rows, Bc, Lc, x2=hs_base.pop())
            p = self.base.prefix
            ab = ops.group_norm_ab(h_base, s.get(p + "out.0.weight"), s.get(p + "out.0.bias"), 32, 1e-5)
            return ops.conv2d(h_base, s.conv(p + "out.2"), gn=ab, gn_silu=True, out_f32=True)

    def _forward(self, x: torch.Tensor, hint: torch.Tensor, t: torch.Tensor, ctx: torch.Tensor) -> torch.Tensor:
        s = self.store
        dt = s.compute_dtype
        B = x.shape[0]
        t = t.to(device=x.device, dtype=torch.int64).contiguous()
        temb = self.timestep_embedding(t)
        emb_c = self.ctrl.time_embed(temb)
        emb_b = self.base.time_embed(temb)
        ctx = ctx.to(dt).contiguous()
        Bc, Lc, Dc = ctx.shape
        ctx_rows = ctx.view(Bc * Lc, Dc)
        sc = self.control_scale * self.control_scale
        h_base = ops.cast(x, dt)
        h_ctr, ctr_x2 = h_base, hint
        hs_base, hs_ctr = [], []
        for i, (lb, lc) in enumerate(zip(self.base.input_blocks, self.ctrl.input_blocks)):
            h_base0 = h_base
            h_base = self.base.run_layers(lb, h_base, emb_b, ctx_rows, Bc, Lc, stats_last=False)
            if i == 0 and dt == torch.bfloat16 and len(lc) == 1 and isinstance(lc[0], Conv) and \
                    h_base0.shape[3] % 64 and hint.shape[3] % 64 == 0:
                h_ctr = ops.conv2d(self._pad64(h_base0), s.conv_split_pad(lc[0].prefix, h_base0.shape[3], 64),
                                   x2=hint, stats=True)
            else:
                h_ctr = self.ctrl.run_layers(lc, h_ctr, emb_c, ctx_rows, Bc, Lc, x2=ctr_x2)
            ctr_x2 = None
            h_base = ops.conv2d(h_ctr, s.conv(self.enc_zero[i], scale=sc), res=h_base, stats=True)
            hs_base.append(h_base)
            hs_ctr.append(h_ctr)
        h_base = self.base.run_layers(self.base.middle, h_base, emb_b, ctx_rows, Bc, Lc, stats_last=False)
        h_ctr = self.ctrl.run_layers(self.ctrl.middle, h_ctr, emb_c, ctx_rows, Bc, Lc, stats_last=False)
        h_base = ops.conv2d(h_ctr, s.conv(self.mid_zero, scale=sc), res=h_base, stats=True)
        nout = len(self.base.output_blocks)
        for i, lb in enumerate(self.base.output_blocks):
            h_base = ops.conv2d(hs_ctr.pop(), s.conv(self.dec_zero[i], scale=sc), res=h_base, stats=True)
            h_base = self.base.run_layers(lb, h_base, emb_b, ctx_rows, Bc, Lc, x2=hs_base.pop(),
                                          stats_last=(i + 1 == nout))
        p = self.base.prefix
        ab = ops.group_norm_ab(h_base, s.get(p + "out.0.weight"), s.get(p + "out.0.bias"), 32, 1e-5)
        return ops.conv2d(h_base, s.conv(p + "out.2"), gn=ab, gn_silu=True, out_f32=True)
```

Before: 161.4 images/s.

## Fuse cross-attention with a batch-1 context into one precomputed-weight kernel

Result: no change. 162.8 images/s, median of 5 (+0.9%).

```diff
diff --git a/include/rdeic_hip.h b/include/rdeic_hip.h
--- a/include/rdeic_hip.h
+++ b/include/rdeic_hip.h
@@ -72,6 +72,9 @@
 int rdeic_attention(const void* q, int32_t ldq, const void* k, int32_t ldk, const void* v, int32_t ldv,
                     void* o, int32_t ldo, int32_t batch, int32_t heads, int32_t lq, int32_t lk, int32_t dh,
                     float scale, int32_t kv_bcast, int32_t dtype, void* stream);
+int rdeic_xattn_ctx(const void* h, int32_t ldh, int64_t rows, int32_t c, const void* mt, const void* nt,
+                    const float* colsum, const float* betam, const float* bias, int32_t heads, int32_t lk,
+                    int32_t lp, float eps, void* out, int32_t ldo, void* stream);
 int rdeic_softmax_rows(const float* s, int64_t rows, int32_t cols, float scale, void* p, int32_t dtype, void* stream);
 int rdeic_transpose(const void* in, int32_t rows, int32_t cols, int32_t ldin, void* out, int32_t ldout,
                     int32_t batch, int64_t in_bs, int64_t out_bs, int32_t dtype, void* stream);
@@ -171,6 +174,8 @@
 #define RDEIC_PROF_GEMM 5
 #define RDEIC_PROF_ATTN_D512 6
 #define RDEIC_PROF_CONV_BYTES 7
+#define RDEIC_PROF_ATTN_CTX 8
+#define RDEIC_PROF_KINDS 9
 int rdeic_prof_start(int32_t capacity, int32_t every);
 int rdeic_prof_read_keys(int32_t kind, int64_t* keys, int64_t* launches, double* work, double* ms, int32_t cap);
 #define RDEIC_COUNT_HALO_CONV 0
diff --git a/rdeic_amd/_lib.py b/rdeic_amd/_lib.py
--- a/rdeic_amd/_lib.py
+++ b/rdeic_amd/_lib.py
@@ -84,6 +84,7 @@
     "rdeic_transpose": (C.c_int, [_p, _i32, _i32, _i32, _p, _i32, _i32, _i64, _i64, _i32, _p]),
     "rdeic_attention": (C.c_int, [_p, _i32, _p, _i32, _p, _i32, _p, _i32, _i32, _i32, _i32, _i32, _i32, _f,
                                   _i32, _i32, _p]),
+    "rdeic_xattn_ctx": (C.c_int, [_p, _i32, _i64, _i32, _p, _p, _p, _p, _p, _i32, _i32, _i32, _f, _p, _i32, _p]),
     "rdeic_geglu": (C.c_int, [_p, _i32, _i32, _i32, _p, _i32, _i32, _p]),
     "rdeic_nchw_to_nhwc": (C.c_int, [_p, _i32, _i32, _i32, _i32, _f, _f, _p, _i32, _i32, _p]),
     "rdeic_nhwc_to_nchw": (C.c_int, [_p, _i32, _i32, _i32, _i32, _i32, _f, _f, _p, _i32, _p]),
diff --git a/rdeic_amd/csrc/coders.cpp b/rdeic_amd/csrc/coders.cpp
--- a/rdeic_amd/csrc/coders.cpp
+++ b/rdeic_amd/csrc/coders.cpp
@@ -420,7 +420,7 @@
 
 int rdeic_version(void) { return 1; }
 
-int rdeic_abi_count(void) { return 102; }
+int rdeic_abi_count(void) { return 103; }
 
 static int pmf_to_quantized_cdf_impl(const float* pmf, int32_t n, int32_t precision, uint32_t* cdf_out) {
   if (!pmf || !cdf_out || n <= 0 || precision <= 0 || precision > 24) return RDEIC_EINVAL;
diff --git a/rdeic_amd/csrc/conv_gemm.hip b/rdeic_amd/csrc/conv_gemm.hip
--- a/rdeic_amd/csrc/conv_gemm.hip
+++ b/rdeic_amd/csrc/conv_gemm.hip
@@ -751,6 +751,7 @@
 
 extern int rdeic_g_attn64;
 extern int rdeic_g_attn512;
+extern int rdeic_g_xattn_ctx;
 
 extern "C" int rdeic_set_conv_option(int32_t key, int32_t value) {
   if (key == 0) { int prev = g_epi_vec; g_epi_vec = value; return prev; }
@@ -763,5 +764,6 @@
   if (key == 9) { int prev = g_halo8; g_halo8 = value; return prev; }
   if (key == 10) { int prev = g_edge; g_edge = value; return prev; }
   if (key == 11) { int prev = g_up2_phases; g_up2_phases = value; return prev; }
+  if (key == 12) { int prev = rdeic_g_xattn_ctx; rdeic_g_xattn_ctx = value; return prev; }
   return RDEIC_EINVAL;
 }
diff --git a/rdeic_amd/csrc/prof.hip b/rdeic_amd/csrc/prof.hip
--- a/rdeic_amd/csrc/prof.hip
+++ b/rdeic_amd/csrc/prof.hip
@@ -28,12 +28,13 @@
 int g_used = 0;
 bool g_on = false;
 int g_every = 1;
-long g_seen[8] = {};
+long g_seen[RDEIC_PROF_KINDS] = {};
 double g_bytes_n = 0.0, g_bytes = 0.0;
 std::mutex g_mu;
 
 double always_threshold(int kind) {
-  return (kind <= RDEIC_PROF_ATTN_SMALL || kind == RDEIC_PROF_GEMM || kind == RDEIC_PROF_ATTN_D512) ? 50e9 : 64e6;
+  return (kind <= RDEIC_PROF_ATTN_SMALL || kind == RDEIC_PROF_GEMM || kind == RDEIC_PROF_ATTN_D512 ||
+          kind == RDEIC_PROF_ATTN_CTX) ? 50e9 : 64e6;
 }
 }
 
@@ -42,7 +43,7 @@
   std::lock_guard<std::mutex> lk(g_mu);
   if (!g_on || g_used >= (int)g_slots.size()) return -1;
   double weight = 1.0;
-  if (kind >= 0 && kind < 8 && g_every > 1 && work < always_threshold(kind)) {
+  if (kind >= 0 && kind < RDEIC_PROF_KINDS && g_every > 1 && work < always_threshold(kind)) {
     unsigned long long z = (unsigned long long)(g_seen[kind]++) + 0x9E3779B97F4A7C15ull;
     z = (z ^ (z >> 30)) * 0xBF58476D1CE4E5B9ull;
     z = (z ^ (z >> 27)) * 0x94D049BB133111EBull;
diff --git a/rdeic_amd/csrc/xattn_ctx.hip b/rdeic_amd/csrc/xattn_ctx.hip
--- /dev/null
+++ b/rdeic_amd/csrc/xattn_ctx.hip
@@ -0,0 +1,264 @@
+#include "common.h"
+#include "prof.h"
+#include "../../include/rdeic_hip.h"
+
+int rdeic_g_xattn_ctx = 1;
+
+namespace {
+
+typedef __attribute__((ext_vector_type(4))) short s16x4;
+typedef __attribute__((ext_vector_type(4))) unsigned u32x4;
+
+__device__ __forceinline__ f32x4 mma32(bf16x8 a, bf16x8 b, f32x4 c) {
+  return __builtin_amdgcn_mfma_f32_16x16x32_bf16(a, b, c, 0, 0, 0);
+}
+__device__ __forceinline__ f32x4 mma16(bf16x4 a, bf16x4 b, f32x4 c) {
+  return __builtin_amdgcn_mfma_f32_16x16x16bf16_1k(__builtin_bit_cast(s16x4, a), __builtin_bit_cast(s16x4, b), c, 0,
+                                                   0, 0);
+}
+__device__ __forceinline__ bf16x4 cvt4(f32x4 v) { return bf16x4{(bf16)v[0], (bf16)v[1], (bf16)v[2], (bf16)v[3]}; }
+__device__ __forceinline__ bf16x8 cat8(bf16x4 lo, bf16x4 hi) {
+  return __builtin_shufflevector(lo, hi, 0, 1, 2, 3, 4, 5, 6, 7);
+}
+
+struct XArgs {
+  const bf16* h; int ldh; long rows;
+  const bf16* mt; const bf16* nt; const float* colsum; const float* betam; const float* bias;
+  int heads, lk; float eps;
+  bf16* out; int ldo;
+};
+
+template <int C> struct XSlab { static constexpr int KS = C <= 160 ? C : (C % 160 == 0 ? 160 : 128); };
+
+template <int C, int NT, int NW> constexpr int xattn_lds_bytes() {
+  constexpr int KS = XSlab<C>::KS, LP = NT * 16;
+  constexpr int ms = LP * (KS + 8), ns = KS * (LP + 8), slab = ms > ns ? ms : ns;
+  constexpr int ring = 2 * slab, epi = NW * 16 * (C + 8);
+  return 2 * (ring > epi ? ring : epi);
+}
+
+template <int C, int NT, int NW>
+__global__ __launch_bounds__(NW * 64) void xattn_ctx_kernel(const XArgs a) {
+  constexpr int KS = XSlab<C>::KS, NS = C / KS, LP = NT * 16, KK = C / 32, CT = C / 16, NTH = NW * 64;
+  constexpr int MST = KS + 8, NST = LP + 8;
+  constexpr int MSLAB = LP * MST, NSLAB = KS * NST, SLAB = MSLAB > NSLAB ? MSLAB : NSLAB;
+  constexpr int CHUNKS = LP * KS / 8, NCH = (CHUNKS + NTH - 1) / NTH;
+  constexpr int EST = C + 8;
+  static_assert(C % KS == 0 && KS % 32 == 0 && C % 32 == 0, "slab");
+  extern __shared__ __attribute__((aligned(16))) char lds_raw[];
+  bf16* lds = (bf16*)lds_raw;
+
+  const int nwg = gridDim.x, orig = blockIdx.x;
+  const int xcd = orig & 7, q8 = nwg >> 3, rr = nwg & 7;
+  const int wgid = (xcd < rr ? xcd * (q8 + 1) : rr * (q8 + 1) + (xcd - rr) * q8) + (orig >> 3);
+
+  const int tid = threadIdx.x, lane = tid & 63, wv = tid >> 6, r16 = lane & 15, g = lane >> 4;
+  const long row0 = (long)wgid * (NW * 16) + wv * 16;
+  const long row = row0 + r16;
+  const bool rv = row < a.rows;
+  const int hl = a.heads * LP;
+
+  bf16x8 hf[KK];
+#pragma unroll
+  for (int kk = 0; kk < KK; ++kk)
+    hf[kk] = rv ? *(const bf16x8*)(a.h + row * a.ldh + kk * 32 + g * 8) : bf16x8{};
+
+  float mean, rstd;
+  {
+    float s = 0.f;
+#pragma unroll
+    for (int kk = 0; kk < KK; ++kk)
+#pragma unroll
+      for (int j = 0; j < 8; ++j) s += (float)hf[kk][j];
+    s += __shfl_xor(s, 16, 64);
+    s += __shfl_xor(s, 32, 64);
+    mean = s * (1.0f / C);
+    float v = 0.f;
+#pragma unroll
+    for (int kk = 0; kk < KK; ++kk)
+#pragma unroll
+      for (int j = 0; j < 8; ++j) {
+        const float d = (float)hf[kk][j] - mean;
+        v += d * d;
+      }
+    v += __shfl_xor(v, 16, 64);
+    v += __shfl_xor(v, 32, 64);
+    rstd = rsqrtf(v * (1.0f / C) + a.eps);
+  }
+
+  u32x4 pre[NCH];
+  auto slab_load = [&](int head, int w) {
+#pragma unroll
+    for (int i = 0; i < NCH; ++i) {
+      int c = tid + i * NTH;
+      if (CHUNKS % NTH != 0 && c >= CHUNKS) c = CHUNKS - 1;
+      const bf16* src;
+      if (w < NS) {
+        const int n = c / (KS / 8), kc = c % (KS / 8);
+        src = a.mt + (long)(head * LP + n) * C + w * KS + kc * 8;
+      } else {
+        const int col = c / (LP / 8), kc = c % (LP / 8);
+        src = a.nt + (long)((w - NS) * KS + col) * hl + head * LP + kc * 8;
+      }
+      pre[i] = *(const u32x4*)src;
+    }
+  };
+  auto slab_store = [&](bf16* buf, int w) {
+#pragma unroll
+    for (int i = 0; i < NCH; ++i) {
+      int c = tid + i * NTH;
+      if (CHUNKS % NTH != 0 && c >= CHUNKS) c = CHUNKS - 1;
+      bf16* dst;
+      if (w < NS) {
+        const int n = c / (KS / 8), kc = c % (KS / 8);
+        dst = buf + n * MST + kc * 8;
+      } else {
+        const int col = c / (LP / 8), kc = c % (LP / 8);
+        dst = buf + col * NST + kc * 8;
+      }
+      *(u32x4*)dst = pre[i];
+    }
+  };
+
+  f32x4 acc[CT];
+#pragma unroll
+  for (int i = 0; i < CT; ++i) acc[i] = f32x4{0.f, 0.f, 0.f, 0.f};
+
+  slab_load(0, 0);
+  for (int head = 0; head < a.heads; ++head) {
+    f32x4 S[NT];
+#pragma unroll
+    for (int t = 0; t < NT; ++t) S[t] = f32x4{0.f, 0.f, 0.f, 0.f};
+    bf16x8 P32[NT / 2 > 0 ? NT / 2 : 1];
+    bf16x4 P16 = bf16x4{};
+#pragma unroll
+    for (int w = 0; w < 2 * NS; ++w) {
+      bf16* buf = lds + (w & 1) * SLAB;
+      slab_store(buf, w);
+      __syncthreads();
+      if (w + 1 < 2 * NS) slab_load(head, w + 1);
+      else if (head + 1 < a.heads) slab_load(head + 1, 0);
+      if (w < NS) {
+#pragma unroll
+        for (int kk = 0; kk < KS / 32; ++kk)
+#pragma unroll
+          for (int t = 0; t < NT; ++t) {
+            const bf16x8 mf = *(const bf16x8*)(buf + (t * 16 + r16) * MST + kk * 32 + g * 8);
+            S[t] = mma32(mf, hf[w * (KS / 32) + kk], S[t]);
+          }
+        if (w == NS - 1) {
+          float mx = -INFINITY;
+#pragma unroll
+          for (int t = 0; t < NT; ++t) {
+            const f32x4 csv = *(const f32x4*)(a.colsum + head * LP + t * 16 + g * 4);
+            const f32x4 bmv = *(const f32x4*)(a.betam + head * LP + t * 16 + g * 4);
+#pragma unroll
+            for (int i = 0; i < 4; ++i) {
+              float x = rstd * (S[t][i] - mean * csv[i]) + bmv[i];
+              if (t * 16 + g * 4 + i >= a.lk) x = -INFINITY;
+              S[t][i] = x;
+              mx = fmaxf(mx, x);
+            }
+          }
+          mx = fmaxf(mx, __shfl_xor(mx, 16, 64));
+          mx = fmaxf(mx, __shfl_xor(mx, 32, 64));
+          float sum = 0.f;
+#pragma unroll
+          for (int t = 0; t < NT; ++t)
+#pragma unroll
+            for (int i = 0; i < 4; ++i) {
+              const float e = __expf(S[t][i] - mx);
+              S[t][i] = e;
+              sum += e;
+            }
+          sum += __shfl_xor(sum, 16, 64);
+          sum += __shfl_xor(sum, 32, 64);
+          const float inv = 1.0f / sum;
+#pragma unroll
+          for (int t = 0; t < NT; ++t) S[t] *= inv;
+#pragma unroll
+          for (int p = 0; p < NT / 2; ++p) P32[p] = cat8(cvt4(S[2 * p]), cvt4(S[2 * p + 1]));
+          if (NT & 1) P16 = cvt4(S[NT - 1]);
+        }
+      } else {
+#pragma unroll
+        for (int ct = 0; ct < KS / 16; ++ct) {
+          const bf16* nr = buf + (ct * 16 + r16) * NST + g * 4;
+          f32x4 o = acc[(w - NS) * (KS / 16) + ct];
+#pragma unroll
+          for (int p = 0; p < NT / 2; ++p)
+            o = mma32(cat8(*(const bf16x4*)(nr + 32 * p), *(const bf16x4*)(nr + 32 * p + 16)), P32[p], o);
+          if (NT == 1) o = mma16(*(const bf16x4*)(nr + (NT - 1) * 16), P16, o);
+          else if (NT & 1) o = mma32(cat8(*(const bf16x4*)(nr + (NT - 1) * 16), bf16x4{}), cat8(P16, bf16x4{}), o);
+          acc[(w - NS) * (KS / 16) + ct] = o;
+        }
+      }
+    }
+  }
+
+  __syncthreads();
+  bf16* ep = lds + wv * 16 * EST;
+#pragma unroll
+  for (int kk = 0; kk < KK; ++kk) *(bf16x8*)(ep + r16 * EST + kk * 32 + g * 8) = hf[kk];
+  __syncthreads();
+#pragma unroll
+  for (int ct = 0; ct < CT; ++ct) {
+    bf16* p = ep + r16 * EST + ct * 16 + g * 4;
+    const bf16x4 hv = *(const bf16x4*)p;
+    const f32x4 bv = a.bias ? *(const f32x4*)(a.bias + ct * 16 + g * 4) : f32x4{0.f, 0.f, 0.f, 0.f};
+    f32x4 o;
+#pragma unroll
+    for (int i = 0; i < 4; ++i) o[i] = acc[ct][i] + bv[i] + (float)hv[i];
+    *(bf16x4*)p = cvt4(o);
+  }
+  __syncthreads();
+  for (int idx = lane; idx < 16 * (C / 8); idx += 64) {
+    const int r = idx / (C / 8), c8 = idx % (C / 8);
+    if (row0 + r < a.rows) *(u32x4*)(a.out + (row0 + r) * a.ldo + c8 * 8) = *(const u32x4*)(ep + r * EST + c8 * 8);
+  }
+}
+
+template <int C, int NT, int NW> int launch_xattn(const XArgs& a, hipStream_t s) {
+  constexpr int lds = xattn_lds_bytes<C, NT, NW>();
+  static_assert(lds <= 160 * 1024, "LDS");
+  const unsigned grid = (unsigned)((a.rows + NW * 16 - 1) / (NW * 16));
+  hipLaunchKernelGGL((xattn_ctx_kernel<C, NT, NW>), dim3(grid), dim3(NW * 64), lds, s, a);
+  return launch_status();
+}
+
+}
+
+extern "C" int rdeic_xattn_ctx(const void* h, int32_t ldh, int64_t rows, int32_t c, const void* mt, const void* nt,
+                               const float* colsum, const float* betam, const float* bias, int32_t heads, int32_t lk,
+                               int32_t lp, float eps, void* out, int32_t ldo, void* stream) {
+  if (!h || !mt || !nt || !colsum || !betam || !out || rows <= 0 || heads <= 0 || lk <= 0 || lk > lp || lp % 16)
+    return RDEIC_EINVAL;
+  if (ldh % 8 || ldo % 8 || ldh < c || ldo < c || ((uintptr_t)h) % 16 || ((uintptr_t)out) % 16 ||
+      ((uintptr_t)mt) % 16 || ((uintptr_t)nt) % 16 || ((uintptr_t)colsum) % 16 || ((uintptr_t)betam) % 16 ||
+      (bias && ((uintptr_t)bias) % 16))
+    return RDEIC_EINVAL;
+  if (!rdeic_g_xattn_ctx) return 1;
+  XArgs a{(const bf16*)h, ldh, (long)rows, (const bf16*)mt, (const bf16*)nt, colsum, betam, bias,
+          heads, lk, eps, (bf16*)out, ldo};
+  hipStream_t s = (hipStream_t)stream;
+#define XATTN_CASE(C_, NT_, NW_)                                                                              \
+  if (c == C_ && lp == NT_ * 16) {                                                                             \
+                             \
+    const long long key = ((long long)(C_ & 0xffff) << 48) | ((long long)(rows < 0xffff ? rows : 0xffff) << 32) | \
+                          ((long long)lk << 16) | (heads & 0xffff);                                            \
+    ProfScope ps(s, RDEIC_PROF_ATTN_CTX, 4.0 * (double)rows * C_ * heads * lp, key);                           \
+    return launch_xattn<C_, NT_, NW_>(a, s);                                                                   \
+  }
+  XATTN_CASE(64, 1, 8)
+  XATTN_CASE(64, 5, 8)
+  XATTN_CASE(128, 1, 8)
+  XATTN_CASE(128, 5, 8)
+  XATTN_CASE(256, 1, 8)
+  XATTN_CASE(256, 5, 8)
+  XATTN_CASE(320, 1, 8)
+  XATTN_CASE(320, 5, 8)
+  XATTN_CASE(640, 1, 4)
+  XATTN_CASE(640, 5, 4)
+#undef XATTN_CASE
+  return 1;
+}
diff --git a/rdeic_amd/finetune.py b/rdeic_amd/finetune.py
--- a/rdeic_amd/finetune.py
+++ b/rdeic_amd/finetune.py
@@ -65,6 +65,7 @@
             self.offsets[n] = (off, k)
             off += k
         st._packed.clear()
+        st._gen += 1
         AG.PACKS.clear()
         AG.STEP_PACKS.clear()
         cb = model.preprocess_model.codebook_size
diff --git a/rdeic_amd/ops.py b/rdeic_amd/ops.py
--- a/rdeic_amd/ops.py
+++ b/rdeic_amd/ops.py
@@ -415,7 +415,7 @@
 
 
 PROF_KINDS = {"conv": 0, "attention": 1, "attention_dh16": 2, "gn_stats": 3, "gn_apply": 4, "gemm": 5,
-              "attention_d512": 6, "conv_bytes": 7}
+              "attention_d512": 6, "conv_bytes": 7, "attention_ctx": 8}
 
 
 def prof_start(capacity: int = 65536, every: int = 1) -> None:
@@ -703,6 +703,50 @@
             "rdeic_attention", q.data_ptr(), q.stride(0), k.data_ptr(), k.stride(0), v.data_ptr(),
             v.stride(0), out.data_ptr(), out.stride(0), batch, heads, lq, lk, dh, float(scale),
             int(kv_bcast), dt_code(q), stream_ptr())
+    return out
+
+
+XATTN_CTX = True
+XATTN_CTX_TABLE = {(320, 5, 65536), (64, 4, 65536)}
+
+
+@dataclass
+class XattnCtx:
+    c: int
+    heads: int
+    lk: int
+    lp: int
+    kv: torch.Tensor
+    mt: Optional[torch.Tensor]
+    nt: Optional[torch.Tensor]
+    colsum: Optional[torch.Tensor]
+    betam: Optional[torch.Tensor]
+    bias: Optional[torch.Tensor]
+
+
+def set_xattn_ctx(on: bool) -> bool:
+    global XATTN_CTX
+    prev = XATTN_CTX
+    XATTN_CTX = bool(on)
+    _lib.load().rdeic_set_conv_option(12, int(XATTN_CTX))
+    return prev
+
+
+def xattn_ctx_fused(c: int, heads: int, rows: int) -> bool:
+    return XATTN_CTX_TABLE is None or (c, heads, rows) in XATTN_CTX_TABLE
+
+
+def xattn_ctx(h: torch.Tensor, f: XattnCtx, eps: float = 1e-5, out: Optional[torch.Tensor] = None):
+    rows, c = h.shape
+    if f.mt is None or h.dtype != torch.bfloat16 or c != f.c or h.stride(1) != 1:
+        return None
+    if out is None:
+        out = torch.empty((rows, c), dtype=h.dtype, device=h.device)
+    tag = ("attention_ctx", 4.0 * rows * c * f.heads * f.lp, None)
+    if not _launch_soft(tag, "rdeic_xattn_ctx", h.data_ptr(), h.stride(0), rows, c, f.mt.data_ptr(), f.nt.data_ptr(),
+                        f.colsum.data_ptr(), f.betam.data_ptr(), _ptr(f.bias), f.heads, f.lk, f.lp, float(eps),
+                        out.data_ptr(), out.stride(0), stream_ptr()):
+        return None
     return out
 
 
diff --git a/rdeic_amd/params.py b/rdeic_amd/params.py
--- a/rdeic_amd/params.py
+++ b/rdeic_amd/params.py
@@ -1,5 +1,6 @@
 from __future__ import annotations
 
+import threading
 from typing import Dict, Iterable, Optional, Sequence, Tuple
 
 import torch
@@ -17,6 +18,41 @@
     return f.reshape(4, cout, 4 * cin).to(dtype).contiguous()
 
 
+def fold_xattn_ctx(wq: torch.Tensor, wk: torch.Tensor, wv: torch.Tensor, wo: torch.Tensor, ctx: torch.Tensor,
+                   heads: int, gamma: Optional[torch.Tensor] = None, beta: Optional[torch.Tensor] = None,
+                   bq: Optional[torch.Tensor] = None, bk: Optional[torch.Tensor] = None,
+                   bv: Optional[torch.Tensor] = None, lp: Optional[int] = None):
+    C = wq.shape[0]
+    d = C // heads
+    lk = ctx.shape[0]
+    lp = -(-lk // 16) * 16 if lp is None else lp
+    c64 = ctx.double()
+    K = c64 @ wk.double().t()
+    V = c64 @ wv.double().t()
+    if bk is not None:
+        K = K + bk.double()
+    if bv is not None:
+        V = V + bv.double()
+    Kh, Vh = K.view(lk, heads, d), V.view(lk, heads, d)
+    scale = float(d) ** -0.5
+    m = scale * torch.einsum("hdc,lhd->chl", wq.double().view(heads, d, C), Kh)
+    bm = torch.zeros((heads, lk), dtype=torch.float64, device=m.device)
+    if beta is not None:
+        bm = bm + torch.einsum("c,chl->hl", beta.double(), m)
+    if bq is not None:
+        bm = bm + scale * torch.einsum("hd,lhd->hl", bq.double().view(heads, d), Kh)
+    if gamma is not None:
+        m = gamma.double()[:, None, None] * m
+    n = torch.einsum("lhd,chd->hlc", Vh, wo.double().view(C, heads, d))
+    mp = torch.zeros((C, heads, lp), dtype=torch.float64, device=m.device)
+    mp[:, :, :lk] = m
+    npad = torch.zeros((heads, lp, C), dtype=torch.float64, device=m.device)
+    npad[:, :lk] = n
+    bmp = torch.zeros((heads, lp), dtype=torch.float64, device=m.device)
+    bmp[:, :lk] = bm
+    return mp.reshape(C, heads * lp), npad.reshape(heads * lp, C), bmp.reshape(heads * lp)
+
+
 class ParamStore:
     def __init__(self, compute_dtype=torch.bfloat16, device="cuda"):
         self.compute_dtype = compute_dtype
@@ -24,6 +60,10 @@
         self.shapes: Dict[str, Tuple[int, ...]] = {}
         self.t: Dict[str, torch.Tensor] = {}
         self._packed: Dict[tuple, ops.ConvParams] = {}
+        self._gen = 0
+        self._xctx_key = None
+        self._xctx: Dict[str, ops.XattnCtx] = {}
+        self._xctx_lock = threading.Lock()
 
     def declare(self, name: str, shape: Sequence[int]):
         shape = tuple(int(s) for s in shape)
@@ -52,6 +92,7 @@
             ops.fill_uniform(t, W.param_seed(name, global_seed), scale, offset)
             self.t[name] = t
         self._packed.clear()
+        self._gen += 1
 
     def load_state_dict(self, sd: Dict[str, torch.Tensor], strict: bool = True):
         missing = [n for n in self.shapes if n not in sd]
@@ -65,6 +106,7 @@
                 raise ValueError(f"{name}: checkpoint shape {tuple(v.shape)} != {shape}")
             self.t[name] = v.detach().to(device=self.device, dtype=torch.float32).contiguous()
         self._packed.clear()
+        self._gen += 1
 
     def names(self) -> Iterable[str]:
         return self.shapes.keys()
@@ -180,3 +222,58 @@
                                     dtype=dtype)
             self._packed[key] = p
         return p
+
+    XCTX_MAX_FOLD_C = 640
+
+    def xattn_ctx(self, ctx: torch.Tensor, blocks: Sequence[Tuple[str, int, int]]) -> Dict[str, ops.XattnCtx]:
+        if ctx.dim() != 3 or ctx.shape[0] != 1:
+            raise ValueError("the context fold is for one context shared by the batch ([1, Lk, D])")
+        names = [b[0] + s for b in blocks for s in (".attn2.to_q.weight", ".attn2.to_k.weight", ".attn2.to_v.weight",
+                                                    ".attn2.to_out.0.weight", ".norm2.weight", ".norm2.bias")]
+        key = (ctx.data_ptr(), tuple(ctx.shape), ctx.dtype, ctx._version, str(ctx.device), self._gen,
+               tuple(b for b in blocks), tuple((self.t[n].data_ptr(), self.t[n]._version) for n in names))
+        with self._xctx_lock:
+            if key == self._xctx_key:
+                return self._xctx
+            from . import _lib
+            if _lib.RECORDER is not None:
+                raise RuntimeError("ParamStore.xattn_ctx inside a recorded region: fold the context before it")
+            dt = self.compute_dtype
+            c2 = ctx.detach().to(device=self.device, dtype=dt).contiguous()[0]
+            lk = c2.shape[0]
+            lp = -(-lk // 16) * 16
+            torch.cuda.synchronize()
+            self._xctx_key = None
+            for tb, C, heads in blocks:
+                ent = self._xctx.get(tb)
+                if ent is None or ent.lk != lk or ent.c != C or ent.heads != heads:
+                    fold = C <= self.XCTX_MAX_FOLD_C and C % 64 == 0 and dt == torch.bfloat16
+                    ent = ops.XattnCtx(
+                        c=C, heads=heads, lk=lk, lp=lp,
+                        kv=torch.empty((lk, 2 * C), dtype=dt, device=self.device),
+                        mt=torch.empty((heads * lp, C), dtype=dt, device=self.device) if fold else None,
+                        nt=torch.empty((C, heads * lp), dtype=dt, device=self.device) if fold else None,
+                        colsum=torch.empty(heads * lp, dtype=torch.float32, device=self.device) if fold else None,
+                        betam=torch.empty(heads * lp, dtype=torch.float32, device=self.device) if fold else None,
+                        bias=None)
+                    self._xctx[tb] = ent
+                ops.linear(c2, self.conv_cat([tb + ".attn2.to_k", tb + ".attn2.to_v"]), images=1, out=ent.kv)
+                if ent.mt is None:
+                    continue
+                g = lambda n: self.t.get(tb + n)
+                m, n, bm = fold_xattn_ctx(g(".attn2.to_q.weight").reshape(C, -1), g(".attn2.to_k.weight").reshape(C, -1),
+                                          g(".attn2.to_v.weight").reshape(C, -1),
+                                          g(".attn2.to_out.0.weight").reshape(C, -1), c2, heads,
+                                          gamma=g(".norm2.weight"), beta=g(".norm2.bias"), bq=g(".attn2.to_q.bias"),
+                                          bk=g(".attn2.to_k.bias"), bv=g(".attn2.to_v.bias"), lp=lp)
+                ent.mt.copy_(m.t().float())
+                ent.nt.copy_(n.t().float())
+                ent.colsum.copy_(ent.mt.double().sum(1).float())
+                ent.betam.copy_(bm.float())
+                ent.bias = self.conv(tb + ".attn2.to_out.0").bias
+            for tb in [k for k in self._xctx if k not in {b[0] for b in blocks}]:
+                del self._xctx[tb]
+            torch.cuda.current_stream().synchronize()
+            self._xctx_key = key
+            self._xctx_ref = ctx
+            return self._xctx
diff --git a/rdeic_amd/rdeic.py b/rdeic_amd/rdeic.py
--- a/rdeic_amd/rdeic.py
+++ b/rdeic_amd/rdeic.py
@@ -11,7 +11,7 @@
 from .compression import Compression
 from .config import default_config
 from .params import ParamStore
-from .unet import NoiseEstimator
+from .unet import NoiseEstimator, ctx_fold_bind, ctx_fold_handed
 from .vae import AutoencoderKL
 
 
@@ -255,6 +255,7 @@
         ops.call("rdeic_axpby", c_latent.data_ptr(), noise.data_ptr(), B, c_latent[0].numel(), c["qa"].data_ptr(),
                  c["qb"].data_ptr(), x.data_ptr(), ops.stream_ptr())
         smp = self._sampler(self, sampler)
+        ctx_fold_bind(context)
         if sampler == "ddpm":
             z = smp.sample_nhwc(steps, x, guide_hint, context, step_noise=list(step_noise.unbind(0)),
                                 ts_tensors=c["ts"])
@@ -274,10 +275,11 @@
         elif sampler != "ddim":
             raise ValueError(f"sampler {sampler!r} (ddpm | ddim)")
         fn = (lambda a, b, c, d, *e: self._relay_decode_u8(a, b, c, d, steps, sampler, e[0] if e else None))
-        if not self.use_plans:
-            return fn(*ins)
-        key = ("relay_decode", steps, sampler) + tuple((tuple(t.shape), t.dtype) for t in ins)
-        return self._plans.run(key, fn, ins).clone()
+        with ctx_fold_handed(self.control_model.ctx_fold(context)):
+            if not self.use_plans:
+                return fn(*ins)
+            key = ("relay_decode", steps, sampler) + tuple((tuple(t.shape), t.dtype) for t in ins)
+            return self._plans.run(key, fn, ins).clone()
 
     @torch.no_grad()
     def codec_images(self, img_u8: torch.Tensor, context: torch.Tensor, noise_nchw: torch.Tensor, steps: int = 2,
diff --git a/rdeic_amd/unet.py b/rdeic_amd/unet.py
--- a/rdeic_amd/unet.py
+++ b/rdeic_amd/unet.py
@@ -1,11 +1,12 @@
 from __future__ import annotations
 
+import threading
 from dataclasses import dataclass, field
 from typing import List, Optional
 
 import torch
 
-from . import ops
+from . import _lib, ops
 from .params import ParamStore
 
 
@@ -17,6 +18,34 @@
             return start
         start -= 1
     return 1
+
+
+_CTX_TLS = threading.local()
+
+
+def ctx_fold_entry(tb: str):
+    fold = getattr(_CTX_TLS, "active", None)
+    return None if fold is None else fold.get(tb)
+
+
+class ctx_fold_handed:
+
+    def __init__(self, fold):
+        self.fold = fold
+
+    def __enter__(self):
+        self._prev = (getattr(_CTX_TLS, "handed", None), getattr(_CTX_TLS, "is_handed", False),
+                      getattr(_CTX_TLS, "handed_ptr", None))
+        _CTX_TLS.handed, _CTX_TLS.is_handed, _CTX_TLS.handed_ptr = self.fold, True, None
+        return self
+
+    def __exit__(self, *exc):
+        _CTX_TLS.handed, _CTX_TLS.is_handed, _CTX_TLS.handed_ptr = self._prev
+
+
+def ctx_fold_bind(ctx: torch.Tensor) -> None:
+    if getattr(_CTX_TLS, "is_handed", False):
+        _CTX_TLS.handed_ptr = ctx.data_ptr()
 
 
 @dataclass
@@ -213,16 +242,26 @@
         ops.attention(qkv[:, :C], qkv[:, C:2 * C], qkv[:, 2 * C:], o, batch=B, heads=t.heads, lq=L, lk=L, dh=t.dh,
                       scale=scale)
         h = ops.linear(o, s.conv(tb + ".attn1.to_out.0"), res=h, images=B)
-        if fold:
-            q = ops.linear(h, s.conv_ln([tb + ".attn2.to_q"], tb + ".norm2"), ln_rows=ops.layer_norm_rowstats(h),
-                           images=B)
+        xf = ctx_fold_entry(tb) if (fold and ctx_batch == 1 and ops.XATTN_CTX) else None
+        if xf is not None and (xf.lk != ctx_len or xf.c != C or xf.heads != t.heads):
+            xf = None
+        h2 = ops.xattn_ctx(h, xf) if (xf is not None and ops.xattn_ctx_fused(C, t.heads, rows)) else None
+        if h2 is not None:
+            h = h2
         else:
-            n2 = ops.layer_norm(h, s.get(tb + ".norm2.weight"), s.get(tb + ".norm2.bias"))
-            q = ops.linear(n2, s.conv(tb + ".attn2.to_q"), images=B)
-        kv = ops.linear(ctx_kv_in, s.conv_cat([tb + ".attn2.to_k", tb + ".attn2.to_v"]), images=ctx_batch)
-        ops.attention(q, kv[:, :C], kv[:, C:], o, batch=B, heads=t.heads, lq=L, lk=ctx_len, dh=t.dh, scale=scale,
-                      kv_bcast=(ctx_batch == 1 and B > 1))
-        h = ops.linear(o, s.conv(tb + ".attn2.to_out.0"), res=h, images=B)
+            if fold:
+                q = ops.linear(h, s.conv_ln([tb + ".attn2.to_q"], tb + ".norm2"), ln_rows=ops.layer_norm_rowstats(h),
+                               images=B)
+            else:
+                n2 = ops.layer_norm(h, s.get(tb + ".norm2.weight"), s.get(tb + ".norm2.bias"))
+                q = ops.linear(n2, s.conv(tb + ".attn2.to_q"), images=B)
+            if xf is not None:
+                kv = xf.kv
+            else:
+                kv = ops.linear(ctx_kv_in, s.conv_cat([tb + ".attn2.to_k", tb + ".attn2.to_v"]), images=ctx_batch)
+            ops.attention(q, kv[:, :C], kv[:, C:], o, batch=B, heads=t.heads, lq=L, lk=ctx_len, dh=t.dh, scale=scale,
+                          kv_bcast=(ctx_batch == 1 and B > 1))
+            h = ops.linear(o, s.conv(tb + ".attn2.to_out.0"), res=h, images=B)
         if fold and ops.GEGLU_FUSED:
             gg = ops.linear(h, s.conv_ln([tb + ".ff.net.0.proj"], tb + ".norm3", geglu=True),
                             ln_rows=ops.layer_norm_rowstats(h), geglu=True, images=B)
@@ -309,9 +348,32 @@
                  out.data_ptr(), ops.stream_ptr())
         return out
 
+    def ctx_fold(self, ctx: torch.Tensor):
+        if not (ops.XATTN_CTX and ops.LN_FOLD and self.store.compute_dtype == torch.bfloat16 and ctx.dim() == 3
+                and ctx.shape[0] == 1):
+            return None
+        blocks = self.__dict__.get("_xattn_blocks")
+        if blocks is None:
+            blocks = tuple((st.prefix + ".transformer_blocks.0", st.ch, st.heads)
+                           for net in (self.base, self.ctrl)
+                           for layers in net.input_blocks + [net.middle] + net.output_blocks
+                           for st in layers if isinstance(st, SpatialTransformer) and st.ch % 64 == 0)
+            self._xattn_blocks = blocks
+        return self.store.xattn_ctx(ctx, blocks)
+
     def forward(self, x: torch.Tensor, hint: torch.Tensor, t: torch.Tensor, ctx: torch.Tensor) -> torch.Tensor:
-        with ops.splitk_allowed():
-            return self._forward(x, hint, t, ctx)
+        if getattr(_CTX_TLS, "is_handed", False):
+            ptr = _CTX_TLS.handed_ptr
+            fold = _CTX_TLS.handed if (ptr is None or ptr == ctx.data_ptr()) else None
+        else:
+            fold = self.ctx_fold(ctx) if _lib.RECORDER is None else None
+        prev = getattr(_CTX_TLS, "active", None)
+        _CTX_TLS.active = fold
+        try:
+            with ops.splitk_allowed():
+                return self._forward(x, hint, t, ctx)
+        finally:
+            _CTX_TLS.active = prev
 
     def forward_unconditional(self, x: torch.Tensor, t: torch.Tensor, ctx: torch.Tensor) -> torch.Tensor:
         with ops.splitk_allowed():
```
